# qirui-chen/RGA3-release

Hardware: AMD Instinct MI355X
Metric: video-QA samples/sec (fwd+bwd) at 7B/16-frame — full RGA3 training step (Qwen2.5-VL-7B + SAM2-L + mask losses + AdamW) (higher is better)
Workload: dtype bf16

## Files before the change

include/rga3_hip.h:

```cpp
#ifndef RGA3_HIP_H
#define RGA3_HIP_H

#include <stddef.h>
#include <stdint.h>

#ifdef __cplusplus
extern "C" {
#endif

#define RGA3_EINVAL (-22)

#define RGA3_BF16 0
#define RGA3_F32 1

#define RGA3_ACT_NONE 0
#define RGA3_ACT_GELU 1
#define RGA3_ACT_SWIGLU 2
#define RGA3_ACT_RELU 3

int rga3_version(void);
int rga3_last_error(char* buf, size_t n);

int rga3_gemm_bf16(const void* A, const void* W, const void* bias, const void* residual, const void* colscale, void* C, int64_t M, int64_t N,
                   int64_t K, int64_t lda, int64_t ldw, int64_t ldc, int64_t ldr, int act, int out_dtype, int tile,
// ... 14 lines not shown


int rga3_attn_varlen_fwd(const void* q, const void* k, const void* v, void* o, float* lse, const int32_t* cu_q,
                         const int32_t* cu_k, int nseg, int max_q, int64_t total_q, int Hq, int Hkv, int D, int64_t q_st, int64_t q_sh,
                         int64_t k_st, int64_t k_sh, int64_t v_st, int64_t v_sh, int64_t o_st, int64_t o_sh,
                         float scale, int causal, int impl, float* split_ws, int64_t split_ws_elems, int max_k, int block_q, int block_k, void* stream);
int rga3_attn_varlen_fwd_rope(const void* q, const void* k, const void* v, void* o, float* lse, const int32_t* cu_q, const int32_t* cu_k, int nseg, int max_q,
                              int64_t total_q, int Hq, int Hkv, int D, int64_t q_st, int64_t q_sh, int64_t k_st, int64_t k_sh, int64_t v_st, int64_t v_sh,
                              int64_t o_st, int64_t o_sh, float scale, int causal, const float* cos_q, const float* sin_q, const float* cos_k,
                              const float* sin_k, void* stream);

int rga3_rmsnorm_fwd(const void* x, const void* add, const void* weight, void* y, void* res_out, int64_t rows,
                     int64_t dim, int64_t ldx, float eps, void* stream);

int rga3_layernorm_fwd(const void* x, const void* weight, const void* bias, void* y, int64_t rows, int64_t dim,
                       int64_t ldx, int64_t ldy, float eps, int act, void* stream);
int rga3_layernorm_stats(const void* x, float* stats, int64_t rows, int64_t dim, int64_t ldx, float eps, void* stream);
int rga3_gemm_ln_bf16(const void* A, const void* Wf, const void* bias, const float* colc, const float* rowstat, void* C, int64_t M, int64_t N, int64_t K,
                      int64_t lda, int64_t ldw, int64_t ldc, int act, int tile, void* stream);
int64_t rga3_gemm_lnsum_slices(int64_t N, int tile);
int rga3_gemm_lnsum_bf16(const void* A, const void* W, const void* bias, const void* residual, void* C, int64_t M, int64_t N, int64_t K, int64_t lda,
                         int64_t ldw, int64_t ldc, int64_t ldr, int tile, float* row_parts, void* stream);
int rga3_gemm_lnq_bf16(const void* A, const void* Wf, const void* bias, const float* colc, const float* row_parts, int64_t slices, int64_t norm_width, float eps,
                       void* C, int64_t M, int64_t N, int64_t K, int64_t lda, int64_t ldw, int64_t ldc, int act, int tile, void* stream);

int rga3_rope_inplace(void* x, const float* cos, const float* sin, int64_t T, int h0, int nh, int D, int64_t st,
                      int64_t sh, void* stream);

int rga3_gather_rows(const void* table, const int64_t* idx, void* out, int64_t n_idx, int64_t rows_per_idx,
                     int64_t dim, int64_t ld_table, int64_t ld_out, void* stream);
int rga3_scatter_rows(const void* src, const int64_t* idx, void* out, int64_t n_idx, int64_t rows_per_idx, int64_t dim,
                      int64_t ld_src, int64_t ld_out, void* stream);

int rga3_pad_cols(const void* src, void* dst, int64_t rows, int64_t cols, int64_t ld_src, int64_t ld_dst, void* stream);

int rga3_silu_mul(const void* a, const void* b, void* out, int64_t n, void* stream);
int rga3_add(const void* a, const void* b, void* out, int64_t n, void* stream);

int rga3_cross_entropy_rows(const void* logits, int logits_dtype, const int64_t* labels, float* row_loss,
                            void* dlogits, int64_t rows, int64_t V, int64_t ld, float grad_scale, void* stream);


int rga3_im2col(const void* img, void* out, int64_t F, int C, int H, int W, int ks, int stride, int pad, int64_t ld_out,
                void* stream);
int rga3_maxpool2x2_win(const void* x, void* y, int64_t nwin, int w, int C, int64_t ldx, int64_t ldy, void* stream);
int rga3_upsample2x_add(const void* a, const void* b, void* out, int64_t F, int H, int W, int C, void* stream);
int rga3_add_bcast(const void* a, const void* b, void* out, int64_t rows, int64_t rows_b, int C, int64_t lda, int64_t ldb,
                   int64_t ldo, float alpha, void* stream);
int rga3_bilinear(const void* in, int in_dtype, float* out, const int32_t* plane_idx, int64_t N, int Hi, int Wi, int Ho, int Wo,
                  void* stream);
int rga3_conv3x3s2(const void* x, int x_dtype, const void* w, const void* bias, void* y, int64_t F, int H, int W, int Cin, int Cout,
                   float sig_scale, float sig_bias, void* stream);
int rga3_decimg_rows(const void* keys, int64_t keys_stride, const void* pe, int64_t pe_stride, int hw, const void* kt, const void* vt, int nk, const void* wq, const void* bq,
                     const void* wo, const void* bo, const void* ln_w, const void* ln_b, float eps, const void* wk2, const void* bk2, const void* wv2, const void* bv2,
                     void* keys_out, int64_t keys_out_stride, void* k2, void* v2, int64_t kv_stride, int v2_transposed, float scale, int64_t M, void* stream);
int rga3_attn_fewq(const void* q, int64_t q_stride, const void* k, int64_t k_stride, int64_t k_head_stride, const void* vt, const void* vbias, void* out, int64_t out_stride,
                   int frames, int nq, int nk, int H, float scale, void* stream);
int rga3_copy_many(void* const* dst, const void* const* src, const int64_t* bytes, int n, void* stream);
int rga3_conv3x3s2_ln_gelu(const void* x, int x_dtype, const void* w, const void* bias, const void* ln_w, const void* ln_b, float eps, void* y, int64_t F, int H, int W,
                           int Cin, int Cout, float sig_scale, float sig_bias, void* stream);
int rga3_im2col3x3s2(const void* x, void* cols, int64_t F, int H, int W, int C, void* stream);
int rga3_dwconv7x7(const void* x, const void* w, const void* bias, void* y, int64_t F, int H, int W, int C, void* stream);
int rga3_rope_axial_inplace(void* x, const float* cos, const float* sin, int64_t n_rope, int nq, int C, int64_t ldx, void* stream);
int rga3_pixel_shuffle2x(const void* g, const void* bias, const void* add, void* out, int64_t F, int H, int W, int Co, int act, void* stream);
int rga3_bce_dice_sums(const float* logits, const float* targets, float* out4, int64_t n_masks, int64_t hw, void* stream);
int64_t rga3_bce_dice_sums_ws_floats(int64_t n_masks, int64_t hw);
int rga3_bce_dice_sums_det(const float* logits, const float* targets, float* out4, float* ws, int64_t ws_floats, int64_t n_masks, int64_t hw, void* stream);
int64_t rga3_mask_jf_ws_bytes(int64_t frames, int64_t h, int64_t w);
int rga3_mask_jf_counts(const void* seg, const void* ann, const void* void_pixels, int64_t* counts, void* ws, int64_t ws_bytes, int64_t frames, int64_t h, int64_t w,
                        int radius, void* stream);
int64_t rga3_stom_ws_bytes(int64_t frames, int64_t h, int64_t w);
int rga3_stom_flow(const float* tracks, const void* visibility, int* records, int64_t frames, int64_t n_points, int vip_frame_idx, void* stream);
int rga3_stom_shift_composite(const void* frames_u8, const void* overlay_rgba, const int* records, void* out, int64_t frames, int64_t h, int64_t w, int vip_frame_idx,
                              void* stream);
int rga3_stom_mask_composite(const void* frames_u8, const void* overlay_rgba, const float* tracks, const void* visibility, void* out, void* ws, int64_t ws_bytes,
                             int64_t frames, int64_t h, int64_t w, int64_t n_points, int vip_frame_idx, const void* spans, int ksize, const void* half_widths,
                             int radius, void* stream);


int rga3_attn_varlen_bwd(const void* q, const void* k, const void* v, const void* o, const void* dout, const float* lse, void* dq,
                         void* dk, void* dv, float* delta_ws, const int32_t* cu_q, const int32_t* cu_k, int nseg, int max_q,
                         int max_k, int64_t total_q, int Hq, int Hkv, int D, const int64_t* strides16, float scale, int causal,
                         float* dkv_ws, int64_t total_k, void* stream);
int rga3_hiera_mlp144(const void* x, const void* w1f, const float* c1, const void* d1, const void* w2, const void* b2, void* y, int64_t M, float eps, void* stream);
int64_t rga3_hiera_mlp288_pack_bytes(void);
int rga3_hiera_mlp288_pack(const void* w1f, const float* c1, const void* d1, const void* w2, void* pack, void* stream);
int rga3_hiera_mlp288(const void* x, const void* pack, const void* b2, void* y, int64_t M, float eps, void* stream);
int rga3_mlp3_rows(const void* const* ptrs, const int64_t* dims, int n, int64_t B, void* stream);
int rga3_sam_select_objptr(const void* iou, const void* obj, const void* toks, int64_t tok_bstride, int C, const void* w0, const void* b0, const void* w1, const void* b1,
                           const void* w2, const void* b2, const void* no_obj_ptr, int64_t* best, int32_t* sel, void* obj_ptr, int64_t B, void* stream);
int64_t rga3_memattn_cross_ws_floats(int64_t Nq, int nsplit);
int rga3_memattn_cross(const void* q, const void* k, const void* m, void* out, int64_t Nq, int64_t Nk, int64_t q_stride, int64_t k_stride, int64_t m_stride,
                       int64_t out_stride, float scale, int nsplit, float* ws, void* stream);
int rga3_memlayer_rows(const void* a, int64_t a_stride, int K1, const float* part_o, const float* part_ml, int nsplit, const void* w1, const void* b1,
                       const void* res, int64_t res_stride, void* x_out, int64_t x_stride, const void* ln_w, const void* ln_b, float eps, void* t_out,
                       int64_t t_stride, const void* w2, const void* b2, int N2, void* y_out, int64_t y_stride, const float* cos, const float* sin,
                       int rope_cols, int nq, int64_t M, void* stream);
int rga3_gemm_rows16_many(const void* const* ptrs, const int64_t* dims, int n, void* stream);
int rga3_gemm_stream_k_timeouts(const void* workspace);
int64_t rga3_gemm_timeout_counter_offset(void);
int rga3_gemm_ragged_plan(int64_t M, int64_t N, int64_t K, int cus, int split, int* plan, unsigned* start);
int rga3_gemm_tiles(int entry, int* ids, int* bm, int* bn, int cap);
int rga3_gemm_candidates(int entry, int64_t M, int64_t N, int64_t K, int act, int out_dtype, int epilogue, int* ids, int cap);
int rga3_gemm_tn_slices(int64_t M, int64_t N, int64_t K);
int rga3_rmsnorm_bwd(const void* x, const void* weight, const void* dy, const void* add, void* dx, int64_t rows, int64_t dim, float eps,
                     void* stream);
int rga3_dropout_bf16(const void* x, void* y, int64_t n, float p, int64_t seed, int accumulate, void* stream);
int rga3_dropout_pair_bf16(const void* xa, const void* xb, void* ya, void* yb, int64_t n, float pa, int64_t seed_a, float pb, int64_t seed_b, int sum, void* stream);
int rga3_swiglu_fwd(const void* gu, void* a, int64_t T, int64_t I, void* stream);
int rga3_swiglu_bwd(const void* gu, const void* da, void* dgu, int64_t T, int64_t I, void* stream);
int rga3_transpose16(const void* in, void* out, int64_t R, int64_t C, int64_t ld_in, int64_t ld_out, void* stream);
int rga3_transpose16_many(const void* const* ptrs, const int64_t* dims, int n, void* stream);
int rga3_segment_sum_rows(const void* x, const int64_t* rows, const int64_t* offsets, void* out, int64_t n_out, int64_t dim, int64_t ldx,
                          void* stream);
int rga3_adamw_step(void* param, float* master, const void* grad, float* m, float* v, int64_t n, float lr, float beta1, float beta2,
                    float eps, float weight_decay, int step, float grad_scale, void* stream);
int rga3_sumsq_accum(const void* g, float* out, int64_t n, void* stream);
int rga3_sumsq_det(const void* g, int64_t n, float* partials, int64_t partials_cap, float* out, int accumulate, void* stream);
int rga3_adamw_step_clip(void* param, float* master, const void* grad, float* m, float* v, int64_t n, float lr, float beta1, float beta2,
                         float eps, float weight_decay, int step, const float* sumsq, float max_norm, void* stream);
int rga3_adamw_step_clip_rows(void* param, float* master, const void* grad, float* m, float* v, int64_t rows, int64_t row_len, const uint8_t* row_active,
                              float lr, float beta1, float beta2, float eps, int step, const float* sumsq, float max_norm, void* stream);
int rga3_scatter_add_rows(void* dst, const int64_t* idx, const void* src, int64_t n, int64_t dim, int64_t ld_dst, int64_t ld_src, float scale,
                          void* stream);


int64_t rga3_layernorm_bwd_ws_floats(int64_t rows, int64_t dim);
int rga3_layernorm_bwd(const void* x, const void* weight, const void* dy, void* dx, float* dweight, float* dbias, int64_t rows, int64_t dim,
                       float eps, float* ws, int64_t ws_floats, void* stream);
int rga3_colsum_accum(const void* x, float* out, int64_t rows, int64_t cols, int64_t ld, void* stream);
int64_t rga3_colsum_ws_floats(int64_t rows, int64_t cols);
int rga3_colsum(const void* x, float* out, int64_t rows, int64_t cols, int64_t ld, float* ws, int64_t ws_floats, void* counters, void* stream);
int rga3_act(const void* a, const void* dy, void* out, int64_t n, int kind, void* stream);
int rga3_bilinear_bwd(const float* dout, float* din, const int32_t* plane_idx, int64_t N, int Hi, int Wi, int Ho, int Wo, void* stream);
int rga3_mask_product(const void* hyper, const void* up, float* masks, int64_t B, int64_t NM, int64_t P, int64_t C, void* stream);
int64_t rga3_mask_product_bwd_ws_floats(int64_t B, int64_t NM, int64_t P, int64_t C);
int rga3_mask_product_bwd(const float* dmasks, const void* hyper, const void* up, void* dup, void* dhyper, int64_t B, int64_t NM, int64_t P, int64_t C,
                          float* ws, int64_t ws_floats, void* stream);
int rga3_pixel_shuffle2x_bwd(const void* dout, void* dg, int64_t F, int H, int W, int Co, void* stream);
int rga3_bce_dice_grad(const float* logits, const float* targets, const float* sums4, float* dlogits, int64_t n_masks, int64_t hw,
                       float coef_bce, float coef_dice, void* stream);
int rga3_bce_dice_grad_dev(const float* logits, const float* targets, const float* sums4, float* dlogits, int64_t n_masks, int64_t hw,
                           const float* coef_bce_dev, const float* coef_dice_dev, void* stream);

int rga3_pil_bicubic_coeffs(int in_size, int out_size, int32_t* bounds, int32_t* kk, int64_t kk_capacity, int* ksize_out);
int rga3_sam_preprocess_u8(const void* frames, int64_t T, int H, int W, int out_h, int out_w, const int32_t* bh, const int32_t* kh,
                           int ksize_h, const int32_t* bv, const int32_t* kv, int ksize_v, void* tmp, void* dst_u8, void* dst_bf16,
                           const float* mean3, const float* std3, void* stream);

int rga3_qwen_norm_lut(const float* mean3, const float* std3, int fused, float* lut768);
int rga3_qwen_patchify_u8(const void* frames, int64_t T, int h, int w, const float* lut768, void* out, int out_dtype, int patch, int tpatch,
                          int merge, void* stream);

int rga3_quant_fp8_rows(const void* x, void* q, float* scales, int64_t rows, int64_t K, int64_t ldx, int64_t ldq, void* stream);
int rga3_gemm_fp8(const void* Aq, const void* Wq, const float* sa, const float* sw, const void* bias, const void* residual, void* C, int64_t M,
                  int64_t N, int64_t K, int64_t lda, int64_t ldw, int64_t ldc, int64_t ldr, void* stream);
int rga3_swiglu_fwd_quant_fp8(const void* gu, void* q, float* scales, int64_t T, int64_t I, void* stream);
int rga3_swiglu_bwd_quant_fp8(const void* gu, const void* da, void* q, float* scales, int64_t T, int64_t I, void* stream);

#ifdef __cplusplus
}
#endif
#endif
```

rga3-release_amd/csrc/attn_bwd.hip:

```cpp
#include "common.h"

namespace rga3 {

struct AttnBwdArgs {
    const unsigned short *q, *k, *v, *o, *dout;
    unsigned short *dq, *dk, *dv;
    const float* lse;
    float* delta;
    const int *cu_q, *cu_k;
    long q_st, q_sh, k_st, k_sh, v_st, v_sh, o_st, o_sh, do_st, do_sh, dq_st, dq_sh, dk_st, dk_sh, dv_st, dv_sh;
    int Hq, Hkv, D;
    long total_q;
    float scale, scale_log2;
    int causal;
    float* dkv_ws;
    long total_k;
    int gx, gy;
};

constexpr int BT = 64;

template <int DP, int QT, int NWAVE, bool PAIR>
__global__ __launch_bounds__(64 * NWAVE) void attn_bwd_dq_kernel(AttnBwdArgs p) {
    constexpr int NT = 64 * NWAVE;
    constexpr int BLOCK_M = NWAVE * QT * 16;
    constexpr int CH = DP / 8;
    constexpr int STRIDE = DP * 2 + 32;
    constexpr int DS = DP / 32, DT = DP / 16;
    constexpr int LOADS = (BT * CH) / NT;
    static_assert((BT * CH) % NT == 0, "tile chunks must divide evenly over threads");

    extern __shared__ __attribute__((aligned(16))) char smem[];
    char* Ks = smem;
    char* Vs = smem + BT * STRIDE;

    const int tid = threadIdx.x, lane = tid & 63;
    const int wid = __builtin_amdgcn_readfirstlane(tid >> 6);
    const int g = lane >> 4, c = lane & 15;
    const Wg3 wg = xcd_decode3(p.gx, p.gy);
    const int seg = wg.z, hq = wg.y;
    const int hk = hq / (p.Hq / p.Hkv);
    const int qs = p.cu_q[seg], Lq = p.cu_q[seg + 1] - qs;
    const int ks = p.cu_k[seg], Lk = p.cu_k[seg + 1] - ks;
    const int shift = Lk - Lq;
    const int nqb = (Lq + BLOCK_M - 1) / BLOCK_M;
    int qb_first = wg.x, qb_second = -1;
    if constexpr (PAIR) {
        qb_first = nqb - 1 - wg.x;
        qb_second = wg.x;
        if (qb_second > qb_first) return;
        if (qb_second == qb_first) qb_second = -1;
    } else if (qb_first >= nqb) {
        return;
    }
    for (int pass = 0; pass < (PAIR ? 2 : 1); ++pass) {
    const int qbi = pass == 0 ? qb_first : qb_second;
    if (qbi < 0) break;
    if (pass == 1) __syncthreads();
    const int qb0 = qbi * BLOCK_M;
    const int qw0 = qb0 + wid * (QT * 16);

    bf16x8 qf[QT][DS], dof[QT][DS];
    float lse2[QT], dl[QT];
#pragma unroll
    for (int t = 0; t < QT; ++t) {
        const int qi = qw0 + t * 16 + c;
        const bool ok = qi < Lq;
#pragma unroll
        for (int ds = 0; ds < DS; ++ds) {
            const int d = ds * 32 + g * 8;
            u32x4 z = {0u, 0u, 0u, 0u}, y = {0u, 0u, 0u, 0u};
            if (ok && d < p.D) {
                z = *(const u32x4*)(p.q + (long)(qs + qi) * p.q_st + (long)hq * p.q_sh + d);
                y = *(const u32x4*)(p.dout + (long)(qs + qi) * p.do_st + (long)hq * p.do_sh + d);
            }
            qf[t][ds] = __builtin_bit_cast(bf16x8, z);
            dof[t][ds] = __builtin_bit_cast(bf16x8, y);
        }
        lse2[t] = ok ? p.lse[(long)hq * p.total_q + qs + qi] * 1.4426950408889634f : 0.f;
    }
#pragma unroll
    for (int t = 0; t < QT; ++t) {
        const int qi = qw0 + t * 16 + c;
        const bool ok = qi < Lq;
        float dp = 0.f;
#pragma unroll
        for (int ds = 0; ds < DS; ++ds) {
            const int d = ds * 32 + g * 8;
            if (ok && d < p.D) {
                const u32x4 ov = *(const u32x4*)(p.o + (long)(qs + qi) * p.o_st + (long)hq * p.o_sh + d);
                const u32x4 dv = __builtin_bit_cast(u32x4, dof[t][ds]);
#pragma unroll
                for (int i = 0; i < 4; ++i) {
                    dp += __uint_as_float(ov[i] << 16) * __uint_as_float(dv[i] << 16);
                    dp += __uint_as_float(ov[i] & 0xffff0000u) * __uint_as_float(dv[i] & 0xffff0000u);
                }
            }
        }
        dp += __shfl_xor(dp, 16, 64);
        dp += __shfl_xor(dp, 32, 64);
        dl[t] = ok ? dp : 0.f;
        if (ok && g == 0) p.delta[(long)hq * p.total_q + qs + qi] = dp;
    }

    f32x4 dqacc[QT][DT];
#pragma unroll
// ... 14 lines not shown
            const int r = idx / CH, ch = idx % CH;
            const int key = kt * BT + r;
            u32x4 zk = {0u, 0u, 0u, 0u}, zv = {0u, 0u, 0u, 0u};
            if (key < Lk && ch * 8 < p.D) {
                zk = *(const u32x4*)(p.k + (long)(ks + key) * p.k_st + (long)hk * p.k_sh + ch * 8);
                zv = *(const u32x4*)(p.v + (long)(ks + key) * p.v_st + (long)hk * p.v_sh + ch * 8);
            }
            kreg[i] = zk;
            vreg[i] = zv;
        }
    };
    auto store_tile = [&]() {
#pragma unroll
        for (int i = 0; i < LOADS; ++i) {
            const int idx = tid + i * NT;
            const int r = idx / CH, ch = idx % CH;
            *(u32x4*)(Ks + r * STRIDE + ch * 16) = kreg[i];
            *(u32x4*)(Vs + r * STRIDE + ch * 16) = vreg[i];
        }
    };

    if (ntiles > 0) load_tile(0);
    for (int kt = 0; kt < ntiles; ++kt) {
        __syncthreads();
        store_tile();
        __syncthreads();
        if (kt + 1 < ntiles) load_tile(kt + 1);
        const int k0 = kt * BT;
        const bool need_mask = (k0 + BT > Lk) || (p.causal && (k0 + BT - 1 > qb0 + shift));
#pragma unroll
        for (int t = 0; t < QT; ++t) {
            const int qi = qw0 + t * 16 + c;
            f32x4 s[4], dp[4];
#pragma unroll
            for (int j = 0; j < 4; ++j) { s[j] = f32x4{0.f, 0.f, 0.f, 0.f}; dp[j] = f32x4{0.f, 0.f, 0.f, 0.f}; }
#pragma unroll
            for (int j = 0; j < 4; ++j)
#pragma unroll
                for (int ds = 0; ds < DS; ++ds) {
                    bf16x8 kf = *(const bf16x8*)(Ks + (j * 16 + c) * STRIDE + ds * 64 + g * 16);
                    bf16x8 vf = *(const bf16x8*)(Vs + (j * 16 + c) * STRIDE + ds * 64 + g * 16);
                    s[j] = __builtin_amdgcn_mfma_f32_16x16x32_bf16(kf, qf[t][ds], s[j], 0, 0, 0);
                    dp[j] = __builtin_amdgcn_mfma_f32_16x16x32_bf16(vf, dof[t][ds], dp[j], 0, 0, 0);
                }
            bf16x8 dsf[2];
#pragma unroll
            for (int ss = 0; ss < 2; ++ss) {
                float e[8];
#pragma unroll
                for (int u = 0; u < 8; ++u) {
                    const int j = 2 * ss + (u >> 2), r = u & 3;
                    float pr = __builtin_amdgcn_exp2f(s[j][r] * p.scale_log2 - lse2[t]);
                    if (need_mask) {
                        const int key = k0 + j * 16 + 4 * g + r;
                        const bool ok = (key < Lk) && (!p.causal || key <= qi + shift);
                        pr = ok ? pr : 0.f;
                    }
                    if (qi >= Lq) pr = 0.f;
                    e[u] = pr * (dp[j][r] - dl[t]) * p.scale;
                }
                u32x4 pk;
                pk[0] = pack_bf2(e[0], e[1]); pk[1] = pack_bf2(e[2], e[3]); pk[2] = pack_bf2(e[4], e[5]); pk[3] = pack_bf2(e[6], e[7]);
                dsf[ss] = __builtin_bit_cast(bf16x8, pk);
            }
#pragma unroll
            for (int d = 0; d < DT; ++d)
#pragma unroll
                for (int ss = 0; ss < 2; ++ss) {
                    const char* a0 = Ks + (ss * 32 + 4 * g + (c >> 2)) * STRIDE + (d * 16 + 4 * (c & 3)) * 2;
                    bf16x4 lo = __builtin_amdgcn_ds_read_tr16_b64_v4bf16((__attribute__((address_space(3))) bf16x4*)(a0));
                    bf16x4 hi = __builtin_amdgcn_ds_read_tr16_b64_v4bf16((__attribute__((address_space(3))) bf16x4*)(a0 + 16 * STRIDE));
                    bf16x8 kt8;
                    kt8[0] = lo[0]; kt8[1] = lo[1]; kt8[2] = lo[2]; kt8[3] = lo[3];
                    kt8[4] = hi[0]; kt8[5] = hi[1]; kt8[6] = hi[2]; kt8[7] = hi[3];
                    dqacc[t][d] = __builtin_amdgcn_mfma_f32_16x16x32_bf16(kt8, dsf[ss], dqacc[t][d], 0, 0, 0);
                }
        }
    }
#pragma unroll
    for (int t = 0; t < QT; ++t) {
        const int qi = qw0 + t * 16 + c;
        if (qi < Lq) {
            unsigned short* row = p.dq + (long)(qs + qi) * p.dq_st + (long)hq * p.dq_sh;
#pragma unroll
            for (int d = 0; d < DT; ++d) {
                const int dd = d * 16 + 4 * g;
                if (dd < p.D) {
                    u32x2 pk;
                    pk[0] = pack_bf2(dqacc[t][d][0], dqacc[t][d][1]);
                    pk[1] = pack_bf2(dqacc[t][d][2], dqacc[t][d][3]);
                    *(u32x2*)(row + dd) = pk;
                }
            }
        }
    }
    }
}

template <int DP, int NWAVE, bool SPLIT, bool PAIR>
__global__ __launch_bounds__(64 * NWAVE) void attn_bwd_dkv_kernel(AttnBwdArgs p) {
    constexpr int NT = 64 * NWAVE;
    constexpr int BLOCK_N = NWAVE * 16;
    constexpr int CH = DP / 8;
    constexpr int STRIDE = DP * 2 + 32;
    constexpr int DS = DP / 32, DT = DP / 16;
    constexpr int LOADS = (BT * CH) / NT;
    static_assert((BT * CH) % NT == 0, "tile chunks must divide evenly over threads");

    extern __shared__ __attribute__((aligned(16))) char smem[];
    char* Qs = smem;
    char* Os = smem + BT * STRIDE;
    float* Ls = (float*)(smem + 2 * BT * STRIDE);

    const int tid = threadIdx.x, lane = tid & 63;
    const int wid = __builtin_amdgcn_readfirstlane(tid >> 6);
    const int g = lane >> 4, c = lane & 15;
    const Wg3 wg = xcd_decode3(p.gx, p.gy);
    const int seg = wg.z;
    const int group = p.Hq / p.Hkv;
    const int hk = SPLIT ? wg.y / group : wg.y;
    const int hh0 = SPLIT ? wg.y % group : 0, hh1 = SPLIT ? hh0 + 1 : group;
    const int qs = p.cu_q[seg], Lq = p.cu_q[seg + 1] - qs;
    const int ks = p.cu_k[seg], Lk = p.cu_k[seg + 1] - ks;
    const int shift = Lk - Lq;
    const int nkb = (Lk + BLOCK_N - 1) / BLOCK_N;
    int kb_first = wg.x, kb_second = -1;
    if constexpr (PAIR) {
        kb_first = wg.x;
        kb_second = nkb - 1 - wg.x;
        if (kb_first > kb_second) return;
        if (kb_second == kb_first) kb_second = -1;
    } else if (kb_first >= nkb) {
        return;
    }
    for (int pass = 0; pass < (PAIR ? 2 : 1); ++pass) {
    const int kbi = pass == 0 ? kb_first : kb_second;
    if (kbi < 0) break;
    if (pass == 1) __syncthreads();
    const int kb0 = kbi * BLOCK_N;
    const int key = kb0 + wid * 16 + c;

    bf16x8 kf[DS], vf[DS];
#pragma unroll
    for (int ds = 0; ds < DS; ++ds) {
        const int d = ds * 32 + g * 8;
        u32x4 z = {0u, 0u, 0u, 0u}, y = {0u, 0u, 0u, 0u};
        if (key < Lk && d < p.D) {
            z = *(const u32x4*)(p.k + (long)(ks + key) * p.k_st + (long)hk * p.k_sh + d);
            y = *(const u32x4*)(p.v + (long)(ks + key) * p.v_st + (long)hk * p.v_sh + d);
        }
        kf[ds] = __builtin_bit_cast(bf16x8, z);
        vf[ds] = __builtin_bit_cast(bf16x8, y);
    }
    f32x4 dkacc[DT], dvacc[DT];
#pragma unroll
    for (int d = 0; d < DT; ++d) { dkacc[d] = f32x4{0.f, 0.f, 0.f, 0.f}; dvacc[d] = f32x4{0.f, 0.f, 0.f, 0.f}; }

    int q_begin = 0;
    if (p.causal) q_begin = max(0, kb0 - shift);
    const int t0 = q_begin / BT;
    const int ntq = (Lq + BT - 1) / BT;

    u32x4 qreg[LOADS], oreg[LOADS];
    float lreg = 0.f, dreg = 0.f;
    auto load_tile = [&](int hq_, int qt_) {
#pragma unroll
        for (int i = 0; i < LOADS; ++i) {
            const int idx = tid + i * NT;
            const int r = idx / CH, ch = idx % CH;
            const int qi = qt_ * BT + r;
            u32x4 zq = {0u, 0u, 0u, 0u}, zo = {0u, 0u, 0u, 0u};
            if (qi < Lq && ch * 8 < p.D) {
                zq = *(const u32x4*)(p.q + (long)(qs + qi) * p.q_st + (long)hq_ * p.q_sh + ch * 8);
                zo = *(const u32x4*)(p.dout + (long)(qs + qi) * p.do_st + (long)hq_ * p.do_sh + ch * 8);
            }
            qreg[i] = zq;
            oreg[i] = zo;
        }
        if (tid < BT) {
            const int qi = qt_ * BT + tid;
            lreg = (qi < Lq) ? p.lse[(long)hq_ * p.total_q + qs + qi] * 1.4426950408889634f : 0.f;
            dreg = (qi < Lq) ? p.delta[(long)hq_ * p.total_q + qs + qi] : 0.f;
        }
// ... 16 lines not shown
        const int hq = hk * group + hh;
        for (int qt = t0; qt < ntq; ++qt) {
            __syncthreads();
            store_tile();
            __syncthreads();
            if (qt + 1 < ntq) load_tile(hq, qt + 1);
            else if (hh + 1 < hh1) load_tile(hq + 1, t0);
            const int q0 = qt * BT;
            f32x4 s[4], dp[4];
#pragma unroll
            for (int j = 0; j < 4; ++j) { s[j] = f32x4{0.f, 0.f, 0.f, 0.f}; dp[j] = f32x4{0.f, 0.f, 0.f, 0.f}; }
#pragma unroll
            for (int j = 0; j < 4; ++j)
#pragma unroll
                for (int ds = 0; ds < DS; ++ds) {
                    bf16x8 qa = *(const bf16x8*)(Qs + (j * 16 + c) * STRIDE + ds * 64 + g * 16);
                    bf16x8 oa = *(const bf16x8*)(Os + (j * 16 + c) * STRIDE + ds * 64 + g * 16);
                    s[j] = __builtin_amdgcn_mfma_f32_16x16x32_bf16(qa, kf[ds], s[j], 0, 0, 0);
                    dp[j] = __builtin_amdgcn_mfma_f32_16x16x32_bf16(oa, vf[ds], dp[j], 0, 0, 0);
                }
            bf16x8 pf[2], dsf[2];
#pragma unroll
            for (int ss = 0; ss < 2; ++ss) {
                float e[8], f[8];
#pragma unroll
                for (int u = 0; u < 8; ++u) {
                    const int j = 2 * ss + (u >> 2), r = u & 3;
                    const int ql = j * 16 + 4 * g + r;
                    const int qi = q0 + ql;
                    float pr = __builtin_amdgcn_exp2f(s[j][r] * p.scale_log2 - Ls[ql]);
                    const bool ok = (qi < Lq) && (key < Lk) && (!p.causal || key <= qi + shift);
                    pr = ok ? pr : 0.f;
                    e[u] = pr;
                    f[u] = pr * (dp[j][r] - Ls[BT + ql]) * p.scale;
                }
                u32x4 a, b;
                a[0] = pack_bf2(e[0], e[1]); a[1] = pack_bf2(e[2], e[3]); a[2] = pack_bf2(e[4], e[5]); a[3] = pack_bf2(e[6], e[7]);
                b[0] = pack_bf2(f[0], f[1]); b[1] = pack_bf2(f[2], f[3]); b[2] = pack_bf2(f[4], f[5]); b[3] = pack_bf2(f[6], f[7]);
                pf[ss] = __builtin_bit_cast(bf16x8, a);
                dsf[ss] = __builtin_bit_cast(bf16x8, b);
            }
#pragma unroll
            for (int d = 0; d < DT; ++d)
#pragma unroll
                for (int ss = 0; ss < 2; ++ss) {
                    const int roff = (ss * 32 + 4 * g + (c >> 2)) * STRIDE + (d * 16 + 4 * (c & 3)) * 2;
                    bf16x4 ol = __builtin_amdgcn_ds_read_tr16_b64_v4bf16((__attribute__((address_space(3))) bf16x4*)(Os + roff));
                    bf16x4 oh = __builtin_amdgcn_ds_read_tr16_b64_v4bf16((__attribute__((address_space(3))) bf16x4*)(Os + roff + 16 * STRIDE));
                    bf16x4 ql_ = __builtin_amdgcn_ds_read_tr16_b64_v4bf16((__attribute__((address_space(3))) bf16x4*)(Qs + roff));
                    bf16x4 qh_ = __builtin_amdgcn_ds_read_tr16_b64_v4bf16((__attribute__((address_space(3))) bf16x4*)(Qs + roff + 16 * STRIDE));
                    bf16x8 ot, qt8;
                    ot[0] = ol[0]; ot[1] = ol[1]; ot[2] = ol[2]; ot[3] = ol[3]; ot[4] = oh[0]; ot[5] = oh[1]; ot[6] = oh[2]; ot[7] = oh[3];
                    qt8[0] = ql_[0]; qt8[1] = ql_[1]; qt8[2] = ql_[2]; qt8[3] = ql_[3]; qt8[4] = qh_[0]; qt8[5] = qh_[1]; qt8[6] = qh_[2]; qt8[7] = qh_[3];
                    dvacc[d] = __builtin_amdgcn_mfma_f32_16x16x32_bf16(ot, pf[ss], dvacc[d], 0, 0, 0);
                    dkacc[d] = __builtin_amdgcn_mfma_f32_16x16x32_bf16(qt8, dsf[ss], dkacc[d], 0, 0, 0);
                }
        }
    }
    if constexpr (SPLIT) {
        if (key < Lk) {
            const long half = (long)group * p.total_k * p.Hkv * p.D;
            float* wk = p.dkv_ws + (((long)hh0 * p.total_k + ks + key) * p.Hkv + hk) * p.D;
#pragma unroll
            for (int d = 0; d < DT; ++d) {
                const int dd = d * 16 + 4 * g;
                if (dd < p.D) {
                    *(f32x4*)(wk + dd) = dkacc[d];
                    *(f32x4*)(wk + half + dd) = dvacc[d];
                }
            }
        }
        continue;
    }
    if (key < Lk) {
        unsigned short* rk = p.dk + (long)(ks + key) * p.dk_st + (long)hk * p.dk_sh;
        unsigned short* rv = p.dv + (long)(ks + key) * p.dv_st + (long)hk * p.dv_sh;
#pragma unroll
        for (int d = 0; d < DT; ++d) {
            const int dd = d * 16 + 4 * g;
            if (dd < p.D) {
                u32x2 a, b;
                a[0] = pack_bf2(dkacc[d][0], dkacc[d][1]); a[1] = pack_bf2(dkacc[d][2], dkacc[d][3]);
                b[0] = pack_bf2(dvacc[d][0], dvacc[d][1]); b[1] = pack_bf2(dvacc[d][2], dvacc[d][3]);
                *(u32x2*)(rk + dd) = a;
                *(u32x2*)(rv + dd) = b;
            }
        }
    }
    }
}

__global__ __launch_bounds__(256) void attn_dkv_reduce_kernel(AttnBwdArgs p) {
    const int group = p.Hq / p.Hkv;
    const int d4 = p.D / 4;
    const long idx = (long)blockIdx.x * 256 + threadIdx.x;
    const long total = p.total_k * p.Hkv * d4;
    if (idx >= total) return;
    const int dd = (int)(idx % d4) * 4;
    const long row = idx / d4;
    const int hk = (int)(row % p.Hkv);
    const long key = row / p.Hkv;
    const long plane = p.total_k * p.Hkv * (long)p.D, half = (long)group * plane;
    const float* w = p.dkv_ws + row * p.D + dd;
    f32x4 sk = *(const f32x4*)w, sv = *(const f32x4*)(w + half);
    for (int h = 1; h < group; ++h) {
        sk += *(const f32x4*)(w + h * plane);
        sv += *(const f32x4*)(w + half + h * plane);
    }
    u32x2 a, b;
    a[0] = pack_bf2(sk[0], sk[1]); a[1] = pack_bf2(sk[2], sk[3]);
    b[0] = pack_bf2(sv[0], sv[1]); b[1] = pack_bf2(sv[2], sv[3]);
    *(u32x2*)(p.dk + key * p.dk_st + (long)hk * p.dk_sh + dd) = a;
    *(u32x2*)(p.dv + key * p.dv_st + (long)hk * p.dv_sh + dd) = b;
}

template <auto K>
static int launch_bwd_grid(AttnBwdArgs& a, int lds, unsigned gx, int gy, int nseg, int nwave, hipStream_t st, const char* name) {
    a.gx = (int)gx; a.gy = gy;
    return launch_lds<K>(dim3(gx * (unsigned)gy * (unsigned)nseg), dim3(64 * nwave), lds, st, name, a);
}

template <int DP>
static int launch_bwd(const AttnBwdArgs& a0, int nseg, int max_q, int max_k, hipStream_t st) {
    AttnBwdArgs a = a0;
    a.gx = 1; a.gy = 1;
    constexpr int NW = (DP == 128) ? 8 : 4;
#ifdef RGA3_BWD_DQ_QT2
    constexpr int QT = 2, NWQ = 4;
#else
    constexpr int QT = (DP >= 128) ? 1 : 2, NWQ = NW;
#endif
    constexpr int BLOCK_M = NWQ * QT * 16;
    constexpr int LDS_DQ = 2 * BT * (DP * 2 + 32);
    constexpr int LDS_DKV = 2 * BT * (DP * 2 + 32) + 2 * BT * 4;
    const unsigned nqb = (unsigned)cdiv(max_q, BLOCK_M), nkb = (unsigned)cdiv(max_k, 16 * NW);
    const bool pair = a.causal && nqb >= 4 && nkb >= 4;
    const unsigned gq = pair ? (nqb + 1) / 2 : nqb, gk = pair ? (nkb + 1) / 2 : nkb;
    if (int rc = pair ? launch_bwd_grid<attn_bwd_dq_kernel<DP, QT, NWQ, true>>(a, LDS_DQ, gq, a.Hq, nseg, NWQ, st, "attn_bwd_dq_kernel")
                      : launch_bwd_grid<attn_bwd_dq_kernel<DP, QT, NWQ, false>>(a, LDS_DQ, gq, a.Hq, nseg, NWQ, st, "attn_bwd_dq_kernel"))
        return rc;
    if (a.dkv_ws && a.Hq > a.Hkv) {
        if (int rc = pair ? launch_bwd_grid<attn_bwd_dkv_kernel<DP, NW, true, true>>(a, LDS_DKV, gk, a.Hq, nseg, NW, st, "attn_bwd_dkv_kernel<split>")
                          : launch_bwd_grid<attn_bwd_dkv_kernel<DP, NW, true, false>>(a, LDS_DKV, gk, a.Hq, nseg, NW, st, "attn_bwd_dkv_kernel<split>"))
            return rc;
        const long rows = a.total_k * a.Hkv;
        hipLaunchKernelGGL(attn_dkv_reduce_kernel, dim3((unsigned)cdiv(rows * (a.D / 4), 256)), dim3(256), 0, st, a);
        RGA3_CHECK_LAUNCH("attn_dkv_reduce_kernel");
        return 0;
    }
    return pair ? launch_bwd_grid<attn_bwd_dkv_kernel<DP, NW, false, true>>(a, LDS_DKV, gk, a.Hkv, nseg, NW, st, "attn_bwd_dkv_kernel")
                : launch_bwd_grid<attn_bwd_dkv_kernel<DP, NW, false, false>>(a, LDS_DKV, gk, a.Hkv, nseg, NW, st, "attn_bwd_dkv_kernel");
}

}

using namespace rga3;

extern "C" int rga3_attn_varlen_bwd(const void* q, const void* k, const void* v, const void* o, const void* dout, const float* lse,
                                    void* dq, void* dk, void* dv, float* delta_ws, const int32_t* cu_q, const int32_t* cu_k, int nseg,
                                    int max_q, int max_k, int64_t total_q, int Hq, int Hkv, int D, const int64_t* strides16, float scale,
                                    int causal, float* dkv_ws, int64_t total_k, void* stream) {
    RGA3_CHECK_ARG(q && k && v && o && dout && lse && dq && dk && dv && delta_ws && cu_q && cu_k && strides16, "attn_bwd: null pointer");
    RGA3_CHECK_ARG(nseg > 0 && max_q > 0 && max_k > 0 && total_q > 0, "attn_bwd: sizes");
    RGA3_CHECK_ARG(Hq > 0 && Hkv > 0 && Hq % Hkv == 0, "attn_bwd: Hq=%d Hkv=%d", Hq, Hkv);
    RGA3_CHECK_ARG(D >= 8 && D <= 128 && D % 8 == 0, "attn_bwd: head dim %d unsupported (multiple of 8, <= 128)", D);
    for (int i = 0; i < 16; ++i) RGA3_CHECK_ARG(strides16[i] % 4 == 0, "attn_bwd: stride %d must be a multiple of 4 elements", i);
    for (int i = 0; i < 10; ++i) RGA3_CHECK_ARG(strides16[i] % 8 == 0, "attn_bwd: input stride %d must be a multiple of 8 elements", i);
    {
        static const char* const names[8] = {"q", "k", "v", "o", "dout", "dq", "dk", "dv"};
        for (int i = 0; i < 8; ++i) {
            const bool kv = i == 1 || i == 2 || i == 6 || i == 7;
            RGA3_CHECK_HEADS("attn_bwd", names[i], strides16[2 * i], strides16[2 * i + 1], kv ? total_k : total_q, kv ? Hkv : Hq, D);
        }
    }
    AttnBwdArgs a;
    a.q = (const unsigned short*)q; a.k = (const unsigned short*)k; a.v = (const unsigned short*)v; a.o = (const unsigned short*)o;
    a.dout = (const unsigned short*)dout; a.dq = (unsigned short*)dq; a.dk = (unsigned short*)dk; a.dv = (unsigned short*)dv;
    a.lse = lse; a.delta = delta_ws; a.cu_q = cu_q; a.cu_k = cu_k;
    a.q_st = strides16[0]; a.q_sh = strides16[1]; a.k_st = strides16[2]; a.k_sh = strides16[3]; a.v_st = strides16[4]; a.v_sh = strides16[5];
    a.o_st = strides16[6]; a.o_sh = strides16[7]; a.do_st = strides16[8]; a.do_sh = strides16[9]; a.dq_st = strides16[10]; a.dq_sh = strides16[11];
    a.dk_st = strides16[12]; a.dk_sh = strides16[13]; a.dv_st = strides16[14]; a.dv_sh = strides16[15];
    a.Hq = Hq; a.Hkv = Hkv; a.D = D; a.total_q = total_q; a.scale = scale; a.scale_log2 = scale * 1.4426950408889634f; a.causal = causal;
    a.dkv_ws = dkv_ws; a.total_k = total_k;
    RGA3_CHECK_ARG(!dkv_ws || (total_k > 0 && D % 4 == 0), "attn_bwd: dkv_ws needs total_k");
    hipStream_t st = (hipStream_t)stream;
    if (D <= 32) return launch_bwd<32>(a, nseg, max_q, max_k, st);
    if (D <= 64) return launch_bwd<64>(a, nseg, max_q, max_k, st);
    if (D <= 96) return launch_bwd<96>(a, nseg, max_q, max_k, st);
    return launch_bwd<128>(a, nseg, max_q, max_k, st);
}
```

rga3-release_amd/csrc/common.h:

```cpp
#pragma once
#include <hip/hip_runtime.h>

#include "errors.h"

namespace rga3 {

#define RGA3_CHECK_LAUNCH(name)                                                                  \
    do {                                                                                         \
        hipError_t e__ = hipGetLastError();                                                      \
        if (e__ != hipSuccess) return ::rga3::fail(-(int)e__, "%s: %s", name, hipGetErrorString(e__)); \
    } while (0)

struct LdsGrant { int bytes[16] = {0}; };
inline int grant_dyn_lds(const void* kern, int bytes, LdsGrant& g, const char* name) {
    if (bytes <= 48 * 1024) return 0;
    int dev = 0;
    if (hipGetDevice(&dev) != hipSuccess || dev < 0) dev = 0;
    const bool tracked = dev < 16;
    if (tracked && g.bytes[dev] >= bytes) return 0;
    hipError_t e = hipFuncSetAttribute(kern, hipFuncAttributeMaxDynamicSharedMemorySize, bytes);
    if (e != hipSuccess) return fail(-(int)e, "%s: hipFuncSetAttribute(%d B dynamic LDS): %s", name, bytes, hipGetErrorString(e));
    if (tracked) g.bytes[dev] = bytes;
    return 0;
}

template <auto K, class... A>
int launch_lds(dim3 grid, dim3 block, int lds, hipStream_t st, const char* name, const A&... args) {
    static LdsGrant grant;
    if (int rc = grant_dyn_lds((const void*)K, lds, grant, name)) return rc;
    hipLaunchKernelGGL(K, grid, block, lds, st, args...);
    RGA3_CHECK_LAUNCH(name);
    return 0;
}

typedef __attribute__((ext_vector_type(8))) __bf16 bf16x8;
typedef __attribute__((ext_vector_type(4))) __bf16 bf16x4;
typedef __attribute__((ext_vector_type(2))) __bf16 bf16x2;
typedef __attribute__((ext_vector_type(4))) float f32x4;
typedef __attribute__((ext_vector_type(16))) float f32x16;
typedef __attribute__((ext_vector_type(4))) unsigned int u32x4;
typedef __attribute__((ext_vector_type(2))) unsigned int u32x2;

typedef __attribute__((address_space(3))) void lds_void;
typedef const __attribute__((address_space(1))) void gbl_void;

__device__ __forceinline__ float bf2f(unsigned short u) { return __uint_as_float(((unsigned int)u) << 16); }
__device__ __forceinline__ unsigned short f2bf(float f) {
    __bf16 b = (__bf16)f;
    return __builtin_bit_cast(unsigned short, b);
}
__device__ __forceinline__ unsigned int pack_bf2(float lo, float hi) {
    bf16x2 v;
    v[0] = (__bf16)lo;
    v[1] = (__bf16)hi;
    return __builtin_bit_cast(unsigned int, v);
}
__device__ __forceinline__ void unpack8(const u32x4& v, float* f) {
#pragma unroll
    for (int i = 0; i < 4; ++i) {
        f[2 * i] = __uint_as_float(v[i] << 16);
        f[2 * i + 1] = __uint_as_float(v[i] & 0xffff0000u);
    }
}
__device__ __forceinline__ u32x4 pack8(const float* f) {
    u32x4 v;
#pragma unroll
    for (int i = 0; i < 4; ++i) v[i] = pack_bf2(f[2 * i], f[2 * i + 1]);
    return v;
}
__device__ __forceinline__ float bf16_round(float v) { return bf2f(f2bf(v)); }

__device__ __forceinline__ float wave_sum(float v) {
#pragma unroll
    for (int o = 32; o > 0; o >>= 1) v += __shfl_xor(v, o, 64);
    return v;
}
__device__ __forceinline__ float wave_max(float v) {
#pragma unroll
    for (int o = 32; o > 0; o >>= 1) v = fmaxf(v, __shfl_xor(v, o, 64));
    return v;
}

__device__ __forceinline__ float swiglu_fwd_elem(float g, float u) {
#pragma clang fp contract(off)
    const float silu = g / (1.f + __expf(-g));
    return bf16_round(silu) * u;
}
__device__ __forceinline__ void swiglu_bwd_elem(float g, float u, float d, float& dg, float& du) {
#pragma clang fp contract(off)
    const float sg = 1.f / (1.f + __expf(-g));
    const float silu = g * sg;
    du = d * silu;
    dg = d * u * sg * (1.f + g * (1.f - sg));
}

static inline int64_t cdiv(int64_t a, int64_t b) { return (a + b - 1) / b; }

static inline unsigned grid1d(long total, int per_block = 256, long cap = 256L * 32) {
    long b = cdiv(total, per_block);
    if (b < 1) b = 1;
    return (unsigned)(b > cap ? cap : b);
}

typedef const unsigned short* cus;
typedef unsigned short* us;

constexpr int kNumXCD = 8;

__device__ __forceinline__ unsigned xcd_remap(unsigned bid, unsigned nwg) {
    unsigned q = nwg / kNumXCD, r = nwg % kNumXCD, x = bid % kNumXCD;
    unsigned base = (x < r) ? x * (q + 1) : r * (q + 1) + (x - r) * q;
    return base + bid / kNumXCD;
}

struct Wg3 { int x, y, z; };
__device__ __forceinline__ Wg3 xcd_decode3(int gx, int gy) {
    const unsigned lid = xcd_remap(blockIdx.x, gridDim.x);
    Wg3 w;
    w.y = (int)(lid % (unsigned)gy);
    w.x = (int)((lid / (unsigned)gy) % (unsigned)gx);
    w.z = (int)(lid / ((unsigned)gy * (unsigned)gx));
    return w;
}

}
```

rga3-release_amd/csrc/rowops.hip:

```cpp
#include "common.h"

namespace rga3 {

template <int MAXC>
__global__ __launch_bounds__(256) void rmsnorm_kernel(const unsigned short* __restrict__ x, const unsigned short* __restrict__ add,
                                                      const unsigned short* __restrict__ w, unsigned short* __restrict__ y,
                                                      unsigned short* __restrict__ res_out, long rows, int dim, long ldx, float eps) {
    const int lane = threadIdx.x & 63;
    const long row = (long)blockIdx.x * 4 + (threadIdx.x >> 6);
    if (row >= rows) return;
    const int nch = dim / 8;
    u32x4 buf[MAXC], abuf[MAXC];
    float ss = 0.f;
#pragma unroll
    for (int i = 0; i < MAXC; ++i) {
        const int ch = lane + i * 64;
        if (ch < nch) {
            buf[i] = *(const u32x4*)(x + row * ldx + ch * 8);
            if (add) abuf[i] = *(const u32x4*)(add + row * ldx + ch * 8);
        }
    }
#pragma unroll
    for (int i = 0; i < MAXC; ++i) {
        const int ch = lane + i * 64;
        if (ch < nch) {
            u32x4 v = buf[i];
            float f[8];
            unpack8(v, f);
            if (add) {
                float fa[8];
                unpack8(abuf[i], fa);
#pragma unroll
                for (int e = 0; e < 8; ++e) f[e] = bf2f(f2bf(f[e] + fa[e]));
                v = pack8(f);
                if (res_out) *(u32x4*)(res_out + row * ldx + ch * 8) = v;
                buf[i] = v;
            }
#pragma unroll
            for (int e = 0; e < 8; ++e) ss += f[e] * f[e];
        }
        __builtin_amdgcn_sched_barrier(0);
    }
    ss = wave_sum(ss);
    const float rinv = rsqrtf(ss / (float)dim + eps);
#pragma unroll
    for (int i = 0; i < MAXC; ++i) asm volatile("" : "+v"(buf[i]));
#pragma unroll
    for (int i = 0; i < MAXC; ++i) {
        const int ch = lane + i * 64;
        if (ch < nch) {
            float f[8], fw[8];
            unpack8(buf[i], f);
            unpack8(*(const u32x4*)(w + ch * 8), fw);
#pragma unroll
            for (int e = 0; e < 8; ++e) f[e] = fw[e] * bf2f(f2bf(f[e] * rinv));
            *(u32x4*)(y + row * ldx + ch * 8) = pack8(f);
        }
        __builtin_amdgcn_sched_barrier(0);
    }
}

template <int MAXC>
__global__ __launch_bounds__(256) void rmsnorm_block_kernel(const unsigned short* __restrict__ x, const unsigned short* __restrict__ add,
                                                            const unsigned short* __restrict__ w, unsigned short* __restrict__ y,
                                                            unsigned short* __restrict__ res_out, long rows, int dim, long ldx, float eps) {
    __shared__ float part[4];
    const int tid = threadIdx.x;
    const long row = blockIdx.x;
    const int nch = dim / 8;
    u32x4 buf[MAXC], wv[MAXC];
    float ss = 0.f;
#pragma unroll
    for (int i = 0; i < MAXC; ++i) {
        const int ch = tid + i * 256;
        if (ch < nch) {
            u32x4 v = *(const u32x4*)(x + row * ldx + ch * 8);
            wv[i] = *(const u32x4*)(w + ch * 8);
            float f[8];
            unpack8(v, f);
            if (add) {
                u32x4 a = *(const u32x4*)(add + row * ldx + ch * 8);
                float fa[8];
                unpack8(a, fa);
#pragma unroll
                for (int e = 0; e < 8; ++e) f[e] = bf2f(f2bf(f[e] + fa[e]));
                v = pack8(f);
                if (res_out) *(u32x4*)(res_out + row * ldx + ch * 8) = v;
            }
            buf[i] = v;
#pragma unroll
            for (int e = 0; e < 8; ++e) ss += f[e] * f[e];
        }
    }
    ss = wave_sum(ss);
    if ((tid & 63) == 0) part[tid >> 6] = ss;
    __syncthreads();
    ss = part[0] + part[1] + part[2] + part[3];
    const float rinv = rsqrtf(ss / (float)dim + eps);
#pragma unroll
    for (int i = 0; i < MAXC; ++i) {
        const int ch = tid + i * 256;
        if (ch < nch) {
            float f[8], fw[8];
            unpack8(buf[i], f);
            unpack8(wv[i], fw);
#pragma unroll
            for (int e = 0; e < 8; ++e) f[e] = fw[e] * bf2f(f2bf(f[e] * rinv));
            *(u32x4*)(y + row * ldx + ch * 8) = pack8(f);
        }
    }
}

template <int MAXC>
__global__ __launch_bounds__(256) void layernorm_kernel(const unsigned short* __restrict__ x, const unsigned short* __restrict__ w,
                                                        const unsigned short* __restrict__ b, unsigned short* __restrict__ y,
                                                        long rows, int dim, long ldx, long ldy, float eps, int act, float* __restrict__ stats = nullptr) {
    const int lane = threadIdx.x & 63;
    const long row = (long)blockIdx.x * 4 + (threadIdx.x >> 6);
    if (row >= rows) return;
    const int nch = dim / 8;
    u32x4 buf[MAXC];
    float s1 = 0.f;
#pragma unroll
    for (int i = 0; i < MAXC; ++i) {
        const int ch = lane + i * 64;
        if (ch < nch) {
            buf[i] = *(const u32x4*)(x + row * ldx + ch * 8);
            float f[8];
            unpack8(buf[i], f);
#pragma unroll
            for (int e = 0; e < 8; ++e) s1 += f[e];
        }
    }
    const float mean = wave_sum(s1) / (float)dim;
    float s2 = 0.f;
#pragma unroll
    for (int i = 0; i < MAXC; ++i) {
        const int ch = lane + i * 64;
        if (ch < nch) {
            float f[8];
            unpack8(buf[i], f);
#pragma unroll
            for (int e = 0; e < 8; ++e) { float d = f[e] - mean; s2 += d * d; }
        }
    }
    const float rinv = rsqrtf(wave_sum(s2) / (float)dim + eps);
    if (stats) {
        if (lane == 0) *(float2*)(stats + 2 * row) = make_float2(mean, rinv);
        return;
    }
#pragma unroll
    for (int i = 0; i < MAXC; ++i) {
        const int ch = lane + i * 64;
        if (ch < nch) {
            float f[8], fw[8], fb[8];
            unpack8(buf[i], f);
            unpack8(*(const u32x4*)(w + ch * 8), fw);
            if (b) unpack8(*(const u32x4*)(b + ch * 8), fb);
#pragma unroll
            for (int e = 0; e < 8; ++e) {
                f[e] = (f[e] - mean) * rinv * fw[e] + (b ? fb[e] : 0.f);
                if (act == 1) { float t = bf2f(f2bf(f[e])); f[e] = 0.5f * t * (1.0f + erff(t * 0.70710678118654752f)); }
            }
            *(u32x4*)(y + row * ldy + ch * 8) = pack8(f);
        }
    }
}

template <int LPR>
__global__ __launch_bounds__(256) void layernorm_rows_kernel(const unsigned short* __restrict__ x, const unsigned short* __restrict__ w,
                                                             const unsigned short* __restrict__ b, unsigned short* __restrict__ y,
                                                             long rows, int dim, long ldx, long ldy, float eps, int act, float* __restrict__ stats = nullptr) {
    constexpr int RPW = 64 / LPR;
    const int lane = threadIdx.x & 63;
    const int sub = lane % LPR;
    const long row = ((long)blockIdx.x * 4 + (threadIdx.x >> 6)) * RPW + lane / LPR;
    const bool live = row < rows;
    const int nch = dim / 8;
    u32x4 buf[2];
    float f[2][8];
    float s1 = 0.f;
#pragma unroll
    for (int i = 0; i < 2; ++i) {
        const int ch = sub + i * LPR;
        buf[i] = u32x4{0u, 0u, 0u, 0u};
        if (live && ch < nch) buf[i] = *(const u32x4*)(x + row * ldx + ch * 8);
        unpack8(buf[i], f[i]);
#pragma unroll
        for (int e = 0; e < 8; ++e) s1 += f[i][e];
    }
#pragma unroll
// ... 45 lines not shown
#pragma unroll
    for (int i = 0; i < NCHL; ++i) {
        const int ch = sub + i * LPR;
        buf[i] = (ch < nch) ? *(const u32x4*)(x + rowc * ldx + ch * 8) : u32x4{0u, 0u, 0u, 0u};
    }
    float s1 = 0.f;
#pragma unroll
    for (int i = 0; i < NCHL; ++i) {
        float f[8];
        unpack8(buf[i], f);
#pragma unroll
        for (int e = 0; e < 8; ++e) s1 += f[e];
    }
#pragma unroll
    for (int o = LPR / 2; o > 0; o >>= 1) s1 += __shfl_xor(s1, o, 64);
    const float mean = s1 / (float)dim;
    float s2 = 0.f;
#pragma unroll
    for (int i = 0; i < NCHL; ++i) {
        if (sub + i * LPR < nch) {
            float f[8];
            unpack8(buf[i], f);
#pragma unroll
            for (int e = 0; e < 8; ++e) { const float d = f[e] - mean; s2 += d * d; }
        }
    }
#pragma unroll
    for (int o = LPR / 2; o > 0; o >>= 1) s2 += __shfl_xor(s2, o, 64);
    if (row < rows && sub == 0) *(float2*)(stats + 2 * row) = make_float2(mean, rsqrtf(s2 / (float)dim + eps));
}

__global__ __launch_bounds__(256) void layernorm_tiny_kernel(const unsigned short* __restrict__ x, const unsigned short* __restrict__ w,
                                                             const unsigned short* __restrict__ b, unsigned short* __restrict__ y, long rows, int dim, long ldx,
                                                             long ldy, float eps, int act) {
    const long row = (long)blockIdx.x * 256 + threadIdx.x;
    if (row >= rows) return;
    float f[16];
    float s1 = 0.f;
    for (int e = 0; e < dim; ++e) { f[e] = bf2f(x[row * ldx + e]); s1 += f[e]; }
    const float mean = s1 / (float)dim;
    float s2 = 0.f;
    for (int e = 0; e < dim; ++e) { const float d = f[e] - mean; s2 += d * d; }
    const float rinv = rsqrtf(s2 / (float)dim + eps);
    for (int e = 0; e < dim; ++e) {
        float v = (f[e] - mean) * rinv * bf2f(w[e]) + (b ? bf2f(b[e]) : 0.f);
        if (act == 1) { const float t = bf2f(f2bf(v)); v = 0.5f * t * (1.0f + erff(t * 0.70710678118654752f)); }
        y[row * ldy + e] = f2bf(v);
    }
}

template <int HG>
__global__ __launch_bounds__(256) void rope_kernel(unsigned short* __restrict__ x, const float* __restrict__ cs, const float* __restrict__ sn,
                                                   long T, int h0, int nh, int D, long st, long sh) {
    const int half = D / 2, cph = half / 8;
    const int ngrp = nh / HG;
    const long idx = (long)blockIdx.x * 256 + threadIdx.x;
    const long total = T * ngrp * cph;
    if (idx >= total) return;
    const int ch = (int)(idx % cph);
    const int hg = (int)((idx / cph) % ngrp);
    const long t = idx / ((long)cph * ngrp);
    float c1[8], s1[8], c2[8], s2[8];
    {
        const float* cp = cs + t * D + ch * 8;
        const float* sp = sn + t * D + ch * 8;
        *(f32x4*)&c1[0] = *(const f32x4*)cp;        *(f32x4*)&c1[4] = *(const f32x4*)(cp + 4);
        *(f32x4*)&s1[0] = *(const f32x4*)sp;        *(f32x4*)&s1[4] = *(const f32x4*)(sp + 4);
        *(f32x4*)&c2[0] = *(const f32x4*)(cp + half); *(f32x4*)&c2[4] = *(const f32x4*)(cp + half + 4);
        *(f32x4*)&s2[0] = *(const f32x4*)(sp + half); *(f32x4*)&s2[4] = *(const f32x4*)(sp + half + 4);
    }
    unsigned short* p1 = x + t * st + (long)(h0 + hg * HG) * sh + ch * 8;
    u32x4 va[HG], vb[HG];
#pragma unroll
    for (int h = 0; h < HG; ++h) {
        va[h] = *(const u32x4*)(p1 + h * sh);
        vb[h] = *(const u32x4*)(p1 + h * sh + half);
    }
#pragma unroll
    for (int h = 0; h < HG; ++h) {
        float a[8], b[8], o1[8], o2[8];
        unpack8(va[h], a);
        unpack8(vb[h], b);
#pragma unroll
        for (int e = 0; e < 8; ++e) {
            o1[e] = a[e] * c1[e] - b[e] * s1[e];
            o2[e] = b[e] * c2[e] + a[e] * s2[e];
        }
        *(u32x4*)(p1 + h * sh) = pack8(o1);
        *(u32x4*)(p1 + h * sh + half) = pack8(o2);
    }
}

template <bool SCATTER>
__global__ __launch_bounds__(256) void move_rows_kernel(const unsigned short* __restrict__ src, const long* __restrict__ idx,
                                                        unsigned short* __restrict__ dst, long n_idx, long rpi, int dim, long ld_src,
                                                        long ld_dst) {
    const int nch = dim / 8;
    const long total = n_idx * rpi * nch;
    for (long i = (long)blockIdx.x * 256 + threadIdx.x; i < total; i += (long)gridDim.x * 256) {
        const int ch = (int)(i % nch);
        const long r = i / nch;
        const long u = r / rpi, w = r % rpi;
        const long other = idx[u] * rpi + w;
        const long srow = SCATTER ? r : other, drow = SCATTER ? other : r;
        *(u32x4*)(dst + drow * ld_dst + ch * 8) = *(const u32x4*)(src + srow * ld_src + ch * 8);
    }
}

__global__ __launch_bounds__(256) void pad_cols_kernel(const unsigned short* __restrict__ src, unsigned short* __restrict__ dst, long rows,
                                                       int cols, long ld_src, long ld_dst) {
    const int nch = (int)(ld_dst / 8);
    const long total = rows * nch;
    for (long i = (long)blockIdx.x * 256 + threadIdx.x; i < total; i += (long)gridDim.x * 256) {
        const int ch = (int)(i % nch);
        const long r = i / nch;
        u32x4 v = {0u, 0u, 0u, 0u};
        if (ch * 8 + 8 <= cols && (ld_src & 7) == 0) {
            v = *(const u32x4*)(src + r * ld_src + ch * 8);
        } else if (ch * 8 < cols) {
            unsigned short tmp[8] = {0, 0, 0, 0, 0, 0, 0, 0};
            for (int e = 0; e < 8 && ch * 8 + e < cols; ++e) tmp[e] = src[r * ld_src + ch * 8 + e];
#pragma unroll
            for (int e = 0; e < 4; ++e) v[e] = (unsigned)tmp[2 * e] | ((unsigned)tmp[2 * e + 1] << 16);
        }
        *(u32x4*)(dst + r * ld_dst + ch * 8) = v;
    }
}

template <int OP>
__global__ __launch_bounds__(256) void ew2_kernel(const unsigned short* __restrict__ a, const unsigned short* __restrict__ b,
                                                  unsigned short* __restrict__ o, long n) {
    const long nv = n / 8;
    for (long i = (long)blockIdx.x * 256 + threadIdx.x; i < nv; i += (long)gridDim.x * 256) {
        float fa[8], fb[8];
        unpack8(*(const u32x4*)(a + i * 8), fa);
        unpack8(*(const u32x4*)(b + i * 8), fb);
#pragma unroll
        for (int e = 0; e < 8; ++e) {
            if (OP == 0) fa[e] = bf2f(f2bf(fa[e] / (1.f + __expf(-fa[e])))) * fb[e];
            else fa[e] = fa[e] + fb[e];
        }
        *(u32x4*)(o + i * 8) = pack8(fa);
    }
    if (blockIdx.x == 0 && threadIdx.x == 0) {
        for (long i = nv * 8; i < n; ++i) {
            float x = bf2f(a[i]), y = bf2f(b[i]);
            o[i] = f2bf(OP == 0 ? bf2f(f2bf(x / (1.f + __expf(-x)))) * y : x + y);
        }
    }
}

template <bool F32>
__global__ __launch_bounds__(256) void ce_rows_kernel(const void* __restrict__ logits, const long* __restrict__ labels, float* __restrict__ row_loss,
                                                      unsigned short* __restrict__ dlogits, long V, long ld, float gscale) {
    __shared__ float red_m[4], red_s[4];
    const long row = blockIdx.x;
    const long lab = labels[row];
    const int tid = threadIdx.x;
    if (lab < 0) {
        if (tid == 0) row_loss[row] = 0.f;
        if (dlogits)
            for (long i = tid; i < V; i += 256) dlogits[row * ld + i] = 0;
        return;
    }
    auto ld1 = [&](long i) -> float {
        if (F32) return ((const float*)logits)[row * ld + i];
        return bf2f(((const unsigned short*)logits)[row * ld + i]);
    };
    constexpr int EPV = F32 ? 4 : 8;
    const bool vec = (ld % EPV == 0) && ((((uintptr_t)logits) & 15) == 0);
// ... 9 lines not shown
    float m = -INFINITY;
    for (long j = tid; j < nv; j += 256) {
        float f[EPV];
        ldv(j, f);
#pragma unroll
        for (int e = 0; e < EPV; ++e) m = fmaxf(m, f[e]);
    }
    for (long i = nv * EPV + tid; i < V; i += 256) m = fmaxf(m, ld1(i));
    m = wave_max(m);
    if ((tid & 63) == 0) red_m[tid >> 6] = m;
    __syncthreads();
    const float M = fmaxf(fmaxf(red_m[0], red_m[1]), fmaxf(red_m[2], red_m[3]));
    float s = 0.f;
    for (long j = tid; j < nv; j += 256) {
        float f[EPV];
        ldv(j, f);
#pragma unroll
        for (int e = 0; e < EPV; ++e) s += __expf(f[e] - M);
    }
    for (long i = nv * EPV + tid; i < V; i += 256) s += __expf(ld1(i) - M);
    s = wave_sum(s);
    if ((tid & 63) == 0) red_s[tid >> 6] = s;
    __syncthreads();
    const float S = (red_s[0] + red_s[1]) + (red_s[2] + red_s[3]);
    const float lse = M + logf(S);
    if (tid == 0) row_loss[row] = lse - ld1(lab);
    if (dlogits) {
        const bool vout = vec && (ld % 8 == 0) && ((((uintptr_t)dlogits) & 15) == 0) && !F32;
        const long nvo = vout ? nv : 0;
        for (long j = tid; j < nvo; j += 256) {
            float f[8];
            unpack8(*(const u32x4*)((const unsigned short*)logits + row * ld + j * 8), f);
#pragma unroll
            for (int e = 0; e < 8; ++e) f[e] = (__expf(f[e] - lse) - ((j * 8 + e) == lab ? 1.f : 0.f)) * gscale;
            *(u32x4*)(dlogits + row * ld + j * 8) = pack8(f);
        }
        for (long i = nvo * 8 + tid; i < V; i += 256) {
            float pr = __expf(ld1(i) - lse);
            dlogits[row * ld + i] = f2bf((pr - (i == lab ? 1.f : 0.f)) * gscale);
        }
    }
}

}

using namespace rga3;

extern "C" int rga3_rmsnorm_fwd(const void* x, const void* add, const void* weight, void* y, void* res_out, int64_t rows,
                                int64_t dim, int64_t ldx, float eps, void* stream) {
    RGA3_CHECK_ARG(x && weight && y, "rmsnorm: null pointer");
    RGA3_CHECK_ARG(rows > 0 && dim > 0 && dim % 8 == 0 && ldx % 8 == 0 && dim <= 8192, "rmsnorm: rows=%ld dim=%ld ldx=%ld", (long)rows, (long)dim, (long)ldx);
    RGA3_CHECK_ARG(!res_out || add, "rmsnorm: res_out requires add");
    RGA3_CHECK_LD("rmsnorm", "ldx", ldx, dim, rows);
    hipStream_t st = (hipStream_t)stream;
    dim3 grid((unsigned)cdiv(rows, 4));
    const unsigned short *xp = (const unsigned short*)x, *ap = (const unsigned short*)add, *wp = (const unsigned short*)weight;
    unsigned short *yp = (unsigned short*)y, *rp = (unsigned short*)res_out;
    if (dim >= 2048 && dim <= 256 * 8 * 4) {
        const int nb = (int)cdiv(dim / 8, 256);
        dim3 g2((unsigned)rows);
        if (nb <= 2) hipLaunchKernelGGL(rmsnorm_block_kernel<2>, g2, dim3(256), 0, st, xp, ap, wp, yp, rp, (long)rows, (int)dim, (long)ldx, eps);
        else hipLaunchKernelGGL(rmsnorm_block_kernel<4>, g2, dim3(256), 0, st, xp, ap, wp, yp, rp, (long)rows, (int)dim, (long)ldx, eps);
        RGA3_CHECK_LAUNCH("rmsnorm_block_kernel");
        return 0;
    }
    const int nslot = (int)cdiv(dim / 8, 64);
#define RGA3_RMS(N) hipLaunchKernelGGL(rmsnorm_kernel<N>, grid, dim3(256), 0, st, xp, ap, wp, yp, rp, (long)rows, (int)dim, (long)ldx, eps)
    switch (nslot) {
        case 1: RGA3_RMS(1); break;
        case 2: RGA3_RMS(2); break;
        case 3: RGA3_RMS(3); break;
        case 4: RGA3_RMS(4); break;
        case 5: RGA3_RMS(5); break;
        case 6: RGA3_RMS(6); break;
        case 7: RGA3_RMS(7); break;
        case 8: RGA3_RMS(8); break;
        default: RGA3_RMS(16); break;
    }
#undef RGA3_RMS
    RGA3_CHECK_LAUNCH("rmsnorm_kernel");
    return 0;
}

extern "C" int rga3_layernorm_fwd(const void* x, const void* weight, const void* bias, void* y, int64_t rows, int64_t dim,
                                  int64_t ldx, int64_t ldy, float eps, int act, void* stream) {
    RGA3_CHECK_ARG(x && weight && y, "layernorm: null pointer");
    RGA3_CHECK_LD("layernorm", "ldx", ldx, dim, rows);
    RGA3_CHECK_LD("layernorm", "ldy", ldy, dim, rows);
    hipStream_t st = (hipStream_t)stream;
    if (rows > 0 && dim > 0 && dim <= 16 && (dim % 8 != 0 || ldx % 8 != 0 || ldy % 8 != 0)) {
        hipLaunchKernelGGL(layernorm_tiny_kernel, dim3((unsigned)cdiv(rows, 256)), dim3(256), 0, st, (const unsigned short*)x, (const unsigned short*)weight,
                           (const unsigned short*)bias, (unsigned short*)y, (long)rows, (int)dim, (long)ldx, (long)ldy, eps, act);
        RGA3_CHECK_LAUNCH("layernorm_tiny_kernel");
        return 0;
    }
    RGA3_CHECK_ARG(rows > 0 && dim > 0 && dim % 8 == 0 && ldx % 8 == 0 && ldy % 8 == 0 && dim <= 8192, "layernorm: rows=%ld dim=%ld", (long)rows, (long)dim);
    dim3 grid((unsigned)cdiv(rows, 4));
    const unsigned short *xp = (const unsigned short*)x, *wp = (const unsigned short*)weight, *bp = (const unsigned short*)bias;
    unsigned short* yp = (unsigned short*)y;
    if (dim <= 16 * 8 * 2) {
        hipLaunchKernelGGL(layernorm_rows_kernel<16>, dim3((unsigned)cdiv(rows, 16)), dim3(256), 0, st, xp, wp, bp, yp, (long)rows, (int)dim, (long)ldx, (long)ldy, eps, act, (float*)nullptr);
    } else if (dim <= 32 * 8 * 2) {
        hipLaunchKernelGGL(layernorm_rows_kernel<32>, dim3((unsigned)cdiv(rows, 8)), dim3(256), 0, st, xp, wp, bp, yp, (long)rows, (int)dim, (long)ldx, (long)ldy, eps, act, (float*)nullptr);
    } else if (dim <= 64 * 8 * 4) hipLaunchKernelGGL(layernorm_kernel<4>, grid, dim3(256), 0, st, xp, wp, bp, yp, (long)rows, (int)dim, (long)ldx, (long)ldy, eps, act, (float*)nullptr);
    else if (dim <= 64 * 8 * 8) hipLaunchKernelGGL(layernorm_kernel<8>, grid, dim3(256), 0, st, xp, wp, bp, yp, (long)rows, (int)dim, (long)ldx, (long)ldy, eps, act, (float*)nullptr);
    else hipLaunchKernelGGL(layernorm_kernel<16>, grid, dim3(256), 0, st, xp, wp, bp, yp, (long)rows, (int)dim, (long)ldx, (long)ldy, eps, act, (float*)nullptr);
    RGA3_CHECK_LAUNCH("layernorm_kernel");
    return 0;
}

extern "C" int rga3_layernorm_stats(const void* x, float* stats, int64_t rows, int64_t dim, int64_t ldx, float eps, void* stream) {
    RGA3_CHECK_ARG(x && stats && rows > 0 && dim > 0 && dim % 8 == 0 && ldx % 8 == 0 && dim <= 8192, "layernorm_stats: rows=%ld dim=%ld", (long)rows, (long)dim);
    RGA3_CHECK_ARG((((uintptr_t)x) & 15) == 0 && (((uintptr_t)stats) & 7) == 0, "layernorm_stats: pointer alignment");
    RGA3_CHECK_LD("layernorm_stats", "ldx", ldx, dim, rows);
    hipStream_t st = (hipStream_t)stream;
    const unsigned short* xp = (const unsigned short*)x;
    const unsigned short* nul = nullptr;
    dim3 grid((unsigned)cdiv(rows, 4));
    if (dim <= 16 * 8 * 2) hipLaunchKernelGGL(layernorm_rows_kernel<16>, dim3((unsigned)cdiv(rows, 16)), dim3(256), 0, st, xp, nul, nul, (unsigned short*)nullptr, (long)rows, (int)dim, (long)ldx, 0L, eps, 0, stats);
    else if (dim <= 32 * 8 * 2) hipLaunchKernelGGL(layernorm_rows_kernel<32>, dim3((unsigned)cdiv(rows, 8)), dim3(256), 0, st, xp, nul, nul, (unsigned short*)nullptr, (long)rows, (int)dim, (long)ldx, 0L, eps, 0, stats);
    else if (dim <= 8 * 9 * 8) hipLaunchKernelGGL((layernorm_stats_kernel<8, 9>), dim3((unsigned)cdiv(rows, 32)), dim3(256), 0, st, xp, stats, (long)rows, (int)dim, (long)ldx, eps);
    else if (dim <= 16 * 9 * 8) hipLaunchKernelGGL((layernorm_stats_kernel<16, 9>), dim3((unsigned)cdiv(rows, 16)), dim3(256), 0, st, xp, stats, (long)rows, (int)dim, (long)ldx, eps);
    else if (dim <= 64 * 8 * 4) hipLaunchKernelGGL(layernorm_kernel<4>, grid, dim3(256), 0, st, xp, nul, nul, (unsigned short*)nullptr, (long)rows, (int)dim, (long)ldx, 0L, eps, 0, stats);
    else if (dim <= 64 * 8 * 8) hipLaunchKernelGGL(layernorm_kernel<8>, grid, dim3(256), 0, st, xp, nul, nul, (unsigned short*)nullptr, (long)rows, (int)dim, (long)ldx, 0L, eps, 0, stats);
    else hipLaunchKernelGGL(layernorm_kernel<16>, grid, dim3(256), 0, st, xp, nul, nul, (unsigned short*)nullptr, (long)rows, (int)dim, (long)ldx, 0L, eps, 0, stats);
    RGA3_CHECK_LAUNCH("layernorm_stats");
    return 0;
}

extern "C" int rga3_rope_inplace(void* x, const float* cos, const float* sin, int64_t T, int h0, int nh, int D, int64_t st,
                                 int64_t sh, void* stream) {
    RGA3_CHECK_ARG(x && cos && sin, "rope: null pointer");
    RGA3_CHECK_ARG(T > 0 && nh > 0 && D > 0 && D % 16 == 0 && st % 8 == 0 && sh % 8 == 0, "rope: T=%ld nh=%d D=%d", (long)T, nh, D);
    RGA3_CHECK_ARG((((uintptr_t)cos | (uintptr_t)sin) & 15) == 0, "rope: cos/sin tables must be 16-byte aligned");
    RGA3_CHECK_ARG(h0 >= 0, "rope: h0 %d", h0);
    RGA3_CHECK_HEADS("rope", "x", st, sh, T, (int64_t)h0 + nh, D);
    if (nh % 4 == 0) {
        const long total = (long)T * (nh / 4) * (D / 16);
        hipLaunchKernelGGL(rope_kernel<4>, dim3((unsigned)cdiv(total, 256)), dim3(256), 0, (hipStream_t)stream, (unsigned short*)x, cos, sin, (long)T,
                           h0, nh, D, (long)st, (long)sh);
    } else {
        const long total = (long)T * nh * (D / 16);
        hipLaunchKernelGGL(rope_kernel<1>, dim3((unsigned)cdiv(total, 256)), dim3(256), 0, (hipStream_t)stream, (unsigned short*)x, cos, sin, (long)T,
                           h0, nh, D, (long)st, (long)sh);
    }
    RGA3_CHECK_LAUNCH("rope_kernel");
    return 0;
}

extern "C" int rga3_gather_rows(const void* table, const int64_t* idx, void* out, int64_t n_idx, int64_t rows_per_idx,
                                int64_t dim, int64_t ld_table, int64_t ld_out, void* stream) {
    RGA3_CHECK_ARG(table && idx && out, "gather_rows: null pointer");
    RGA3_CHECK_ARG(n_idx > 0 && rows_per_idx > 0 && dim > 0 && dim % 8 == 0 && ld_table % 8 == 0 && ld_out % 8 == 0, "gather_rows: bad shape");
    RGA3_CHECK_LD("gather_rows", "ld_table", ld_table, dim, 2);
    RGA3_CHECK_LD("gather_rows", "ld_out", ld_out, dim, n_idx * rows_per_idx);
    const long total = n_idx * rows_per_idx * (dim / 8);
    hipLaunchKernelGGL(move_rows_kernel<false>, dim3(grid1d(total)), dim3(256), 0, (hipStream_t)stream, (const unsigned short*)table,
                       (const long*)idx, (unsigned short*)out, (long)n_idx, (long)rows_per_idx, (int)dim, (long)ld_table, (long)ld_out);
    RGA3_CHECK_LAUNCH("gather_rows");
    return 0;
}

extern "C" int rga3_scatter_rows(const void* src, const int64_t* idx, void* out, int64_t n_idx, int64_t rows_per_idx, int64_t dim,
                                 int64_t ld_src, int64_t ld_out, void* stream) {
    RGA3_CHECK_ARG(src && idx && out, "scatter_rows: null pointer");
    RGA3_CHECK_ARG(n_idx > 0 && rows_per_idx > 0 && dim > 0 && dim % 8 == 0 && ld_src % 8 == 0 && ld_out % 8 == 0, "scatter_rows: bad shape");
// ... 53 lines not shown
```

rga3-release_amd/csrc/trainops.hip:

```cpp
#include "common.h"

namespace rga3 {

template <int MAXC>
__global__ __launch_bounds__(256) void rmsnorm_bwd_kernel(const unsigned short* __restrict__ x, const unsigned short* __restrict__ w,
                                                          const unsigned short* __restrict__ dy, const unsigned short* __restrict__ add,
                                                          unsigned short* __restrict__ dx, long rows, int dim, float eps) {
    const int lane = threadIdx.x & 63;
    const long row = (long)blockIdx.x * 4 + (threadIdx.x >> 6);
    if (row >= rows) return;
    const int nch = dim / 8;
    u32x4 xb[MAXC], gb[MAXC];
    float ss = 0.f, sg = 0.f;
#pragma unroll
    for (int i = 0; i < MAXC; ++i) {
        const int ch = lane + i * 64;
        if (ch < nch) {
            float fx[8], fd[8], fw[8];
            xb[i] = *(const u32x4*)(x + row * dim + ch * 8);
            unpack8(xb[i], fx);
            unpack8(*(const u32x4*)(dy + row * dim + ch * 8), fd);
            unpack8(*(const u32x4*)(w + ch * 8), fw);
#pragma unroll
            for (int e = 0; e < 8; ++e) {
                fd[e] *= fw[e];
                ss += fx[e] * fx[e];
                sg += fd[e] * fx[e];
            }
            gb[i] = pack8(fd);
        }
    }
    ss = wave_sum(ss);
    sg = wave_sum(sg);
    const float r = rsqrtf(ss / (float)dim + eps);
    const float coef = r * r * r * sg / (float)dim;
#pragma unroll
    for (int i = 0; i < MAXC; ++i) {
        const int ch = lane + i * 64;
        if (ch < nch) {
            float fx[8], fg[8], fa[8];
            unpack8(xb[i], fx);
            unpack8(gb[i], fg);
            if (add) unpack8(*(const u32x4*)(add + row * dim + ch * 8), fa);
#pragma unroll
            for (int e = 0; e < 8; ++e) fg[e] = r * fg[e] - fx[e] * coef + (add ? fa[e] : 0.f);
            *(u32x4*)(dx + row * dim + ch * 8) = pack8(fg);
        }
    }
}

template <int NC>
__global__ __launch_bounds__(256) void rmsnorm_bwd_block_kernel(const unsigned short* __restrict__ x, const unsigned short* __restrict__ w,
                                                                const unsigned short* __restrict__ dy, const unsigned short* __restrict__ add,
                                                                unsigned short* __restrict__ dx, int dim, float eps) {
    __shared__ float red[2][4];
    const int lane = threadIdx.x & 63, wv = threadIdx.x >> 6;
    const long row = blockIdx.x;
    const int nch = dim / 8;
    float fx[NC][8], fg[NC][8];
    float ss = 0.f, sg = 0.f;
#pragma unroll
    for (int i = 0; i < NC; ++i) {
        const int ch = threadIdx.x + i * 256;
        if (ch < nch) {
            float fw[8];
            unpack8(*(const u32x4*)(x + row * dim + ch * 8), fx[i]);
            unpack8(*(const u32x4*)(dy + row * dim + ch * 8), fg[i]);
            unpack8(*(const u32x4*)(w + ch * 8), fw);
#pragma unroll
            for (int e = 0; e < 8; ++e) {
                fg[i][e] *= fw[e];
                ss += fx[i][e] * fx[i][e];
                sg += fg[i][e] * fx[i][e];
            }
        }
    }
    ss = wave_sum(ss);
    sg = wave_sum(sg);
    if (lane == 0) { red[0][wv] = ss; red[1][wv] = sg; }
    __syncthreads();
    ss = (red[0][0] + red[0][1]) + (red[0][2] + red[0][3]);
    sg = (red[1][0] + red[1][1]) + (red[1][2] + red[1][3]);
    const float r = rsqrtf(ss / (float)dim + eps);
    const float coef = r * r * r * sg / (float)dim;
#pragma unroll
    for (int i = 0; i < NC; ++i) {
        const int ch = threadIdx.x + i * 256;
        if (ch < nch) {
            float fa[8], o[8];
            if (add) unpack8(*(const u32x4*)(add + row * dim + ch * 8), fa);
#pragma unroll
            for (int e = 0; e < 8; ++e) o[e] = r * fg[i][e] - fx[i][e] * coef + (add ? fa[e] : 0.f);
            *(u32x4*)(dx + row * dim + ch * 8) = pack8(o);
        }
    }
}

__global__ __launch_bounds__(256) void swiglu_bwd_kernel(const unsigned short* __restrict__ gu, const unsigned short* __restrict__ da,
                                                         unsigned short* __restrict__ dgu, long T, long I) {
    const long nch = I / 8;
    const long total = T * nch;
    for (long i = (long)blockIdx.x * 256 + threadIdx.x; i < total; i += (long)gridDim.x * 256) {
        const long ch = i % nch, t = i / nch;
        const long blk = ch / 2, half = ch % 2;
        const long goff = t * 2 * I + blk * 32 + half * 8;
        float g[8], u[8], d[8], dg[8], du[8];
        unpack8(*(const u32x4*)(gu + goff), g);
        unpack8(*(const u32x4*)(gu + goff + 16), u);
        unpack8(*(const u32x4*)(da + t * I + ch * 8), d);
#pragma unroll
        for (int e = 0; e < 8; ++e) swiglu_bwd_elem(g[e], u[e], d[e], dg[e], du[e]);
        *(u32x4*)(dgu + goff) = pack8(dg);
        *(u32x4*)(dgu + goff + 16) = pack8(du);
    }
}

__global__ __launch_bounds__(256) void swiglu_fwd_kernel(const unsigned short* __restrict__ gu, unsigned short* __restrict__ a, long T, long I) {
    const long nch = I / 8;
    const long total = T * nch;
    for (long i = (long)blockIdx.x * 256 + threadIdx.x; i < total; i += (long)gridDim.x * 256) {
        const long ch = i % nch, t = i / nch;
        const long blk = ch / 2, half = ch % 2;
        const long goff = t * 2 * I + blk * 32 + half * 8;
        float g[8], u[8], o[8];
        unpack8(*(const u32x4*)(gu + goff), g);
        unpack8(*(const u32x4*)(gu + goff + 16), u);
#pragma unroll
        for (int e = 0; e < 8; ++e) o[e] = swiglu_fwd_elem(g[e], u[e]);
        *(u32x4*)(a + t * I + ch * 8) = pack8(o);
    }
}

__global__ __launch_bounds__(256) void transpose16_kernel(const unsigned short* __restrict__ in, unsigned short* __restrict__ out, long R, long C,
                                                          long ldi, long ldo) {
    __shared__ unsigned short tile[64][66];
    const long r0 = (long)blockIdx.y * 64, c0 = (long)blockIdx.x * 64;
    const int tx = threadIdx.x & 63, ty = threadIdx.x >> 6;
    for (int i = ty; i < 64; i += 4) {
        const long r = r0 + i, c = c0 + tx;
        tile[i][tx] = (r < R && c < C) ? in[r * ldi + c] : (unsigned short)0;
    }
    __syncthreads();
    for (int i = ty; i < 64; i += 4) {
        const long c = c0 + i, r = r0 + tx;
        if (c < C && r < R) out[c * ldo + r] = tile[tx][i];
    }
}

constexpr int TR_MANY = 64;
struct TransposeMany {
// ... 71 lines not shown
    float s = 0.f;
    const long n8 = n / 8;
    for (long i = (long)blockIdx.x * 256 + threadIdx.x; i < n8; i += (long)gridDim.x * 256) {
        float f[8];
        unpack8(*(const u32x4*)(g + i * 8), f);
#pragma unroll
        for (int e = 0; e < 8; ++e) s += f[e] * f[e];
    }
    if (blockIdx.x == 0 && threadIdx.x < (n & 7)) {
        const float x = bf2f(g[n8 * 8 + threadIdx.x]);
        s += x * x;
    }
    s = wave_sum(s);
    if ((threadIdx.x & 63) == 0) red[threadIdx.x >> 6] = s;
    __syncthreads();
    if (threadIdx.x == 0) partials[blockIdx.x] = (red[0] + red[1]) + (red[2] + red[3]);
}

__global__ __launch_bounds__(256) void sumsq_finish_kernel(const float* __restrict__ partials, int np, float* __restrict__ out, int accumulate) {
    __shared__ float red[256];
    float s = 0.f;
    for (int i = threadIdx.x; i < np; i += 256) s += partials[i];
    red[threadIdx.x] = s;
    __syncthreads();
    for (int o = 128; o > 0; o >>= 1) {
        if ((int)threadIdx.x < o) red[threadIdx.x] += red[threadIdx.x + o];
        __syncthreads();
    }
    if (threadIdx.x == 0) out[0] = (accumulate ? out[0] : 0.f) + red[0];
}

__global__ __launch_bounds__(256) void adamw8_kernel(unsigned short* __restrict__ p, float* __restrict__ master, const unsigned short* __restrict__ g,
                                                     float* __restrict__ m, float* __restrict__ v, long n, float lr, float b1, float b2, float eps,
                                                     float wd, float bc1, float bc2, const float* __restrict__ sumsq, float max_norm,
                                                     const unsigned char* __restrict__ row_active, long row_len8) {
    float gscale = 1.f;
    if (sumsq) gscale = fminf(1.f, max_norm / (sqrtf(sumsq[0]) + 1e-6f));
    const long n8 = n / 8;
    const float decay = 1.f - lr * wd, ibc1 = 1.f / bc1, ibc2 = 1.f / bc2;
    for (long i = (long)blockIdx.x * 256 + threadIdx.x; i < n8; i += (long)gridDim.x * 256) {
        if (row_active && !row_active[i / row_len8]) continue;
        float gr[8], w[8], mi[8], vi[8];
        unpack8(*(const u32x4*)(g + i * 8), gr);
        *(f32x4*)(w) = *(const f32x4*)(master + i * 8);     *(f32x4*)(w + 4) = *(const f32x4*)(master + i * 8 + 4);
        *(f32x4*)(mi) = *(const f32x4*)(m + i * 8);         *(f32x4*)(mi + 4) = *(const f32x4*)(m + i * 8 + 4);
        *(f32x4*)(vi) = *(const f32x4*)(v + i * 8);         *(f32x4*)(vi + 4) = *(const f32x4*)(v + i * 8 + 4);
#pragma unroll
        for (int e = 0; e < 8; ++e) {
            const float x = gr[e] * gscale;
            mi[e] = b1 * mi[e] + (1.f - b1) * x;
            vi[e] = b2 * vi[e] + (1.f - b2) * x * x;
            w[e] = w[e] * decay - lr * (mi[e] * ibc1) / (sqrtf(vi[e] * ibc2) + eps);
        }
        *(f32x4*)(master + i * 8) = *(f32x4*)(w);           *(f32x4*)(master + i * 8 + 4) = *(f32x4*)(w + 4);
        *(f32x4*)(m + i * 8) = *(f32x4*)(mi);               *(f32x4*)(m + i * 8 + 4) = *(f32x4*)(mi + 4);
        *(f32x4*)(v + i * 8) = *(f32x4*)(vi);               *(f32x4*)(v + i * 8 + 4) = *(f32x4*)(vi + 4);
        *(u32x4*)(p + i * 8) = pack8(w);
    }
    if (blockIdx.x == 0 && threadIdx.x < (n & 7)) {
        const long i = n8 * 8 + threadIdx.x;
        const float x = bf2f(g[i]) * gscale;
        const float mm = b1 * m[i] + (1.f - b1) * x, vv = b2 * v[i] + (1.f - b2) * x * x;
        const float w = master[i] * decay - lr * (mm * ibc1) / (sqrtf(vv * ibc2) + eps);
        m[i] = mm; v[i] = vv; master[i] = w; p[i] = f2bf(w);
    }
}

__global__ __launch_bounds__(256) void scatter_add_rows_kernel(unsigned short* __restrict__ dst, const long* __restrict__ idx, const unsigned short* __restrict__ src,
                                                               long n, int dim, long ld_dst, long ld_src, float scale) {
    const int nch = dim / 8;
    for (long t = (long)blockIdx.x * 256 + threadIdx.x; t < n * nch; t += (long)gridDim.x * 256) {
        const long r = t / nch;
        const int ch = (int)(t % nch);
        float a[8], b[8];
        unsigned short* d = dst + idx[r] * ld_dst + ch * 8;
        unpack8(*(const u32x4*)d, a);
        unpack8(*(const u32x4*)(src + r * ld_src + ch * 8), b);
#pragma unroll
        for (int e = 0; e < 8; ++e) a[e] += scale * b[e];
        *(u32x4*)d = pack8(a);
    }
}

__device__ __forceinline__ unsigned dropout_hash(unsigned long long seed, unsigned long long ctr) {
    unsigned x = (unsigned)ctr ^ (unsigned)seed, y = (unsigned)(ctr >> 32) ^ (unsigned)(seed >> 32);
    x *= 0xcc9e2d51u; x = (x << 15) | (x >> 17); x *= 0x1b873593u;
    y ^= x; y = (y << 13) | (y >> 19); y = y * 5u + 0xe6546b64u;
    y ^= y >> 16; y *= 0x85ebca6bu; y ^= y >> 13; y *= 0xc2b2ae35u; y ^= y >> 16;
    return y;
}

__global__ __launch_bounds__(256) void dropout_kernel(const unsigned short* __restrict__ x, unsigned short* __restrict__ y, long n8, unsigned thr,
                                                      float inv_keep, unsigned long long seed, int accumulate) {
    for (long g = (long)blockIdx.x * 256 + threadIdx.x; g < n8; g += (long)gridDim.x * 256) {
        const u32x4 v = *(const u32x4*)(x + g * 8);
        u32x4 o = {0u, 0u, 0u, 0u};
        if (accumulate) o = *(const u32x4*)(y + g * 8);
#pragma unroll
        for (int j = 0; j < 4; ++j) {
            const unsigned h = dropout_hash(seed, (unsigned long long)g * 4 + j);
            const float lo = ((h & 0xffffu) >= thr) ? __uint_as_float(v[j] << 16) * inv_keep : 0.f;
            const float hi = ((h >> 16) >= thr) ? __uint_as_float(v[j] & 0xffff0000u) * inv_keep : 0.f;
            const float alo = accumulate ? __uint_as_float(o[j] << 16) : 0.f, ahi = accumulate ? __uint_as_float(o[j] & 0xffff0000u) : 0.f;
            o[j] = pack_bf2(alo + lo, ahi + hi);
        }
        *(u32x4*)(y + g * 8) = o;
    }
}

__global__ __launch_bounds__(256) void dropout_pair_kernel(const unsigned short* __restrict__ xa, const unsigned short* __restrict__ xb, unsigned short* ya,
                                                           unsigned short* yb, long n8, unsigned thr_a, float ik_a, unsigned long long seed_a, unsigned thr_b,
                                                           float ik_b, unsigned long long seed_b, int sum) {
    const bool same = xa == xb;
    for (long g = (long)blockIdx.x * 256 + threadIdx.x; g < n8; g += (long)gridDim.x * 256) {
        const u32x4 va = *(const u32x4*)(xa + g * 8);
        const u32x4 vb = same ? va : *(const u32x4*)(xb + g * 8);
        u32x4 o = {0u, 0u, 0u, 0u};
        if (sum) o = *(const u32x4*)(ya + g * 8);
        u32x4 oa, ob;
#pragma unroll
        for (int j = 0; j < 4; ++j) {
            const unsigned ha = dropout_hash(seed_a, (unsigned long long)g * 4 + j), hb = dropout_hash(seed_b, (unsigned long long)g * 4 + j);
            const float alo = ((ha & 0xffffu) >= thr_a) ? __uint_as_float(va[j] << 16) * ik_a : 0.f;
            const float ahi = ((ha >> 16) >= thr_a) ? __uint_as_float(va[j] & 0xffff0000u) * ik_a : 0.f;
            const float blo = ((hb & 0xffffu) >= thr_b) ? __uint_as_float(vb[j] << 16) * ik_b : 0.f;
            const float bhi = ((hb >> 16) >= thr_b) ? __uint_as_float(vb[j] & 0xffff0000u) * ik_b : 0.f;
            if (sum) {
                oa[j] = pack_bf2(__uint_as_float(o[j] << 16) + alo + blo, __uint_as_float(o[j] & 0xffff0000u) + ahi + bhi);
            } else {
                oa[j] = pack_bf2(alo, ahi);
                ob[j] = pack_bf2(blo, bhi);
            }
        }
        *(u32x4*)(ya + g * 8) = oa;
        if (!sum) *(u32x4*)(yb + g * 8) = ob;
    }
}

}

using namespace rga3;

extern "C" int rga3_rmsnorm_bwd(const void* x, const void* weight, const void* dy, const void* add, void* dx, int64_t rows, int64_t dim,
                                float eps, void* stream) {
    RGA3_CHECK_ARG(x && weight && dy && dx && rows > 0 && dim > 0 && dim % 8 == 0 && dim <= 8192, "rmsnorm_bwd: bad args");
    hipStream_t st = (hipStream_t)stream;
    if (dim > 1024) {
        dim3 gb((unsigned)rows);
        if (dim <= 2048) hipLaunchKernelGGL(rmsnorm_bwd_block_kernel<1>, gb, dim3(256), 0, st, (cus)x, (cus)weight, (cus)dy, (cus)add, (us)dx, (int)dim, eps);
        else if (dim <= 4096) hipLaunchKernelGGL(rmsnorm_bwd_block_kernel<2>, gb, dim3(256), 0, st, (cus)x, (cus)weight, (cus)dy, (cus)add, (us)dx, (int)dim, eps);
        else hipLaunchKernelGGL(rmsnorm_bwd_block_kernel<4>, gb, dim3(256), 0, st, (cus)x, (cus)weight, (cus)dy, (cus)add, (us)dx, (int)dim, eps);
        RGA3_CHECK_LAUNCH("rmsnorm_bwd_block");
        return 0;
    }
    dim3 grid((unsigned)cdiv(rows, 4));
    if (dim <= 2048) hipLaunchKernelGGL(rmsnorm_bwd_kernel<4>, grid, dim3(256), 0, st, (cus)x, (cus)weight, (cus)dy, (cus)add, (us)dx, (long)rows, (int)dim, eps);
    else if (dim <= 4096) hipLaunchKernelGGL(rmsnorm_bwd_kernel<8>, grid, dim3(256), 0, st, (cus)x, (cus)weight, (cus)dy, (cus)add, (us)dx, (long)rows, (int)dim, eps);
    else hipLaunchKernelGGL(rmsnorm_bwd_kernel<16>, grid, dim3(256), 0, st, (cus)x, (cus)weight, (cus)dy, (cus)add, (us)dx, (long)rows, (int)dim, eps);
    RGA3_CHECK_LAUNCH("rmsnorm_bwd");
    return 0;
}

extern "C" int rga3_dropout_bf16(const void* x, void* y, int64_t n, float p, int64_t seed, int accumulate, void* stream) {
    RGA3_CHECK_ARG(x && y && n > 0 && n % 8 == 0, "dropout: n=%ld must be a positive multiple of 8", (long)n);
    RGA3_CHECK_ARG(p >= 0.f && p < 1.f, "dropout: p=%f", p);
    const unsigned thr = (unsigned)(p * 65536.0f + 0.5f);
    const float inv_keep = 1.0f / (1.0f - (float)thr / 65536.0f);
    long blocks = cdiv(n / 8, 256);
    if (blocks > 65536) blocks = 65536;
    hipLaunchKernelGGL(dropout_kernel, dim3((unsigned)blocks), dim3(256), 0, (hipStream_t)stream, (const unsigned short*)x, (unsigned short*)y, (long)(n / 8),
                       thr, inv_keep, (unsigned long long)seed, accumulate);
    RGA3_CHECK_LAUNCH("dropout_kernel");
    return 0;
}

extern "C" int rga3_dropout_pair_bf16(const void* xa, const void* xb, void* ya, void* yb, int64_t n, float pa, int64_t seed_a, float pb, int64_t seed_b, int sum,
                                      void* stream) {
    RGA3_CHECK_ARG(xa && xb && ya && (sum || yb) && n > 0 && n % 8 == 0, "dropout_pair: null pointer / n=%ld must be a positive multiple of 8", (long)n);
    RGA3_CHECK_ARG(pa >= 0.f && pa < 1.f && pb >= 0.f && pb < 1.f, "dropout_pair: p=%f / %f", pa, pb);
    RGA3_CHECK_ARG((((uintptr_t)xa | (uintptr_t)xb | (uintptr_t)ya | (uintptr_t)yb) & 15) == 0, "dropout_pair: pointers must be 16-byte aligned");
    const unsigned ta = (unsigned)(pa * 65536.0f + 0.5f), tb = (unsigned)(pb * 65536.0f + 0.5f);
    long blocks = cdiv(n / 8, 256);
    if (blocks > 65536) blocks = 65536;
    hipLaunchKernelGGL(dropout_pair_kernel, dim3((unsigned)blocks), dim3(256), 0, (hipStream_t)stream, (cus)xa, (cus)xb, (us)ya, (us)yb, (long)(n / 8), ta,
                       1.0f / (1.0f - (float)ta / 65536.0f), (unsigned long long)seed_a, tb, 1.0f / (1.0f - (float)tb / 65536.0f), (unsigned long long)seed_b, sum);
    RGA3_CHECK_LAUNCH("dropout_pair_kernel");
    return 0;
}

extern "C" int rga3_swiglu_bwd(const void* gu, const void* da, void* dgu, int64_t T, int64_t I, void* stream) {
    RGA3_CHECK_ARG(gu && da && dgu && T > 0 && I > 0 && I % 16 == 0, "swiglu_bwd: bad args");
    hipLaunchKernelGGL(swiglu_bwd_kernel, dim3(grid1d(T * (I / 8))), dim3(256), 0, (hipStream_t)stream, (cus)gu, (cus)da, (us)dgu, (long)T, (long)I);
    RGA3_CHECK_LAUNCH("swiglu_bwd");
    return 0;
}

extern "C" int rga3_swiglu_fwd(const void* gu, void* a, int64_t T, int64_t I, void* stream) {
    RGA3_CHECK_ARG(gu && a && T > 0 && I > 0 && I % 16 == 0, "swiglu_fwd: bad args");
    hipLaunchKernelGGL(swiglu_fwd_kernel, dim3(grid1d(T * (I / 8))), dim3(256), 0, (hipStream_t)stream, (cus)gu, (us)a, (long)T, (long)I);
    RGA3_CHECK_LAUNCH("swiglu_fwd");
    return 0;
}

extern "C" int rga3_transpose16(const void* in, void* out, int64_t R, int64_t C, int64_t ld_in, int64_t ld_out, void* stream) {
    RGA3_CHECK_ARG(in && out && R > 0 && C > 0, "transpose16: bad args");
    RGA3_CHECK_LD("transpose16", "ld_in", ld_in, C, 2);
    RGA3_CHECK_LD("transpose16", "ld_out", ld_out, R, 2);
    RGA3_CHECK_ARG(cdiv(R, 64) <= 65535, "transpose16: too many rows");
    hipLaunchKernelGGL(transpose16_kernel, dim3((unsigned)cdiv(C, 64), (unsigned)cdiv(R, 64)), dim3(256), 0, (hipStream_t)stream, (cus)in, (us)out, (long)R,
                       (long)C, (long)ld_in, (long)ld_out);
    RGA3_CHECK_LAUNCH("transpose16");
    return 0;
}

extern "C" int rga3_transpose16_many(const void* const* ptrs, const int64_t* dims, int n, void* stream) {
    RGA3_CHECK_ARG(ptrs && dims && n >= 1 && n <= TR_MANY, "transpose16_many: n %d (1..64)", n);
    TransposeMany p;
    long mr = 0, mc = 0;
    for (int i = 0; i < n; ++i) {
        p.in[i] = (const unsigned short*)ptrs[2 * i];
        p.out[i] = (unsigned short*)ptrs[2 * i + 1];
        RGA3_CHECK_ARG(p.in[i] && p.out[i] && dims[2 * i] > 0 && dims[2 * i + 1] > 0 && dims[2 * i] < (1 << 30) && dims[2 * i + 1] < (1 << 30), "transpose16_many: matrix %d", i);
        p.R[i] = (int)dims[2 * i];
        p.C[i] = (int)dims[2 * i + 1];
        if (p.R[i] > mr) mr = p.R[i];
        if (p.C[i] > mc) mc = p.C[i];
    }
    RGA3_CHECK_ARG(cdiv(mr, 64) <= 65535, "transpose16_many: too many rows");
    hipLaunchKernelGGL(transpose16_many_kernel, dim3((unsigned)cdiv(mc, 64), (unsigned)cdiv(mr, 64), (unsigned)n), dim3(256), 0, (hipStream_t)stream, p);
    RGA3_CHECK_LAUNCH("transpose16_many");
    return 0;
}

extern "C" int rga3_segment_sum_rows(const void* x, const int64_t* rows, const int64_t* offsets, void* out, int64_t n_out, int64_t dim,
                                     int64_t ldx, void* stream) {
    RGA3_CHECK_ARG(x && rows && offsets && out && n_out > 0 && dim % 8 == 0 && ldx % 8 == 0, "segment_sum_rows: bad args");
    RGA3_CHECK_LD("segment_sum_rows", "ldx", ldx, dim, 2);
    hipLaunchKernelGGL(segment_sum_rows_kernel, dim3((unsigned)n_out), dim3(256), 0, (hipStream_t)stream, (cus)x, (const long*)rows, (const long*)offsets,
                       (us)out, (int)dim, (long)ldx);
    RGA3_CHECK_LAUNCH("segment_sum_rows");
    return 0;
}

extern "C" int rga3_adamw_step(void* param, float* master, const void* grad, float* m, float* v, int64_t n, float lr, float beta1, float beta2,
                               float eps, float weight_decay, int step, float grad_scale, void* stream) {
    RGA3_CHECK_ARG(param && master && grad && m && v && n > 0 && step >= 1, "adamw_step: bad args");
    const float bc1 = 1.f - powf(beta1, (float)step), bc2 = 1.f - powf(beta2, (float)step);
    hipLaunchKernelGGL(adamw_kernel, dim3(grid1d(n)), dim3(256), 0, (hipStream_t)stream, (us)param, master, (cus)grad, m, v, (long)n, lr, beta1, beta2, eps,
                       weight_decay, bc1, bc2, grad_scale);
    RGA3_CHECK_LAUNCH("adamw_step");
    return 0;
}

extern "C" int rga3_sumsq_accum(const void* g, float* out, int64_t n, void* stream) {
    RGA3_CHECK_ARG(g && out && n > 0, "sumsq_accum: bad args");
    hipLaunchKernelGGL(sumsq_kernel, dim3(grid1d(n, 256, 2048)), dim3(256), 0, (hipStream_t)stream, (cus)g, out, (long)n);
    RGA3_CHECK_LAUNCH("sumsq_accum");
    return 0;
}

extern "C" int rga3_sumsq_det(const void* g, int64_t n, float* partials, int64_t partials_cap, float* out, int accumulate, void* stream) {
    RGA3_CHECK_ARG(g && partials && out && n > 0 && partials_cap >= 1, "sumsq_det: bad args");
    RGA3_CHECK_ARG(((uintptr_t)g & 15) == 0, "sumsq_det: gradient pointer must be 16-byte aligned");
    long nb = cdiv(n, 8 * 256 * 4);
    if (nb < 1) nb = 1;
    if (nb > partials_cap) nb = partials_cap;
    if (nb > 2048) nb = 2048;
    hipLaunchKernelGGL(sumsq_partials_kernel, dim3((unsigned)nb), dim3(256), 0, (hipStream_t)stream, (cus)g, partials, (long)n);
// ... 40 lines not shown
```

rga3-release_amd/rga3/hip/lib.py:

```python
from __future__ import annotations

import ctypes as C
import os

_HERE = os.path.dirname(os.path.abspath(__file__))
LIB_PATH = os.path.normpath(os.path.join(_HERE, "..", "..", "librga3_hip.so"))

_p, _i, _i64, _f, _sz = C.c_void_p, C.c_int, C.c_int64, C.c_float, C.c_size_t

SIGNATURES = {
    "rga3_version": [],
    "rga3_last_error": [C.c_char_p, _sz],
    "rga3_gemm_bf16": [_p, _p, _p, _p, _p, _p, _i64, _i64, _i64, _i64, _i64, _i64, _i64, _i, _i, _i, _p, _i64, _p],
    "rga3_gemm_rms_bf16": [_p, _p, _p, _p, _p, _i64, _i64, _i64, _i64, _i64, _i64, _i64, _i, _i, _p, _i64, _p, _i64, _f, _p, _p],
    "rga3_gemm_workspace_bytes": [],
    "rga3_gemm_tn_bf16": [_p, _p, _p, _p, _i64, _i64, _i64, _i64, _i64, _i64, _i, _p, _i64, _p, _p],
    "rga3_gemm_tn_many": [_p, _p, _i, _p, _i64, _p],
    "rga3_gemm_swiglu_pre_bf16": [_p, _p, _p, _p, _p, _i64, _i64, _i64, _i64, _i64, _i64, _i64, _i, _p, _i64, _p],
    "rga3_gemm_cat_bf16": [_p, _p, _p, _p, _i64, _i64, _i64, _i64, _i64, _i64, _p, _p, _i64, _i64, _i64, _p, _p, _i64, _i64, _i64, _i, _p],
    "rga3_attn_varlen_fwd": [_p, _p, _p, _p, _p, _p, _p, _i, _i, _i64, _i, _i, _i, _i64, _i64, _i64, _i64, _i64, _i64,
                             _i64, _i64, _f, _i, _i, _p, _i64, _i, _i, _i, _p],
    "rga3_attn_varlen_fwd_rope": [_p, _p, _p, _p, _p, _p, _p, _i, _i, _i64, _i, _i, _i, _i64, _i64, _i64, _i64, _i64, _i64, _i64, _i64, _f, _i, _p, _p, _p, _p, _p],
    "rga3_rmsnorm_fwd": [_p, _p, _p, _p, _p, _i64, _i64, _i64, _f, _p],
    "rga3_layernorm_fwd": [_p, _p, _p, _p, _i64, _i64, _i64, _i64, _f, _i, _p],
    "rga3_layernorm_stats": [_p, _p, _i64, _i64, _i64, _f, _p],
    "rga3_gemm_ln_bf16": [_p, _p, _p, _p, _p, _p, _i64, _i64, _i64, _i64, _i64, _i64, _i, _i, _p],
    "rga3_gemm_lnsum_slices": [_i64, _i],
    "rga3_gemm_lnsum_bf16": [_p, _p, _p, _p, _p, _i64, _i64, _i64, _i64, _i64, _i64, _i64, _i, _p, _p],
    "rga3_gemm_lnq_bf16": [_p, _p, _p, _p, _p, _i64, _i64, _f, _p, _i64, _i64, _i64, _i64, _i64, _i64, _i, _i, _p],
    "rga3_rope_inplace": [_p, _p, _p, _i64, _i, _i, _i, _i64, _i64, _p],
    "rga3_gather_rows": [_p, _p, _p, _i64, _i64, _i64, _i64, _i64, _p],
    "rga3_scatter_rows": [_p, _p, _p, _i64, _i64, _i64, _i64, _i64, _p],
    "rga3_pad_cols": [_p, _p, _i64, _i64, _i64, _i64, _p],
    "rga3_silu_mul": [_p, _p, _p, _i64, _p],
    "rga3_add": [_p, _p, _p, _i64, _p],
    "rga3_cross_entropy_rows": [_p, _i, _p, _p, _p, _i64, _i64, _i64, _f, _p],
    "rga3_im2col": [_p, _p, _i64, _i, _i, _i, _i, _i, _i, _i64, _p],
    "rga3_maxpool2x2_win": [_p, _p, _i64, _i, _i, _i64, _i64, _p],
    "rga3_upsample2x_add": [_p, _p, _p, _i64, _i, _i, _i, _p],
    "rga3_add_bcast": [_p, _p, _p, _i64, _i64, _i, _i64, _i64, _i64, _f, _p],
    "rga3_bilinear": [_p, _i, _p, _p, _i64, _i, _i, _i, _i, _p],
    "rga3_conv3x3s2": [_p, _i, _p, _p, _p, _i64, _i, _i, _i, _i, _f, _f, _p],
    "rga3_decimg_rows": [_p, _i64, _p, _i64, _i, _p, _p, _i, _p, _p, _p, _p, _p, _p, _f, _p, _p, _p, _p, _p, _i64, _p, _p, _i64, _i, _f, _i64, _p],
    "rga3_attn_fewq": [_p, _i64, _p, _i64, _i64, _p, _p, _p, _i64, _i, _i, _i, _i, _f, _p],
    "rga3_copy_many": [_p, _p, _p, _i, _p],
    "rga3_conv3x3s2_ln_gelu": [_p, _i, _p, _p, _p, _p, _f, _p, _i64, _i, _i, _i, _i, _f, _f, _p],
    "rga3_dwconv7x7": [_p, _p, _p, _p, _i64, _i, _i, _i, _p],
    "rga3_rope_axial_inplace": [_p, _p, _p, _i64, _i, _i, _i64, _p],
    "rga3_pixel_shuffle2x": [_p, _p, _p, _p, _i64, _i, _i, _i, _i, _p],
    "rga3_bce_dice_sums": [_p, _p, _p, _i64, _i64, _p],
    "rga3_bce_dice_sums_ws_floats": [_i64, _i64],
    "rga3_bce_dice_sums_det": [_p, _p, _p, _p, _i64, _i64, _i64, _p],
    "rga3_mask_jf_ws_bytes": [_i64, _i64, _i64],
    "rga3_mask_jf_counts": [_p, _p, _p, _p, _p, _i64, _i64, _i64, _i64, _i, _p],
    "rga3_stom_ws_bytes": [_i64, _i64, _i64],
    "rga3_stom_flow": [_p, _p, _p, _i64, _i64, _i, _p],
    "rga3_stom_shift_composite": [_p, _p, _p, _p, _i64, _i64, _i64, _i, _p],
    "rga3_stom_mask_composite": [_p, _p, _p, _p, _p, _p, _i64, _i64, _i64, _i64, _i64, _i, _p, _i, _p, _i, _p],
    "rga3_attn_varlen_bwd": [_p, _p, _p, _p, _p, _p, _p, _p, _p, _p, _p, _p, _i, _i, _i, _i64, _i, _i, _i, _p, _f, _i, _p, _i64, _p],
    "rga3_transpose16_many": [_p, _p, _i, _p],
    "rga3_hiera_mlp144": [_p, _p, _p, _p, _p, _p, _p, _i64, _f, _p],
    "rga3_hiera_mlp288_pack_bytes": [],
    "rga3_hiera_mlp288_pack": [_p, _p, _p, _p, _p, _p],
    "rga3_hiera_mlp288": [_p, _p, _p, _p, _i64, _f, _p],
    "rga3_mlp3_rows": [_p, _p, _i, _i64, _p],
    "rga3_sam_select_objptr": [_p, _p, _p, _i64, _i, _p, _p, _p, _p, _p, _p, _p, _p, _p, _p, _i64, _p],
    "rga3_memattn_cross_ws_floats": [_i64, _i],
    "rga3_memattn_cross": [_p, _p, _p, _p, _i64, _i64, _i64, _i64, _i64, _i64, _f, _i, _p, _p],
    "rga3_memlayer_rows": [_p, _i64, _i, _p, _p, _i, _p, _p, _p, _i64, _p, _i64, _p, _p, _f, _p, _i64, _p, _p, _i, _p, _i64, _p, _p, _i, _i, _i64, _p],
    "rga3_gemm_rows16_many": [_p, _p, _i, _p],
    "rga3_gemm_stream_k_timeouts": [_p],
    "rga3_gemm_timeout_counter_offset": [],
    "rga3_gemm_ragged_plan": [_i64, _i64, _i64, _i, _i, _p, _p],
    "rga3_gemm_tiles": [_i, _p, _p, _p, _i],
    "rga3_gemm_candidates": [_i, _i64, _i64, _i64, _i, _i, _i, _p, _i],
    "rga3_gemm_tn_slices": [_i64, _i64, _i64],
    "rga3_quant_fp8_rows": [_p, _p, _p, _i64, _i64, _i64, _i64, _p],
    "rga3_gemm_fp8": [_p, _p, _p, _p, _p, _p, _p, _i64, _i64, _i64, _i64, _i64, _i64, _i64, _p],
    "rga3_swiglu_fwd_quant_fp8": [_p, _p, _p, _i64, _i64, _p],
    "rga3_swiglu_bwd_quant_fp8": [_p, _p, _p, _p, _i64, _i64, _p],
    "rga3_im2col3x3s2": [_p, _p, _i64, _i, _i, _i, _p],
    "rga3_pil_bicubic_coeffs": [_i, _i, _p, _p, _i64, _p],
    "rga3_sam_preprocess_u8": [_p, _i64, _i, _i, _i, _i, _p, _p, _i, _p, _p, _i, _p, _p, _p, _p, _p, _p],
    "rga3_qwen_norm_lut": [_p, _p, _i, _p],
    "rga3_qwen_patchify_u8": [_p, _i64, _i, _i, _p, _p, _i, _i, _i, _i, _p],
    "rga3_rmsnorm_bwd": [_p, _p, _p, _p, _p, _i64, _i64, _f, _p],
    "rga3_dropout_bf16": [_p, _p, _i64, _f, _i64, _i, _p],
    "rga3_dropout_pair_bf16": [_p, _p, _p, _p, _i64, _f, _i64, _f, _i64, _i, _p],
    "rga3_swiglu_fwd": [_p, _p, _i64, _i64, _p],
    "rga3_swiglu_bwd": [_p, _p, _p, _i64, _i64, _p],
    "rga3_transpose16": [_p, _p, _i64, _i64, _i64, _i64, _p],
    "rga3_segment_sum_rows": [_p, _p, _p, _p, _i64, _i64, _i64, _p],
    "rga3_adamw_step": [_p, _p, _p, _p, _p, _i64, _f, _f, _f, _f, _f, _i, _f, _p],
    "rga3_sumsq_accum": [_p, _p, _i64, _p],
    "rga3_sumsq_det": [_p, _i64, _p, _i64, _p, _i, _p],
    "rga3_adamw_step_clip": [_p, _p, _p, _p, _p, _i64, _f, _f, _f, _f, _f, _i, _p, _f, _p],
    "rga3_adamw_step_clip_rows": [_p, _p, _p, _p, _p, _i64, _i64, _p, _f, _f, _f, _f, _i, _p, _f, _p],
    "rga3_scatter_add_rows": [_p, _p, _p, _i64, _i64, _i64, _i64, _f, _p],
    "rga3_layernorm_bwd_ws_floats": [_i64, _i64],
    "rga3_layernorm_bwd": [_p, _p, _p, _p, _p, _p, _i64, _i64, _f, _p, _i64, _p],
    "rga3_colsum_accum": [_p, _p, _i64, _i64, _i64, _p],
    "rga3_colsum_ws_floats": [_i64, _i64],
    "rga3_colsum": [_p, _p, _i64, _i64, _i64, _p, _i64, _p, _p],
    "rga3_act": [_p, _p, _p, _i64, _i, _p],
    "rga3_bilinear_bwd": [_p, _p, _p, _i64, _i, _i, _i, _i, _p],
    "rga3_mask_product": [_p, _p, _p, _i64, _i64, _i64, _i64, _p],
    "rga3_mask_product_bwd_ws_floats": [_i64, _i64, _i64, _i64],
    "rga3_mask_product_bwd": [_p, _p, _p, _p, _p, _i64, _i64, _i64, _i64, _p, _i64, _p],
    "rga3_pixel_shuffle2x_bwd": [_p, _p, _i64, _i, _i, _i, _p],
    "rga3_bce_dice_grad": [_p, _p, _p, _p, _i64, _i64, _f, _f, _p],
    "rga3_bce_dice_grad_dev": [_p, _p, _p, _p, _i64, _i64, _p, _p, _p],
}

_INT64_RESULTS = ("rga3_gemm_lnsum_slices", "rga3_hiera_mlp288_pack_bytes", "rga3_gemm_workspace_bytes", "rga3_memattn_cross_ws_floats", "rga3_gemm_timeout_counter_offset", "rga3_layernorm_bwd_ws_floats", "rga3_colsum_ws_floats", "rga3_mask_product_bwd_ws_floats", "rga3_bce_dice_sums_ws_floats", "rga3_mask_jf_ws_bytes", "rga3_stom_ws_bytes")

_lib = None


class Rga3Error(RuntimeError):
    pass


def load():
    global _lib
    if _lib is not None:
        return _lib
    if not os.path.exists(LIB_PATH):
        raise Rga3Error(
            f"{LIB_PATH} not found: the HIP extension is required (no fallback path). "
            "Run `make -C rga3-release_amd/csrc` or `python -c 'import __graft_entry__ as g; g.build()'`.")
    import torch

    _thip = os.path.join(os.path.dirname(torch.__file__), "lib", "libamdhip64.so")
    if os.path.exists(_thip):
        C.CDLL(_thip, mode=C.RTLD_GLOBAL)
    lib = C.CDLL(LIB_PATH)
    for name, argtypes in SIGNATURES.items():
        fn = getattr(lib, name)
        fn.argtypes = argtypes
        fn.restype = C.c_int64 if name in _INT64_RESULTS else C.c_int
    _lib = lib
    return lib


def last_error() -> str:
    buf = C.create_string_buffer(512)
    load().rga3_last_error(buf, 512)
    return buf.value.decode("utf-8", "replace")


_TILE_ENTRIES = ("plain", "shared", "ln", "lnsum", "cat_k", "cat_n")
_tiles = {}


def gemm_tiles(entry: str) -> dict:
    if entry not in _tiles:
        ids, bm, bn = ((C.c_int * 64)() for _ in range(3))
        n = load().rga3_gemm_tiles(_TILE_ENTRIES.index(entry), ids, bm, bn, 64)
        if not 0 < n <= 64:
            raise Rga3Error("rga3_gemm_tiles failed: " + last_error())
        _tiles[entry] = {ids[i]: bn[i] for i in range(n)}
    return _tiles[entry]


def gemm_candidates(entry: str, M: int, N: int, K: int, act: int = 0, out_dtype: int = 0, bias=False, residual=False, colscale=False) -> tuple:
    ids = (C.c_int * 64)()
    n = load().rga3_gemm_candidates(_TILE_ENTRIES.index(entry), M, N, K, act, out_dtype, bool(bias) | bool(residual) << 1 | bool(colscale) << 2, ids, 64)
    if not 0 <= n <= 64:
        raise Rga3Error("rga3_gemm_candidates failed: " + last_error())
    return tuple(ids[:n])

# ... 12 lines not shown
```

rga3-release_amd/rga3/hip/ops.py:

```python
from __future__ import annotations

import math

import torch

from . import lib as _lib
from . import tuner as _tuner
from .derived import derived as _derived

BF16, F32 = 0, 1
ACT = {"none": 0, "gelu": 1, "swiglu": 2, "relu": 3}


def _stream():
    return torch.cuda.current_stream().cuda_stream


def _ptr(t):
    return 0 if t is None else t.data_ptr()


def _need_cuda(*ts):
    for t in ts:
        if t is not None and not t.is_cuda:
# ... 841 lines not shown
    seg, ann, vd = (None if t is None else t.contiguous() for t in (segmentation, annotation, void_pixels))
    out = torch.empty((T, 6), dtype=torch.int64, device=ann.device)
    ws = torch.empty(nws, dtype=torch.uint8, device=ann.device)
    _lib.check(L.rga3_mask_jf_counts(seg.data_ptr(), ann.data_ptr(), _ptr(vd), out.data_ptr(), ws.data_ptr(), nws, T, h, w, int(radius), _stream()), "mask_jf_counts")
    return out


STOM_MAX_POINTS = 16384
STOM_MAX_KERNEL = 128
_stom_ws = {}


def _stom_points(name, tracks, visibility, vip_frame_idx):
    _need_cuda(tracks, visibility)
    if tracks.dtype != torch.float32 or tracks.dim() != 3 or tracks.shape[2] != 2 or not tracks.is_contiguous():
        raise _lib.Rga3Error(f"{name}: tracks are contiguous float32 [T, N, 2], got {tracks.dtype} {tuple(tracks.shape)}")
    T, N = tracks.shape[:2]
    if visibility.dtype not in (torch.bool, torch.uint8) or tuple(visibility.shape) != (T, N) or not visibility.is_contiguous() or visibility.device != tracks.device:
        raise _lib.Rga3Error(f"{name}: visibility is contiguous bool [{T}, {N}] on {tracks.device}, got {visibility.dtype} {tuple(visibility.shape)} on {visibility.device}")
    if not 1 <= N <= STOM_MAX_POINTS:
        raise _lib.Rga3Error(f"{name}: {N} points per frame (1..{STOM_MAX_POINTS})")
    if not 0 <= vip_frame_idx < T:
        raise _lib.Rga3Error(f"{name}: vip_frame_idx {vip_frame_idx} outside [0, {T})")
    return T, N


def _stom_frames(name, frames, overlay):
    _need_cuda(frames, overlay)
    if frames.dtype != torch.uint8 or frames.dim() != 4 or frames.shape[3] != 3 or frames.shape[0] == 0 or not frames.is_contiguous():
        raise _lib.Rga3Error(f"{name}: frames are contiguous uint8 [T, H, W, 3], got {frames.dtype} {tuple(frames.shape)}")
    T, H, W, _ = frames.shape
    if overlay.dtype != torch.uint8 or tuple(overlay.shape) != (H, W, 4) or not overlay.is_contiguous() or overlay.device != frames.device:
        raise _lib.Rga3Error(f"{name}: the overlay is contiguous uint8 [{H}, {W}, 4] on {frames.device}, got {overlay.dtype} {tuple(overlay.shape)} on {overlay.device}")
    return T, H, W


def stom_flow(tracks, visibility, vip_frame_idx: int):
    T, N = _stom_points("stom_flow", tracks, visibility, vip_frame_idx)
    rec = torch.empty((T, 4), dtype=torch.int32, device=tracks.device)
    _lib.check(_lib.load().rga3_stom_flow(tracks.data_ptr(), visibility.data_ptr(), rec.data_ptr(), T, N, int(vip_frame_idx), _stream()), "stom_flow")
    return rec


def stom_shift_composite(frames, overlay, records, vip_frame_idx: int):
    T, H, W = _stom_frames("stom_shift_composite", frames, overlay)
    _need_cuda(records)
    if records.dtype != torch.int32 or tuple(records.shape) != (T, 4) or not records.is_contiguous() or records.device != frames.device:
        raise _lib.Rga3Error(f"stom_shift_composite: records are contiguous int32 [{T}, 4] on {frames.device}, got {records.dtype} {tuple(records.shape)}")
    if not 0 <= vip_frame_idx < T:
        raise _lib.Rga3Error(f"stom_shift_composite: vip_frame_idx {vip_frame_idx} outside [0, {T})")
    out = torch.empty_like(frames)
    _lib.check(_lib.load().rga3_stom_shift_composite(frames.data_ptr(), overlay.data_ptr(), records.data_ptr(), out.data_ptr(), T, H, W, int(vip_frame_idx), _stream()),
               "stom_shift_composite")
    return out


def stom_mask_composite(frames, overlay, tracks, visibility, vip_frame_idx: int, spans, ksize: int, half_widths, radius: int):
    import numpy as np

    T, H, W = _stom_frames("stom_mask_composite", frames, overlay)
    Tp, N = _stom_points("stom_mask_composite", tracks, visibility, vip_frame_idx)
    if Tp != T or tracks.device != frames.device:
        raise _lib.Rga3Error(f"stom_mask_composite: {Tp} frames of tracks on {tracks.device} for {T} frames on {frames.device}")
    if not 0 <= ksize <= STOM_MAX_KERNEL:
        raise _lib.Rga3Error(f"stom_mask_composite: structuring element of {ksize} (0..{STOM_MAX_KERNEL})")
    spans = np.ascontiguousarray(spans, dtype=np.uint8)
    half_widths = np.ascontiguousarray(half_widths, dtype=np.uint8)
    if spans.shape != (max(ksize, 1), 2) or radius < 0 or half_widths.shape != (radius + 1,):
        raise _lib.Rga3Error(f"stom_mask_composite: spans {spans.shape} / half widths {half_widths.shape} do not fit ksize {ksize} / radius {radius}")
    L = _lib.load()
    nws = int(L.rga3_stom_ws_bytes(T, H, W))
    if nws < 0:
        raise _lib.Rga3Error("stom_ws_bytes failed: " + _lib.last_error())
    key = _ws_key(frames.device)
    ws = _stom_ws.get(key)
    if ws is None or ws.numel() < nws:
        ws = _stom_ws[key] = torch.empty(nws, dtype=torch.uint8, device=frames.device)
    out = torch.empty_like(frames)
    _lib.check(L.rga3_stom_mask_composite(frames.data_ptr(), overlay.data_ptr(), tracks.data_ptr(), visibility.data_ptr(), out.data_ptr(), ws.data_ptr(), nws, T, H, W, N,
                                          int(vip_frame_idx), spans.ctypes.data, int(ksize), half_widths.ctypes.data, int(radius), _stream()), "stom_mask_composite")
    return out


def attn_varlen_bwd(q, k, v, o, dout, lse, cu_q, cu_k, max_q: int, max_k: int, scale: float, causal: bool, dq=None, dk=None, dv=None):
    import ctypes
    _need_cuda(q, k, v, o, dout, lse)
    Tq, Hq, D = q.shape
    Hkv = k.shape[1]
    dq = torch.empty_like(q) if dq is None else dq
    dk = torch.empty((k.shape[0], Hkv, D), dtype=torch.bfloat16, device=q.device) if dk is None else dk
    dv = torch.empty((k.shape[0], Hkv, D), dtype=torch.bfloat16, device=q.device) if dv is None else dv
    for t in (q, k, v, o, dout, dq, dk, dv):
        assert t.dtype == torch.bfloat16 and t.stride(2) == 1
    delta = torch.empty((Hq, Tq), dtype=torch.float32, device=q.device)
    Tk = k.shape[0]
    dkv_ws = torch.empty((2 * Hq * Tk * D,), dtype=torch.float32, device=q.device) if (Hq > Hkv and D % 4 == 0) else None
    st = (ctypes.c_int64 * 16)(q.stride(0), q.stride(1), k.stride(0), k.stride(1), v.stride(0), v.stride(1), o.stride(0), o.stride(1),
                               dout.stride(0), dout.stride(1), dq.stride(0), dq.stride(1), dk.stride(0), dk.stride(1), dv.stride(0), dv.stride(1))
    rc = _lib.load().rga3_attn_varlen_bwd(q.data_ptr(), k.data_ptr(), v.data_ptr(), o.data_ptr(), dout.data_ptr(), lse.data_ptr(), dq.data_ptr(),
                                          dk.data_ptr(), dv.data_ptr(), delta.data_ptr(), cu_q.data_ptr(), cu_k.data_ptr(), cu_q.numel() - 1, int(max_q),
                                          int(max_k), Tq, Hq, Hkv, D, ctypes.cast(st, ctypes.c_void_p), float(scale), int(bool(causal)), _ptr(dkv_ws), Tk, _stream())
    _lib.check(rc, "attn_varlen_bwd")
    return dq, dk, dv


def rmsnorm_bwd(x, weight, dy, eps: float, add=None):
    _need_cuda(x, weight, dy, add)
    assert x.is_contiguous() and dy.is_contiguous() and x.dtype == dy.dtype == torch.bfloat16 and (add is None or add.is_contiguous())
    dx = torch.empty_like(x)
    _lib.check(_lib.load().rga3_rmsnorm_bwd(x.data_ptr(), weight.data_ptr(), dy.data_ptr(), _ptr(add), dx.data_ptr(), x.shape[0], x.shape[1], float(eps),
                                            _stream()), "rmsnorm_bwd")
    return dx


def quant_fp8_rows(x):
    _need_cuda(x)
    assert x.dtype == torch.bfloat16 and x.dim() == 2 and x.stride(1) == 1 and x.shape[1] % 8 == 0
    rows, K = x.shape
    q = torch.empty((rows, K), dtype=torch.uint8, device=x.device)
    sc = torch.empty((rows,), dtype=torch.float32, device=x.device)
    _lib.check(_lib.load().rga3_quant_fp8_rows(x.data_ptr(), q.data_ptr(), sc.data_ptr(), rows, K, x.stride(0), q.stride(0), _stream()), "quant_fp8_rows")
    return q, sc


def gemm_fp8(aq, sa, wq, sw, bias=None, residual=None, out=None):
    _need_cuda(aq, wq, sa, sw, bias, residual)
    assert aq.dtype == torch.uint8 and wq.dtype == torch.uint8 and aq.stride(1) == 1 and wq.stride(1) == 1 and aq.shape[1] == wq.shape[1]
    M, K = aq.shape
    N = wq.shape[0]
    if out is None:
        out = torch.empty((M, N), dtype=torch.bfloat16, device=aq.device)
    assert out.dtype == torch.bfloat16 and out.stride(1) == 1 and sa.dtype == torch.float32 and sw.dtype == torch.float32
    _lib.check(_lib.load().rga3_gemm_fp8(aq.data_ptr(), wq.data_ptr(), sa.data_ptr(), sw.data_ptr(), _ptr(bias), _ptr(residual), out.data_ptr(), M, N, K,
                                         aq.stride(0), wq.stride(0), out.stride(0), residual.stride(0) if residual is not None else 0, _stream()), "gemm_fp8")
    return out


def swiglu_fwd_quant(gu):
    _need_cuda(gu)
    assert gu.dtype == torch.bfloat16 and gu.is_contiguous() and gu.shape[1] % 32 == 0
    T, I = gu.shape[0], gu.shape[1] // 2
    q = torch.empty((T, I), dtype=torch.uint8, device=gu.device)
    sc = torch.empty((T,), dtype=torch.float32, device=gu.device)
    _lib.check(_lib.load().rga3_swiglu_fwd_quant_fp8(gu.data_ptr(), q.data_ptr(), sc.data_ptr(), T, I, _stream()), "swiglu_fwd_quant_fp8")
    return q, sc


def swiglu_bwd_quant(gu, da):
    _need_cuda(gu, da)
    assert gu.dtype == da.dtype == torch.bfloat16 and gu.is_contiguous() and da.is_contiguous() and gu.shape[1] == 2 * da.shape[1]
    T, I = da.shape
    q = torch.empty((T, 2 * I), dtype=torch.uint8, device=gu.device)
    sc = torch.empty((T,), dtype=torch.float32, device=gu.device)
    _lib.check(_lib.load().rga3_swiglu_bwd_quant_fp8(gu.data_ptr(), da.data_ptr(), q.data_ptr(), sc.data_ptr(), T, I, _stream()), "swiglu_bwd_quant_fp8")
    return q, sc


def dropout(x, p: float, seed: int, out=None, accumulate: bool = False):
    _need_cuda(x, out)
    assert x.dtype == torch.bfloat16 and x.is_contiguous() and x.numel() % 8 == 0
    if out is None:
        assert not accumulate
        out = torch.empty_like(x)
    assert out.is_contiguous() and out.shape == x.shape and out.dtype == torch.bfloat16
    _lib.check(_lib.load().rga3_dropout_bf16(x.data_ptr(), out.data_ptr(), x.numel(), float(p), int(seed) & 0x7FFFFFFFFFFFFFFF, int(bool(accumulate)), _stream()),
               "dropout")
    return out


def dropout_pair(xa, pa: float, seed_a: int, xb, pb: float, seed_b: int, accumulate_into=None):
    _need_cuda(xa, xb, accumulate_into)
    assert xa.dtype == xb.dtype == torch.bfloat16 and xa.is_contiguous() and xb.is_contiguous() and xa.shape == xb.shape and xa.numel() % 8 == 0
    L = _lib.load()
    if accumulate_into is None:
        ya, yb = torch.empty_like(xa), torch.empty_like(xb)
        _lib.check(L.rga3_dropout_pair_bf16(xa.data_ptr(), xb.data_ptr(), ya.data_ptr(), yb.data_ptr(), xa.numel(), float(pa), int(seed_a), float(pb), int(seed_b), 0,
                                            _stream()), "dropout_pair_bf16")
        return ya, yb
    out = accumulate_into
    assert out.dtype == torch.bfloat16 and out.is_contiguous() and out.shape == xa.shape
    _lib.check(L.rga3_dropout_pair_bf16(xa.data_ptr(), xb.data_ptr(), out.data_ptr(), None, xa.numel(), float(pa), int(seed_a), float(pb), int(seed_b), 1, _stream()),
               "dropout_pair_bf16")
    return out


def swiglu_fwd(gu):
    _need_cuda(gu)
    assert gu.dtype == torch.bfloat16 and gu.is_contiguous() and gu.shape[1] % 32 == 0
    a = torch.empty((gu.shape[0], gu.shape[1] // 2), dtype=torch.bfloat16, device=gu.device)
    _lib.check(_lib.load().rga3_swiglu_fwd(gu.data_ptr(), a.data_ptr(), gu.shape[0], gu.shape[1] // 2, _stream()), "swiglu_fwd")
    return a


def swiglu_bwd(gu, da):
    _need_cuda(gu, da)
    assert gu.is_contiguous() and da.is_contiguous() and gu.shape[1] == 2 * da.shape[1]
    dgu = torch.empty_like(gu)
    _lib.check(_lib.load().rga3_swiglu_bwd(gu.data_ptr(), da.data_ptr(), dgu.data_ptr(), gu.shape[0], da.shape[1], _stream()), "swiglu_bwd")
    return dgu


def transpose(x):
    _need_cuda(x)
    assert x.dim() == 2 and x.stride(1) == 1 and x.element_size() == 2
    R, C = x.shape
    out = torch.empty((C, R), dtype=x.dtype, device=x.device)
    _lib.check(_lib.load().rga3_transpose16(x.data_ptr(), out.data_ptr(), R, C, x.stride(0), R, _stream()), "transpose16")
    return out


def transpose_many(mats):
    import ctypes
    outs = []
    for a in range(0, len(mats), 64):
        grp = mats[a:a + 64]
        n = len(grp)
        ptrs, dims = (ctypes.c_void_p * (2 * n))(), (ctypes.c_int64 * (2 * n))()
        for i, x in enumerate(grp):
            _need_cuda(x)
            assert x.dim() == 2 and x.is_contiguous() and x.element_size() == 2
            o = torch.empty((x.shape[1], x.shape[0]), dtype=x.dtype, device=x.device)
            ptrs[2 * i], ptrs[2 * i + 1] = x.data_ptr(), o.data_ptr()
            dims[2 * i], dims[2 * i + 1] = x.shape[0], x.shape[1]
            outs.append(o)
        _lib.check(_lib.load().rga3_transpose16_many(ctypes.cast(ptrs, ctypes.c_void_p), ctypes.cast(dims, ctypes.c_void_p), n, _stream()), "transpose16_many")
    return outs


def segment_sum_rows(x, rows, offsets):
    _need_cuda(x, rows, offsets)
    assert x.dtype == torch.bfloat16 and x.stride(1) == 1 and rows.dtype == torch.int64 and offsets.dtype == torch.int64
    n = offsets.numel() - 1
    out = torch.empty((n, x.shape[1]), dtype=torch.bfloat16, device=x.device)
    if n > 0:
        _lib.check(_lib.load().rga3_segment_sum_rows(x.data_ptr(), rows.data_ptr(), offsets.data_ptr(), out.data_ptr(), n, x.shape[1], x.stride(0), _stream()),
                   "segment_sum_rows")
    return out


def adamw_step_(param, master, grad, m, v, lr, beta1, beta2, eps, weight_decay, step: int, grad_scale: float = 1.0):
    _need_cuda(param, master, grad, m, v)
    assert param.dtype == grad.dtype == torch.bfloat16 and master.dtype == m.dtype == v.dtype == torch.float32
    assert param.is_contiguous() and grad.is_contiguous() and master.is_contiguous()
    _lib.check(_lib.load().rga3_adamw_step(param.data_ptr(), master.data_ptr(), grad.data_ptr(), m.data_ptr(), v.data_ptr(), param.numel(), float(lr),
                                           float(beta1), float(beta2), float(eps), float(weight_decay), int(step), float(grad_scale), _stream()), "adamw_step")


def sumsq_accum_(g, out):
    _need_cuda(g, out)
    assert g.dtype == torch.bfloat16 and g.is_contiguous() and out.dtype == torch.float32
    _lib.check(_lib.load().rga3_sumsq_accum(g.data_ptr(), out.data_ptr(), g.numel(), _stream()), "sumsq_accum")


def sumsq_det_(g, partials, out, accumulate: bool):
    _need_cuda(g, partials, out)
    assert g.dtype == torch.bfloat16 and g.is_contiguous() and out.dtype == partials.dtype == torch.float32
    _lib.check(_lib.load().rga3_sumsq_det(g.data_ptr(), g.numel(), partials.data_ptr(), partials.numel(), out.data_ptr(), int(bool(accumulate)), _stream()), "sumsq_det")


def adamw_step_clip_(param, master, grad, m, v, lr, beta1, beta2, eps, weight_decay, step: int, sumsq=None, max_norm: float = 0.0):
    _need_cuda(param, master, grad, m, v, sumsq)
    assert param.dtype == grad.dtype == torch.bfloat16 and master.dtype == m.dtype == v.dtype == torch.float32
    assert param.is_contiguous() and grad.is_contiguous() and master.is_contiguous()
    _lib.check(_lib.load().rga3_adamw_step_clip(param.data_ptr(), master.data_ptr(), grad.data_ptr(), m.data_ptr(), v.data_ptr(), param.numel(), float(lr),
                                                float(beta1), float(beta2), float(eps), float(weight_decay), int(step), _ptr(sumsq), float(max_norm), _stream()),
               "adamw_step_clip")
# ... 178 lines not shown
```

rga3-release_amd/rga3/model/qwen_train.py:

```python
from __future__ import annotations

import math
import os

import numpy as np
import torch
import torch.nn as nn

from ..hip import ops
from ..hip.derived import derived as _wt
from ..utils.staging import upload
from . import qwen2_5_vl as _Q
from .qwen2_5_vl import GatedMLP, Linear


class LoRALinear(Linear):

    def __init__(self, base: Linear, r: int, alpha: float, dropout: float = 0.0):
        super().__init__(base.in_features, base.out_features, bias=base.bias is not None, device=base.weight.device, dtype=base.weight.dtype)
        self.weight, self.bias = base.weight, base.bias
        self.weight.requires_grad_(False)
        if self.bias is not None:
            self.bias.requires_grad_(False)
        mk = lambda i, o: Linear(i, o, bias=False, device=base.weight.device, dtype=base.weight.dtype)
# ... 58 lines not shown

def _fgemm(x, owner, key, srcs, build, bias=None, residual=None, out=None):
    if _fp8["on"] and x.shape[1] % 128 == 0:
        q, sc = _fp8_pack(owner, key, *srcs, build=build)
        xq, xs = ops.quant_fp8_rows(x)
        if _fp8_tap[0] is not None:
            _fp8_tap[0](key, xq, xs)
        return ops.gemm_fp8(xq, xs, q, sc, bias=bias, residual=residual, out=out)
    w = _wt(owner, key, *srcs, build=build)
    return ops.gemm(x, w, bias, residual=residual, out=out)


def _fgemm_q(xq, xs, owner, key, srcs, build, bias=None, residual=None, out=None):
    q, sc = _fp8_pack(owner, key, *srcs, build=build)
    if _fp8_tap[0] is not None:
        _fp8_tap[0](key, xq, xs)
    return ops.gemm_fp8(xq, xs, q, sc, bias=bias, residual=residual, out=out)


def _fp8_fused(k: int) -> bool:
    return _fp8["on"] and k % 128 == 0


def vision_block_forward_fp8(blk, x, cu, max_len, cos, sin):
    at, mlp = blk.attn, blk.mlp
    N = x.shape[0]
    H, D = at.num_heads, at.head_dim
    h1 = blk.norm1(x)
    qkv = _fgemm(h1, at, "wqkv", (at.qkv.weight,), lambda: at.qkv.weight.detach(), bias=at.qkv.bias).view(N, 3 * H, D)
    if ops.attn_rope_win_ok(max_len, D):
        att = ops.attn_varlen_rope(qkv[:, :H], qkv[:, H:2 * H], qkv[:, 2 * H:], cu, cu, max_len, D ** -0.5, cos, sin, causal=False, rope_k=True)
    else:
        ops.rope_(qkv, cos, sin, 0, 2 * H)
        att = ops.attn_varlen(qkv[:, :H], qkv[:, H:2 * H], qkv[:, 2 * H:], cu, cu, max_len, D ** -0.5, causal=False, max_k=max_len)
    x1 = _fgemm(att.view(N, H * D), at, "wproj", (at.proj.weight,), lambda: at.proj.weight.detach(), bias=at.proj.bias, residual=x)
    h2 = blk.norm2(x1)
    wgu, bgu, wd = mlp._packed()
    gu = _fgemm(h2, mlp, "wgu", (mlp.gate_proj.weight, mlp.up_proj.weight), lambda: wgu, bias=bgu)
    return _down_from_gu(mlp, gu, wd, x1)


def _lora_parts(lin):
    if isinstance(lin, LoRALinear):
        return lin.lora_A["default"].weight, lin.lora_B["default"].weight, lin.scaling
    return None


_lora_cache = {}


def _lora_versions(lin):
    A, B = lin.lora_A["default"].weight, lin.lora_B["default"].weight
    return A._version, A.data_ptr(), B._version, B.data_ptr()


def _lora_build(mods):
    groups = {}
    for m in mods:
        A, B = m.lora_A["default"].weight, m.lora_B["default"].weight
        groups.setdefault((tuple(A.shape), tuple(B.shape), float(m.scaling), A.dtype, A.device), []).append(m)
    with torch.no_grad():
        for (_, _, sc, _, _), grp in groups.items():
            A = torch.stack([m.lora_A["default"].weight.detach() for m in grp])
            B = torch.stack([m.lora_B["default"].weight.detach() for m in grp])
            As = A * sc
            At = A.transpose(1, 2).contiguous()
            Bts = (B * sc).transpose(1, 2).contiguous()
            for i, m in enumerate(grp):
                _lora_cache[id(m)] = (_lora_versions(m), As[i], At[i], Bts[i])


def lora_refresh(layers):
    mods = [p for layer in layers for p in (layer.self_attn.q_proj, layer.self_attn.v_proj) if isinstance(p, LoRALinear)]
    if mods and any((e := _lora_cache.get(id(m))) is None or e[0] != _lora_versions(m) for m in (mods[0], mods[-1])):
        _lora_build(mods)
    ats = [layer.self_attn for layer in layers if _lora_cat_ok(layer.self_attn)]
    if ats and len({(a.num_heads, a.num_kv, a.head_dim, a.q_proj.lora_A["default"].weight.shape[0], float(a.q_proj.scaling), float(a.v_proj.scaling)) for a in ats}) == 1:
        if any((e := _lora_cat.get(id(a))) is None or e[0] != _lora_versions(a.q_proj) + _lora_versions(a.v_proj) for a in (ats[0], ats[-1])):
            _lora_cat_build(ats)


_LORA_FOLD = os.environ.get("RGA3_LORA_FOLD", "1") != "0"
_SWIGLU_PRE = os.environ.get("RGA3_SWIGLU_PRE", "1") != "0"
_lora_cat = {}
_lora_cat_store = {}


def set_lora_fold(on: bool):
    global _LORA_FOLD
    _LORA_FOLD = bool(on)


def _lora_cat_ok(at) -> bool:
    q, v = at.q_proj, at.v_proj
    if not (_LORA_FOLD and isinstance(q, LoRALinear) and isinstance(v, LoRALinear)) or isinstance(at.k_proj, LoRALinear):
        return False
    rq, rv = q.lora_A["default"].weight.shape[0], v.lora_A["default"].weight.shape[0]
    return rq == rv and (2 * rq) % 64 == 0 and q.lora_A["default"].weight.dtype == torch.bfloat16 and q.weight.shape[1] % 64 == 0


def _lora_cat_build(ats):
    with torch.no_grad():
        at0 = ats[0]
        Hq, Hk, D = at0.num_heads, at0.num_kv, at0.head_dim
        r = at0.q_proj.lora_A["default"].weight.shape[0]
        Nq, Nall = Hq * D, (Hq + 2 * Hk) * D
        Bq = torch.stack([a.q_proj.lora_B["default"].weight.detach() for a in ats])
        Bv = torch.stack([a.v_proj.lora_B["default"].weight.detach() for a in ats])
        ids = tuple(id(a) for a in ats)
        key = (ids, Nall, r, Bq.dtype, Bq.device)
        st = _lora_cat_store.get(key)
        if st is None:
            for k in [k for k in _lora_cat_store if k != key and not set(k[0]).isdisjoint(ids)]:
                del _lora_cat_store[k]
            st = (torch.zeros((len(ats), Nall, 2 * r), dtype=Bq.dtype, device=Bq.device), torch.zeros((len(ats), 2 * r, Nall), dtype=Bq.dtype, device=Bq.device))
            _lora_cat_store[key] = st
        W2, Wn = st
        W2[:, :Nq, :r] = Bq
        W2[:, Nq + Hk * D:, r:] = Bv
        Wn[:, :r, :Nq] = (Bq * float(at0.q_proj.scaling)).transpose(1, 2)
        Wn[:, r:, Nq + Hk * D:] = (Bv * float(at0.v_proj.scaling)).transpose(1, 2)
        for i, a in enumerate(ats):
            _lora_cat[id(a)] = (_lora_versions(a.q_proj) + _lora_versions(a.v_proj), W2[i], Wn[i])


def _lora_cat_ops(at):
    e = _lora_cat.get(id(at))
    if e is None or e[0] != _lora_versions(at.q_proj) + _lora_versions(at.v_proj):
        _lora_cat_build([at])
        e = _lora_cat[id(at)]
    return e[1], e[2]


def _lora_ops(lin):
    e = _lora_cache.get(id(lin))
    if e is None or e[0] != _lora_versions(lin):
        _lora_build([lin])
        e = _lora_cache[id(lin)]
    return e[1], e[2], e[3]


_drop_state = {"step": 0}


def next_dropout_seed(layer_idx: int, which: int, advance: bool = True) -> int:
    if advance:
        _drop_state["step"] += 1
    base = torch.initial_seed() & 0xFFFFFF
    return ((base << 39) ^ (_drop_state["step"] << 12) ^ (layer_idx << 2) ^ which) & 0x7FFFFFFFFFFFFFFF


def preview_dropout_seeds(n_layers: int):
    saved = _drop_state["step"]
    try:
        return [(next_dropout_seed(li, 0), next_dropout_seed(li, 1, advance=False)) for li in range(n_layers)]
    finally:
        _drop_state["step"] = saved


def _lora_dropout(at):
    pq = at.q_proj.dropout_p if isinstance(at.q_proj, LoRALinear) and at.q_proj.training else 0.0
    pv = at.v_proj.dropout_p if isinstance(at.v_proj, LoRALinear) and at.v_proj.training else 0.0
    return pq, pv


def _drop_pair(h1, pq, pv, seeds):
    if pq > 0.0 and pv > 0.0 and h1.is_contiguous():
        return ops.dropout_pair(h1, pq, seeds[0], h1, pv, seeds[1])
    return (ops.dropout(h1, pq, seeds[0]) if pq > 0.0 else h1), (ops.dropout(h1, pv, seeds[1]) if pv > 0.0 else h1)


def qkv_with_lora(at, h1, seeds=None, want_inputs=False):
    Hq, Hk, D = at.num_heads, at.num_kv, at.head_dim
    wqkv, bqkv = at._packed()
    lq, lv = _lora_parts(at.q_proj), _lora_parts(at.v_proj)
    pq, pv = _lora_dropout(at)
    if seeds is None and (pq > 0.0 or pv > 0.0):
        lid = getattr(at, "layer_idx", 0) or 0
        seeds = (next_dropout_seed(lid, 0), next_dropout_seed(lid, 1, advance=False))
    if not _fp8["on"] and h1.shape[0] > 16 and _lora_cat_ok(at):
        r = lq[0].shape[0]
        hq, hv = _drop_pair(h1, pq, pv, seeds)
        tt = torch.empty((h1.shape[0], 2 * r), dtype=h1.dtype, device=h1.device)
        tq = ops.gemm(hq, _lora_ops(at.q_proj)[0], out=tt[:, :r])
        tv = ops.gemm(hv, _lora_ops(at.v_proj)[0], out=tt[:, r:])
        qkv2 = ops.gemm_cat(h1, wqkv, bqkv, a2=tt, w2=_lora_cat_ops(at)[0])
        return (qkv2, tq, tv, hq, hv) if want_inputs else (qkv2, tq, tv)
    if _fp8["on"] and h1.shape[1] % 128 == 0:
        qkv2 = _fgemm(h1, at, "wqkv", (at.q_proj.weight, at.k_proj.weight, at.v_proj.weight), lambda: wqkv, bias=bqkv)
    else:
        qkv2 = ops.gemm(h1, wqkv, bqkv)
    tq = tv = None
    hq = hv = h1
    if lq is not None and lv is not None and pq > 0.0 and pv > 0.0:
        hq, hv = _drop_pair(h1, pq, pv, seeds)
        pq = pv = 0.0
    if lq is not None:
        if pq > 0.0:
            hq = ops.dropout(h1, pq, seeds[0])
        tq = ops.gemm(hq, _lora_ops(at.q_proj)[0])
        oq = qkv2[:, : Hq * D]
        ops.gemm(tq, lq[1].detach(), residual=oq, out=oq)
    if lv is not None:
        if pv > 0.0:
            hv = ops.dropout(h1, pv, seeds[1])
        tv = ops.gemm(hv, _lora_ops(at.v_proj)[0])
        ov = qkv2[:, (Hq + Hk) * D:]
        ops.gemm(tv, lv[1].detach(), residual=ov, out=ov)
    return (qkv2, tq, tv, hq, hv) if want_inputs else (qkv2, tq, tv)


def _layer_forward_fp8(layer, x, cos, sin, cu, max_len, seeds):
    at, mlp = layer.self_attn, layer.mlp
    Hq, Hk, D = at.num_heads, at.num_kv, at.head_dim
    T = x.shape[0]
    w1, w2 = layer.input_layernorm, layer.post_attention_layernorm
    h1 = ops.rmsnorm(x, w1.weight, w1.variance_epsilon)
    qkv2 = qkv_with_lora(at, h1, seeds=seeds)[0]
    qkv = qkv2.view(T, Hq + 2 * Hk, D)
    ops.rope_(qkv, cos, sin, 0, Hq + Hk)
    att = ops.attn_varlen(qkv[:, :Hq], qkv[:, Hq:Hq + Hk], qkv[:, Hq + Hk:], cu, cu, max_len, D ** -0.5, causal=True)
    x1 = _fgemm(att.view(T, Hq * D), at, "wo", (at.o_proj.weight,), lambda: at.o_proj.weight.detach(), residual=x)
    h2 = ops.rmsnorm(x1, w2.weight, w2.variance_epsilon)
    wgu, bgu, wd = mlp._packed()
    gu = _fgemm(h2, mlp, "wgu", (mlp.gate_proj.weight, mlp.up_proj.weight), lambda: wgu, bias=bgu)
    return _down_from_gu(mlp, gu, wd, x1)


def _down_from_gu(mlp, gu, wd, x1):
    if _fp8_fused(gu.shape[1] // 2):
        aq, asc = ops.swiglu_fwd_quant(gu)
        return _fgemm_q(aq, asc, mlp, "wd", (mlp.down_proj.weight,), lambda: wd, bias=mlp.down_proj.bias, residual=x1)
    return _fgemm(ops.swiglu_fwd(gu), mlp, "wd", (mlp.down_proj.weight,), lambda: wd, bias=mlp.down_proj.bias, residual=x1)


_acts = {"store": True}


def set_activation_recompute(on: bool):
    _acts["store"] = not on


def _layer_forward_store(layer, x, cos, sin, cu, max_len, seeds):
    at, mlp = layer.self_attn, layer.mlp
    Hq, Hk, D = at.num_heads, at.num_kv, at.head_dim
    T = x.shape[0]
    w1, w2 = layer.input_layernorm, layer.post_attention_layernorm
    h1 = ops.rmsnorm(x, w1.weight, w1.variance_epsilon)
    qkv2, tq, tv, hq_in, hv_in = qkv_with_lora(at, h1, seeds=seeds, want_inputs=True)
    qkv = qkv2.view(T, Hq + 2 * Hk, D)
    ops.rope_(qkv, cos, sin, 0, Hq + Hk)
    att, lse = ops.attn_varlen(qkv[:, :Hq], qkv[:, Hq:Hq + Hk], qkv[:, Hq + Hk:], cu, cu, max_len, D ** -0.5, causal=True, return_lse=True)
    x1 = _fgemm(att.view(T, Hq * D), at, "wo", (at.o_proj.weight,), lambda: at.o_proj.weight.detach(), residual=x)
    h2 = ops.rmsnorm(x1, w2.weight, w2.variance_epsilon)
    wgu, bgu, wd = mlp._packed()
    if not _fp8["on"] and _SWIGLU_PRE and T > 4:
        a_, gu = ops.gemm_swiglu_pre(h2, wgu, bgu)
        y = _fgemm(a_, mlp, "wd", (mlp.down_proj.weight,), lambda: wd, bias=mlp.down_proj.bias, residual=x1)
    else:
        gu = _fgemm(h2, mlp, "wgu", (mlp.gate_proj.weight, mlp.up_proj.weight), lambda: wgu, bias=bgu)
        y = _down_from_gu(mlp, gu, wd, x1)
    return y, (h1, qkv, att, lse, x1, h2, gu, tq, tv, hq_in, hv_in)


def _neg_table(sin):
    return _wt(None, "neg_sin", sin, build=lambda: (-sin).contiguous())


class DecoderLayerFn(torch.autograd.Function):

    @staticmethod
    def forward(ctx, x, aq, bq, av, bv, layer, cos, sin, cu, max_len, seeds):
        at0 = layer.self_attn
        ctx.stored = False
        if _acts["store"]:
            with torch.no_grad():
                y, saved = _layer_forward_store(layer, x, cos, sin, cu, max_len, seeds)
            ctx.stored = True
            ctx.seeds = seeds
            ctx.layer, ctx.cos, ctx.sin, ctx.cu, ctx.max_len = layer, cos, sin, cu, max_len
            ctx.save_for_backward(x, *saved)
            return y
        if _fp8["on"]:
            with torch.no_grad():
                y = _layer_forward_fp8(layer, x, cos, sin, cu, max_len, seeds)
        else:
            at0._lora_drop_seeds = seeds
            try:
                with torch.no_grad():
                    y = layer(x, cos, sin, cu, max_len, None)
            finally:
                at0._lora_drop_seeds = None
        ctx.seeds = seeds
        ctx.layer, ctx.cos, ctx.sin, ctx.cu, ctx.max_len = layer, cos, sin, cu, max_len
        ctx.save_for_backward(x)
        return y

    @staticmethod
    def backward(ctx, dy):
        x = ctx.saved_tensors[0]
        layer, cos, sin, cu, max_len = ctx.layer, ctx.cos, ctx.sin, ctx.cu, ctx.max_len
        at, mlp = layer.self_attn, layer.mlp
        Hq, Hk, D = at.num_heads, at.num_kv, at.head_dim
        T = x.shape[0]
        dy = dy.contiguous()
        with torch.no_grad():
            w1, w2 = layer.input_layernorm, layer.post_attention_layernorm
            wqkv, bqkv = at._packed()
            lq, lv = _lora_parts(at.q_proj), _lora_parts(at.v_proj)
            pq, pv = _lora_dropout(at)
            wgu, bgu, wd = mlp._packed()
            if ctx.stored:
                h1, qkv, att, lse, x1, h2, gu, tq, tv, hq_in, hv_in = ctx.saved_tensors[1:]
            else:
                h1 = ops.rmsnorm(x, w1.weight, w1.variance_epsilon)
                qkv2, tq, tv, hq_in, hv_in = qkv_with_lora(at, h1, seeds=ctx.seeds, want_inputs=True)
                qkv = qkv2.view(T, Hq + 2 * Hk, D)
                ops.rope_(qkv, cos, sin, 0, Hq + Hk)
                att, lse = ops.attn_varlen(qkv[:, :Hq], qkv[:, Hq:Hq + Hk], qkv[:, Hq + Hk:], cu, cu, max_len, D ** -0.5, causal=True, return_lse=True)
                x1 = _fgemm(att.view(T, Hq * D), at, "wo", (at.o_proj.weight,), lambda: at.o_proj.weight.detach(), residual=x)
                h2 = ops.rmsnorm(x1, w2.weight, w2.variance_epsilon)
                gu = _fgemm(h2, mlp, "wgu", (mlp.gate_proj.weight, mlp.up_proj.weight), lambda: wgu, bias=bgu)
            q, k, v = qkv[:, :Hq], qkv[:, Hq:Hq + Hk], qkv[:, Hq + Hk:]
            da = _fgemm(dy, mlp, "wd_t", (mlp.down_proj.weight,), lambda: ops.transpose(wd))
            if _fp8_fused(gu.shape[1]):
                dq, dsc = ops.swiglu_bwd_quant(gu, da)
                del gu, da
                dh2 = _fgemm_q(dq, dsc, mlp, "wgu_t", (mlp.gate_proj.weight, mlp.up_proj.weight), lambda: ops.transpose(wgu))
                del dq
            else:
                dgu = ops.swiglu_bwd(gu, da)
                del gu, da
                dh2 = _fgemm(dgu, mlp, "wgu_t", (mlp.gate_proj.weight, mlp.up_proj.weight), lambda: ops.transpose(wgu))
                del dgu
            dx1 = ops.rmsnorm_bwd(x1, w2.weight, dh2, w2.variance_epsilon, add=dy)
            datt = _fgemm(dx1, at, "wo_t", (at.o_proj.weight,), lambda: ops.transpose(at.o_proj.weight.detach())).view(T, Hq, D)
            dqkv = torch.empty_like(qkv)
            ops.attn_varlen_bwd(q, k, v, att, datt, lse, cu, cu, max_len, max_len, D ** -0.5, True, dq=dqkv[:, :Hq], dk=dqkv[:, Hq:Hq + Hk],
                                dv=dqkv[:, Hq + Hk:])
            ops.rope_(dqkv, cos, _neg_table(sin), 0, Hq + Hk)
            dqkv2 = dqkv.view(T, (Hq + 2 * Hk) * D)
            fold = (not _fp8["on"]) and T > 16 and _lora_cat_ok(at)
            dtt = None
            if fold:
                wqkv_t = _wt(at, "wqkv_t", at.q_proj.weight, at.k_proj.weight, at.v_proj.weight, build=lambda: ops.transpose(wqkv))
                dh1, dtt = ops.gemm_cat(dqkv2, wqkv_t, wn=_lora_cat_ops(at)[1])
            else:
                dh1 = _fgemm(dqkv2, at, "wqkv_t", (at.q_proj.weight, at.k_proj.weight, at.v_proj.weight), lambda: ops.transpose(wqkv))
            grads = [None, None, None, None]
            if lq is not None or lv is not None:
                tn_pairs, tn_slots = [], []
                pend = []
                for slot, lp, lin, t_, cols, pdrop, hin, sd in ((0, lq, at.q_proj, tq, (0, Hq * D), pq, hq_in, 0),
                                                                (2, lv, at.v_proj, tv, ((Hq + Hk) * D, (Hq + 2 * Hk) * D), pv, hv_in, 1)):
                    if lp is None:
                        continue
                    _, At, Bts = _lora_ops(lin)
                    dsl = dqkv2[:, cols[0]:cols[1]]
                    if dtt is not None:
                        rr = dtt.shape[1] // 2
                        dt = dtt[:, :rr] if slot == 0 else dtt[:, rr:]
                    else:
                        dt = ops.gemm(dsl, Bts)
                    tn_pairs += [(dt, h1 if pdrop == 0.0 else hin), (dsl, t_)]
                    tn_slots += [slot, slot + 1]
                    if pdrop == 0.0:
                        ops.gemm(dt, At, residual=dh1, out=dh1)
                    else:
                        pend.append((ops.gemm(dt, At), pdrop, ctx.seeds[sd]))
                if len(pend) == 2 and dh1.is_contiguous():
                    ops.dropout_pair(pend[0][0], pend[0][1], pend[0][2], pend[1][0], pend[1][1], pend[1][2], accumulate_into=dh1)
                else:
                    for xg, pg, sg in pend:
                        ops.dropout(xg, pg, sg, out=dh1, accumulate=True)
                for sl, gw in zip(tn_slots, ops.gemm_tn_many(tn_pairs)):
                    grads[sl] = gw
            dx = ops.rmsnorm_bwd(x, w1.weight, dh1, w1.variance_epsilon, add=dx1)
        return (dx, grads[0], grads[1], grads[2], grads[3], None, None, None, None, None, None)


class EmbedFn(torch.autograd.Function):

    @staticmethod
    def forward(ctx, weight, ids_dev, ids_np, grad_rows_np, plan=None):
        from ..parallel.ddp import sparse_sink_for

        ctx.shape = weight.shape
        ctx.sink = sparse_sink_for(weight)
        ctx.weight = weight
        plan = plan if plan is not None else {}
        if "embed_bwd" not in plan:
            rows = grad_rows_np
            ids = ids_np[rows]
            order = np.argsort(ids, kind="stable")
            uniq, counts = np.unique(ids[order], return_counts=True)
            off = np.concatenate([[0], np.cumsum(counts)]).astype(np.int64)
            dev = weight.device
            plan["embed_bwd"] = (upload(rows[order].astype(np.int64), dev), upload(off, dev), upload(uniq.astype(np.int64), dev),
                                 uniq.astype(np.int64))
        ctx.csr = plan["embed_bwd"]
        if ctx.sink is not None:
            ctx.sink.announce_sparse(weight, ctx.csr[3])
        return ops.gather_rows(weight, ids_dev)

    @staticmethod
    def backward(ctx, dx):
        rows_dev, off_dev, uniq_dev, _ = ctx.csr
        seg = ops.segment_sum_rows(dx.contiguous(), rows_dev, off_dev)
        if ctx.sink is not None:
            ctx.sink.add_sparse(ctx.weight, uniq_dev, seg)
            return None, None, None, None, None
        dW = torch.zeros(ctx.shape, dtype=dx.dtype, device=dx.device)
        ops.scatter_rows_(dW, uniq_dev, seg)
        return dW, None, None, None, None


class NormHeadCEFn(torch.autograd.Function):

    @staticmethod
    def forward(ctx, h, lm_w, norm_w, eps, valid_rows_dev, targets_dev, n_valid):
        hn = ops.rmsnorm(h, norm_w, eps)
        if n_valid == 0:
            ctx.n = 0
            ctx.save_for_backward(h, norm_w)
            ctx.eps = eps
            return torch.zeros((), device=h.device, dtype=torch.float32), hn
        hv = ops.gather_rows(hn, valid_rows_dev)
        logits = ops.gemm(hv, lm_w)
        row_loss, dlogits = ops.cross_entropy_rows(logits, targets_dev, want_grad=True, grad_scale=1.0 / n_valid)
        ctx.save_for_backward(h, lm_w, norm_w, hv, dlogits, valid_rows_dev)
        ctx.eps, ctx.n = eps, n_valid
        return row_loss.sum() / n_valid, hn

    @staticmethod
    def backward(ctx, gloss, ghn):
        if ctx.n == 0:
            h, norm_w = ctx.saved_tensors
            with torch.no_grad():
                dh = ops.rmsnorm_bwd(h, norm_w, ghn.contiguous() if ghn is not None else torch.zeros_like(h), ctx.eps)
            return dh, None, None, None, None, None, None
        h, lm_w, norm_w, hv, dlogits, rows = ctx.saved_tensors
        n = ctx.n
        with torch.no_grad():
            dlogits = (dlogits.float() * gloss).to(dlogits.dtype)
            dW = None
            if lm_w.requires_grad:
                from ..parallel.ddp import dense_grad_out_for
                dW = ops.gemm_tn(dlogits, hv, out=dense_grad_out_for(lm_w))
            n8 = (n + 7) // 8 * 8
            dl = dlogits
            if n8 != n:
                dl = torch.zeros((n8, dlogits.shape[1]), dtype=dlogits.dtype, device=dlogits.device)
                dl[:n] = dlogits
            dhv = ops.gemm_tn(ops.transpose(dl), lm_w.detach())[:n].contiguous()
            dhn = ghn.contiguous().clone() if ghn is not None else torch.zeros_like(h)
            dhn_rows = ops.add(ops.gather_rows(dhn, rows), dhv)
            ops.scatter_rows_(dhn, rows, dhn_rows)
            dh = ops.rmsnorm_bwd(h, norm_w, dhn, ctx.eps)
        return dh, dW, None, None, None, None, None

# ... 25 lines not shown
```

Measured before the change: 7.599.

## Fuse RoPE into attention backward, rmsnorm with LoRA dropout fwd and bwd

```diff
diff --git a/include/rga3_hip.h b/include/rga3_hip.h
--- a/include/rga3_hip.h
+++ b/include/rga3_hip.h
@@ -120,6 +120,11 @@
                          void* dk, void* dv, float* delta_ws, const int32_t* cu_q, const int32_t* cu_k, int nseg, int max_q,
                          int max_k, int64_t total_q, int Hq, int Hkv, int D, const int64_t* strides16, float scale, int causal,
                          float* dkv_ws, int64_t total_k, void* stream);
+int rga3_attn_varlen_bwd_rope(const void* q, const void* k, const void* v, const void* o, const void* dout, const float* lse, void* dq,
+                              void* dk, void* dv, float* delta_ws, const int32_t* cu_q, const int32_t* cu_k, int nseg, int max_q,
+                              int max_k, int64_t total_q, int Hq, int Hkv, int D, const int64_t* strides16, float scale, int causal,
+                              float* dkv_ws, int64_t total_k, const float* cos_q, const float* sin_q, const float* cos_k, const float* sin_k,
+                              void* stream);
 int rga3_hiera_mlp144(const void* x, const void* w1f, const float* c1, const void* d1, const void* w2, const void* b2, void* y, int64_t M, float eps, void* stream);
 int64_t rga3_hiera_mlp288_pack_bytes(void);
 int rga3_hiera_mlp288_pack(const void* w1f, const float* c1, const void* d1, const void* w2, void* pack, void* stream);
@@ -145,6 +150,10 @@
                      void* stream);
 int rga3_dropout_bf16(const void* x, void* y, int64_t n, float p, int64_t seed, int accumulate, void* stream);
 int rga3_dropout_pair_bf16(const void* xa, const void* xb, void* ya, void* yb, int64_t n, float pa, int64_t seed_a, float pb, int64_t seed_b, int sum, void* stream);
+int rga3_rmsnorm_drop_pair_fwd(const void* x, const void* weight, void* y, void* ya, void* yb, int64_t rows, int64_t dim, int64_t ldx, int64_t ldy, int64_t ld_ya,
+                               int64_t ld_yb, float eps, float pa, int64_t seed_a, float pb, int64_t seed_b, void* stream);
+int rga3_rmsnorm_bwd_lora(const void* x, const void* weight, const void* dy, const void* add, void* dx, const void* pq, const void* pv, int64_t rows, int64_t dim,
+                          int64_t ld_pq, int64_t ld_pv, float eps, float pa, int64_t seed_a, float pb, int64_t seed_b, void* stream);
 int rga3_swiglu_fwd(const void* gu, void* a, int64_t T, int64_t I, void* stream);
 int rga3_swiglu_bwd(const void* gu, const void* da, void* dgu, int64_t T, int64_t I, void* stream);
 int rga3_transpose16(const void* in, void* out, int64_t R, int64_t C, int64_t ld_in, int64_t ld_out, void* stream);
diff --git a/rga3-release_amd/csrc/attn_bwd.hip b/rga3-release_amd/csrc/attn_bwd.hip
--- a/rga3-release_amd/csrc/attn_bwd.hip
+++ b/rga3-release_amd/csrc/attn_bwd.hip
@@ -16,12 +16,26 @@
     float* dkv_ws;
     long total_k;
     int gx, gy;
+    const float *cos_q, *sin_q, *cos_k, *sin_k;
 };
 
+__device__ __forceinline__ void store_rotated(unsigned short* row, int dd, const f32x4& lo, const f32x4& hi, const float* cs, const float* sn) {
+    const f32x4 c1 = *(const f32x4*)(cs + dd), s1 = *(const f32x4*)(sn + dd), c2 = *(const f32x4*)(cs + dd + 64), s2 = *(const f32x4*)(sn + dd + 64);
+    float o1[4], o2[4];
+#pragma unroll
+    for (int e = 0; e < 4; ++e) rope_rotate(bf16_round(lo[e]), bf16_round(hi[e]), c1[e], s1[e], c2[e], s2[e], o1[e], o2[e]);
+    u32x2 a, b;
+    a[0] = pack_bf2(o1[0], o1[1]); a[1] = pack_bf2(o1[2], o1[3]);
+    b[0] = pack_bf2(o2[0], o2[1]); b[1] = pack_bf2(o2[2], o2[3]);
+    *(u32x2*)(row + dd) = a;
+    *(u32x2*)(row + dd + 64) = b;
+}
+
 constexpr int BT = 64;
 
-template <int DP, int QT, int NWAVE, bool PAIR>
+template <int DP, int QT, int NWAVE, bool PAIR, bool ROPE = false>
 __global__ __launch_bounds__(64 * NWAVE) void attn_bwd_dq_kernel(AttnBwdArgs p) {
+    static_assert(!ROPE || DP == 128, "the rotated stores are written for D = 128");
     constexpr int NT = 64 * NWAVE;
     constexpr int BLOCK_M = NWAVE * QT * 16;
     constexpr int CH = DP / 8;
@@ -202,6 +216,12 @@
         const int qi = qw0 + t * 16 + c;
         if (qi < Lq) {
             unsigned short* row = p.dq + (long)(qs + qi) * p.dq_st + (long)hq * p.dq_sh;
+            if constexpr (ROPE) {
+#pragma unroll
+                for (int d = 0; d < DT / 2; ++d)
+                    store_rotated(row, d * 16 + 4 * g, dqacc[t][d], dqacc[t][d + DT / 2], p.cos_q + (long)(qs + qi) * DP, p.sin_q + (long)(qs + qi) * DP);
+                continue;
+            }
 #pragma unroll
             for (int d = 0; d < DT; ++d) {
                 const int dd = d * 16 + 4 * g;
@@ -217,8 +237,9 @@
     }
 }
 
-template <int DP, int NWAVE, bool SPLIT, bool PAIR>
+template <int DP, int NWAVE, bool SPLIT, bool PAIR, bool ROPE = false>
 __global__ __launch_bounds__(64 * NWAVE) void attn_bwd_dkv_kernel(AttnBwdArgs p) {
+    static_assert(!ROPE || (DP == 128 && !SPLIT), "the rotated stores are written for D = 128; the split path rotates in attn_dkv_reduce_kernel");
     constexpr int NT = 64 * NWAVE;
     constexpr int BLOCK_N = NWAVE * 16;
     constexpr int CH = DP / 8;
@@ -401,17 +422,23 @@
                 u32x2 a, b;
                 a[0] = pack_bf2(dkacc[d][0], dkacc[d][1]); a[1] = pack_bf2(dkacc[d][2], dkacc[d][3]);
                 b[0] = pack_bf2(dvacc[d][0], dvacc[d][1]); b[1] = pack_bf2(dvacc[d][2], dvacc[d][3]);
-                *(u32x2*)(rk + dd) = a;
+                if constexpr (!ROPE) *(u32x2*)(rk + dd) = a;
                 *(u32x2*)(rv + dd) = b;
             }
         }
-    }
-    }
-}
-
+        if constexpr (ROPE) {
+#pragma unroll
+            for (int d = 0; d < DT / 2; ++d)
+                store_rotated(rk, d * 16 + 4 * g, dkacc[d], dkacc[d + DT / 2], p.cos_k + (long)(ks + key) * DP, p.sin_k + (long)(ks + key) * DP);
+        }
+    }
+    }
+}
+
+template <bool ROPE = false>
 __global__ __launch_bounds__(256) void attn_dkv_reduce_kernel(AttnBwdArgs p) {
     const int group = p.Hq / p.Hkv;
-    const int d4 = p.D / 4;
+    const int d4 = ROPE ? p.D / 8 : p.D / 4;
     const long idx = (long)blockIdx.x * 256 + threadIdx.x;
     const long total = p.total_k * p.Hkv * d4;
     if (idx >= total) return;
@@ -429,8 +456,18 @@
     u32x2 a, b;
     a[0] = pack_bf2(sk[0], sk[1]); a[1] = pack_bf2(sk[2], sk[3]);
     b[0] = pack_bf2(sv[0], sv[1]); b[1] = pack_bf2(sv[2], sv[3]);
-    *(u32x2*)(p.dk + key * p.dk_st + (long)hk * p.dk_sh + dd) = a;
+    if constexpr (!ROPE) *(u32x2*)(p.dk + key * p.dk_st + (long)hk * p.dk_sh + dd) = a;
     *(u32x2*)(p.dv + key * p.dv_st + (long)hk * p.dv_sh + dd) = b;
+    if constexpr (ROPE) {
+        f32x4 sk2 = *(const f32x4*)(w + 64), sv2 = *(const f32x4*)(w + half + 64);
+        for (int h = 1; h < group; ++h) {
+            sk2 += *(const f32x4*)(w + h * plane + 64);
+            sv2 += *(const f32x4*)(w + half + h * plane + 64);
+        }
+        b[0] = pack_bf2(sv2[0], sv2[1]); b[1] = pack_bf2(sv2[2], sv2[3]);
+        *(u32x2*)(p.dv + key * p.dv_st + (long)hk * p.dv_sh + dd + 64) = b;
+        store_rotated(p.dk + key * p.dk_st + (long)hk * p.dk_sh, dd, sk, sk2, p.cos_k + key * 128, p.sin_k + key * 128);
+    }
 }
 
 template <auto K>
@@ -439,7 +476,7 @@
     return launch_lds<K>(dim3(gx * (unsigned)gy * (unsigned)nseg), dim3(64 * nwave), lds, st, name, a);
 }
 
-template <int DP>
+template <int DP, bool ROPE = false>
 static int launch_bwd(const AttnBwdArgs& a0, int nseg, int max_q, int max_k, hipStream_t st) {
     AttnBwdArgs a = a0;
     a.gx = 1; a.gy = 1;
@@ -455,30 +492,29 @@
     const unsigned nqb = (unsigned)cdiv(max_q, BLOCK_M), nkb = (unsigned)cdiv(max_k, 16 * NW);
     const bool pair = a.causal && nqb >= 4 && nkb >= 4;
     const unsigned gq = pair ? (nqb + 1) / 2 : nqb, gk = pair ? (nkb + 1) / 2 : nkb;
-    if (int rc = pair ? launch_bwd_grid<attn_bwd_dq_kernel<DP, QT, NWQ, true>>(a, LDS_DQ, gq, a.Hq, nseg, NWQ, st, "attn_bwd_dq_kernel")
-                      : launch_bwd_grid<attn_bwd_dq_kernel<DP, QT, NWQ, false>>(a, LDS_DQ, gq, a.Hq, nseg, NWQ, st, "attn_bwd_dq_kernel"))
+    if (int rc = pair ? launch_bwd_grid<attn_bwd_dq_kernel<DP, QT, NWQ, true, ROPE>>(a, LDS_DQ, gq, a.Hq, nseg, NWQ, st, "attn_bwd_dq_kernel")
+                      : launch_bwd_grid<attn_bwd_dq_kernel<DP, QT, NWQ, false, ROPE>>(a, LDS_DQ, gq, a.Hq, nseg, NWQ, st, "attn_bwd_dq_kernel"))
         return rc;
     if (a.dkv_ws && a.Hq > a.Hkv) {
         if (int rc = pair ? launch_bwd_grid<attn_bwd_dkv_kernel<DP, NW, true, true>>(a, LDS_DKV, gk, a.Hq, nseg, NW, st, "attn_bwd_dkv_kernel<split>")
                           : launch_bwd_grid<attn_bwd_dkv_kernel<DP, NW, true, false>>(a, LDS_DKV, gk, a.Hq, nseg, NW, st, "attn_bwd_dkv_kernel<split>"))
             return rc;
         const long rows = a.total_k * a.Hkv;
-        hipLaunchKernelGGL(attn_dkv_reduce_kernel, dim3((unsigned)cdiv(rows * (a.D / 4), 256)), dim3(256), 0, st, a);
+        hipLaunchKernelGGL(attn_dkv_reduce_kernel<ROPE>, dim3((unsigned)cdiv(rows * (a.D / (ROPE ? 8 : 4)), 256)), dim3(256), 0, st, a);
         RGA3_CHECK_LAUNCH("attn_dkv_reduce_kernel");
         return 0;
     }
-    return pair ? launch_bwd_grid<attn_bwd_dkv_kernel<DP, NW, false, true>>(a, LDS_DKV, gk, a.Hkv, nseg, NW, st, "attn_bwd_dkv_kernel")
-                : launch_bwd_grid<attn_bwd_dkv_kernel<DP, NW, false, false>>(a, LDS_DKV, gk, a.Hkv, nseg, NW, st, "attn_bwd_dkv_kernel");
+    return pair ? launch_bwd_grid<attn_bwd_dkv_kernel<DP, NW, false, true, ROPE>>(a, LDS_DKV, gk, a.Hkv, nseg, NW, st, "attn_bwd_dkv_kernel")
+                : launch_bwd_grid<attn_bwd_dkv_kernel<DP, NW, false, false, ROPE>>(a, LDS_DKV, gk, a.Hkv, nseg, NW, st, "attn_bwd_dkv_kernel");
 }
 
 }
 
 using namespace rga3;
 
-extern "C" int rga3_attn_varlen_bwd(const void* q, const void* k, const void* v, const void* o, const void* dout, const float* lse,
-                                    void* dq, void* dk, void* dv, float* delta_ws, const int32_t* cu_q, const int32_t* cu_k, int nseg,
-                                    int max_q, int max_k, int64_t total_q, int Hq, int Hkv, int D, const int64_t* strides16, float scale,
-                                    int causal, float* dkv_ws, int64_t total_k, void* stream) {
+static int attn_varlen_bwd_impl(const void* q, const void* k, const void* v, const void* o, const void* dout, const float* lse, void* dq, void* dk, void* dv,
+                                float* delta_ws, const int32_t* cu_q, const int32_t* cu_k, int nseg, int max_q, int max_k, int64_t total_q, int Hq, int Hkv, int D,
+                                const int64_t* strides16, float scale, int causal, float* dkv_ws, int64_t total_k, const float* const rope[4], void* stream) {
     RGA3_CHECK_ARG(q && k && v && o && dout && lse && dq && dk && dv && delta_ws && cu_q && cu_k && strides16, "attn_bwd: null pointer");
     RGA3_CHECK_ARG(nseg > 0 && max_q > 0 && max_k > 0 && total_q > 0, "attn_bwd: sizes");
     RGA3_CHECK_ARG(Hq > 0 && Hkv > 0 && Hq % Hkv == 0, "attn_bwd: Hq=%d Hkv=%d", Hq, Hkv);
@@ -501,10 +537,35 @@
     a.dk_st = strides16[12]; a.dk_sh = strides16[13]; a.dv_st = strides16[14]; a.dv_sh = strides16[15];
     a.Hq = Hq; a.Hkv = Hkv; a.D = D; a.total_q = total_q; a.scale = scale; a.scale_log2 = scale * 1.4426950408889634f; a.causal = causal;
     a.dkv_ws = dkv_ws; a.total_k = total_k;
+    a.cos_q = rope[0]; a.sin_q = rope[1]; a.cos_k = rope[2]; a.sin_k = rope[3];
     RGA3_CHECK_ARG(!dkv_ws || (total_k > 0 && D % 4 == 0), "attn_bwd: dkv_ws needs total_k");
     hipStream_t st = (hipStream_t)stream;
+    if (rope[0]) return launch_bwd<128, true>(a, nseg, max_q, max_k, st);
     if (D <= 32) return launch_bwd<32>(a, nseg, max_q, max_k, st);
     if (D <= 64) return launch_bwd<64>(a, nseg, max_q, max_k, st);
     if (D <= 96) return launch_bwd<96>(a, nseg, max_q, max_k, st);
     return launch_bwd<128>(a, nseg, max_q, max_k, st);
 }
+
+extern "C" int rga3_attn_varlen_bwd(const void* q, const void* k, const void* v, const void* o, const void* dout, const float* lse,
+                                    void* dq, void* dk, void* dv, float* delta_ws, const int32_t* cu_q, const int32_t* cu_k, int nseg,
+                                    int max_q, int max_k, int64_t total_q, int Hq, int Hkv, int D, const int64_t* strides16, float scale,
+                                    int causal, float* dkv_ws, int64_t total_k, void* stream) {
+    static const float* const none[4] = {nullptr, nullptr, nullptr, nullptr};
+    return attn_varlen_bwd_impl(q, k, v, o, dout, lse, dq, dk, dv, delta_ws, cu_q, cu_k, nseg, max_q, max_k, total_q, Hq, Hkv, D, strides16, scale, causal, dkv_ws,
+                                total_k, none, stream);
+}
+
+extern "C" int rga3_attn_varlen_bwd_rope(const void* q, const void* k, const void* v, const void* o, const void* dout, const float* lse,
+                                         void* dq, void* dk, void* dv, float* delta_ws, const int32_t* cu_q, const int32_t* cu_k, int nseg,
+                                         int max_q, int max_k, int64_t total_q, int Hq, int Hkv, int D, const int64_t* strides16, float scale,
+                                         int causal, float* dkv_ws, int64_t total_k, const float* cos_q, const float* sin_q, const float* cos_k,
+                                         const float* sin_k, void* stream) {
+    RGA3_CHECK_ARG(D == 128, "attn_bwd_rope: head dim %d: the rotated stores are written for 128 only", D);
+    RGA3_CHECK_ARG(cos_q && sin_q && cos_k && sin_k, "attn_bwd_rope: null table");
+    RGA3_CHECK_ARG((((uintptr_t)cos_q | (uintptr_t)sin_q | (uintptr_t)cos_k | (uintptr_t)sin_k) & 15) == 0, "attn_bwd_rope: cos / sin tables must be 16-byte aligned");
+    RGA3_CHECK_ARG(total_k > 0, "attn_bwd_rope: total_k=%ld (rows of the key tables)", (long)total_k);
+    const float* const rope[4] = {cos_q, sin_q, cos_k, sin_k};
+    return attn_varlen_bwd_impl(q, k, v, o, dout, lse, dq, dk, dv, delta_ws, cu_q, cu_k, nseg, max_q, max_k, total_q, Hq, Hkv, D, strides16, scale, causal, dkv_ws,
+                                total_k, rope, stream);
+}
diff --git a/rga3-release_amd/csrc/common.h b/rga3-release_amd/csrc/common.h
--- a/rga3-release_amd/csrc/common.h
+++ b/rga3-release_amd/csrc/common.h
@@ -94,6 +94,36 @@
     dg = d * u * sg * (1.f + g * (1.f - sg));
 }
 
+__device__ __forceinline__ unsigned dropout_hash(unsigned long long seed, unsigned long long ctr) {
+    unsigned x = (unsigned)ctr ^ (unsigned)seed, y = (unsigned)(ctr >> 32) ^ (unsigned)(seed >> 32);
+    x *= 0xcc9e2d51u; x = (x << 15) | (x >> 17); x *= 0x1b873593u;
+    y ^= x; y = (y << 13) | (y >> 19); y = y * 5u + 0xe6546b64u;
+    y ^= y >> 16; y *= 0x85ebca6bu; y ^= y >> 13; y *= 0xc2b2ae35u; y ^= y >> 16;
+    return y;
+}
+struct DropPair {
+    unsigned thr_a, thr_b;
+    float ik_a, ik_b;
+    unsigned long long seed_a, seed_b;
+};
+static inline DropPair drop_pair_of(float pa, int64_t seed_a, float pb, int64_t seed_b) {
+    const unsigned ta = (unsigned)(pa * 65536.0f + 0.5f), tb = (unsigned)(pb * 65536.0f + 0.5f);
+    return DropPair{ta, tb, 1.0f / (1.0f - (float)ta / 65536.0f), 1.0f / (1.0f - (float)tb / 65536.0f), (unsigned long long)seed_a, (unsigned long long)seed_b};
+}
+__device__ __forceinline__ void drop_pair_word(const DropPair& m, unsigned long long g, int j, unsigned wa, unsigned wb, float& alo, float& ahi, float& blo,
+                                               float& bhi) {
+    const unsigned ha = dropout_hash(m.seed_a, g * 4 + j), hb = dropout_hash(m.seed_b, g * 4 + j);
+    alo = ((ha & 0xffffu) >= m.thr_a) ? __uint_as_float(wa << 16) * m.ik_a : 0.f;
+    ahi = ((ha >> 16) >= m.thr_a) ? __uint_as_float(wa & 0xffff0000u) * m.ik_a : 0.f;
+    blo = ((hb & 0xffffu) >= m.thr_b) ? __uint_as_float(wb << 16) * m.ik_b : 0.f;
+    bhi = ((hb >> 16) >= m.thr_b) ? __uint_as_float(wb & 0xffff0000u) * m.ik_b : 0.f;
+}
+
+__device__ __forceinline__ void rope_rotate(float a, float b, float c1, float s1, float c2, float s2, float& o1, float& o2) {
+    o1 = __builtin_fmaf(a, c1, -(b * s1));
+    o2 = __builtin_fmaf(b, c2, a * s2);
+}
+
 static inline int64_t cdiv(int64_t a, int64_t b) { return (a + b - 1) / b; }
 
 static inline unsigned grid1d(long total, int per_block = 256, long cap = 256L * 32) {
diff --git a/rga3-release_amd/csrc/rowops.hip b/rga3-release_amd/csrc/rowops.hip
--- a/rga3-release_amd/csrc/rowops.hip
+++ b/rga3-release_amd/csrc/rowops.hip
@@ -60,10 +60,12 @@
     }
 }
 
-template <int MAXC>
+template <int MAXC, bool DROP = false>
 __global__ __launch_bounds__(256) void rmsnorm_block_kernel(const unsigned short* __restrict__ x, const unsigned short* __restrict__ add,
                                                             const unsigned short* __restrict__ w, unsigned short* __restrict__ y,
-                                                            unsigned short* __restrict__ res_out, long rows, int dim, long ldx, float eps) {
+                                                            unsigned short* __restrict__ res_out, long rows, int dim, long ldx, float eps,
+                                                            unsigned short* __restrict__ ya = nullptr, unsigned short* __restrict__ yb = nullptr,
+                                                            DropPair m = DropPair{}) {
     __shared__ float part[4];
     const int tid = threadIdx.x;
     const long row = blockIdx.x;
@@ -106,7 +108,21 @@
             unpack8(wv[i], fw);
 #pragma unroll
             for (int e = 0; e < 8; ++e) f[e] = fw[e] * bf2f(f2bf(f[e] * rinv));
-            *(u32x4*)(y + row * ldx + ch * 8) = pack8(f);
+            const u32x4 o = pack8(f);
+            *(u32x4*)(y + row * ldx + ch * 8) = o;
+            if constexpr (DROP) {
+                const long g = row * nch + ch;
+                u32x4 oa, ob;
+#pragma unroll
+                for (int j = 0; j < 4; ++j) {
+                    float alo, ahi, blo, bhi;
+                    drop_pair_word(m, (unsigned long long)g, j, o[j], o[j], alo, ahi, blo, bhi);
+                    oa[j] = pack_bf2(alo, ahi);
+                    ob[j] = pack_bf2(blo, bhi);
+                }
+                *(u32x4*)(ya + g * 8) = oa;
+                *(u32x4*)(yb + g * 8) = ob;
+            }
         }
     }
 }
@@ -318,10 +334,7 @@
         unpack8(va[h], a);
         unpack8(vb[h], b);
 #pragma unroll
-        for (int e = 0; e < 8; ++e) {
-            o1[e] = a[e] * c1[e] - b[e] * s1[e];
-            o2[e] = b[e] * c2[e] + a[e] * s2[e];
-        }
+        for (int e = 0; e < 8; ++e) rope_rotate(a[e], b[e], c1[e], s1[e], c2[e], s2[e], o1[e], o2[e]);
         *(u32x4*)(p1 + h * sh) = pack8(o1);
         *(u32x4*)(p1 + h * sh + half) = pack8(o2);
     }
@@ -497,6 +510,28 @@
     return 0;
 }
 
+extern "C" int rga3_rmsnorm_drop_pair_fwd(const void* x, const void* weight, void* y, void* ya, void* yb, int64_t rows, int64_t dim, int64_t ldx, int64_t ldy,
+                                          int64_t ld_ya, int64_t ld_yb, float eps, float pa, int64_t seed_a, float pb, int64_t seed_b, void* stream) {
+    RGA3_CHECK_ARG(x && weight && y && ya && yb, "rmsnorm_drop_pair: null pointer");
+    RGA3_CHECK_ARG(rows > 0 && dim >= 2048 && dim % 8 == 0 && dim <= 8192, "rmsnorm_drop_pair: rows=%ld / dim=%ld outside [2048, 8192] or no multiple of 8",
+                   (long)rows, (long)dim);
+    RGA3_CHECK_ARG(ldx == dim && ldy == dim && ld_ya == dim && ld_yb == dim, "rmsnorm_drop_pair: ldx=%ld ldy=%ld ld_ya=%ld ld_yb=%ld: all must be contiguous [rows, %ld]",
+                   (long)ldx, (long)ldy, (long)ld_ya, (long)ld_yb, (long)dim);
+    RGA3_CHECK_ARG(pa >= 0.f && pa < 1.f && pb >= 0.f && pb < 1.f, "rmsnorm_drop_pair: p=%f / %f", pa, pb);
+    RGA3_CHECK_ARG((((uintptr_t)x | (uintptr_t)weight | (uintptr_t)y | (uintptr_t)ya | (uintptr_t)yb) & 15) == 0, "rmsnorm_drop_pair: pointers must be 16-byte aligned");
+    const DropPair m = drop_pair_of(pa, seed_a, pb, seed_b);
+    hipStream_t st = (hipStream_t)stream;
+    dim3 g2((unsigned)rows);
+    if (cdiv(dim / 8, 256) <= 2)
+        hipLaunchKernelGGL((rmsnorm_block_kernel<2, true>), g2, dim3(256), 0, st, (cus)x, (cus) nullptr, (cus)weight, (us)y, (us) nullptr, (long)rows, (int)dim, (long)ldx,
+                           eps, (us)ya, (us)yb, m);
+    else
+        hipLaunchKernelGGL((rmsnorm_block_kernel<4, true>), g2, dim3(256), 0, st, (cus)x, (cus) nullptr, (cus)weight, (us)y, (us) nullptr, (long)rows, (int)dim, (long)ldx,
+                           eps, (us)ya, (us)yb, m);
+    RGA3_CHECK_LAUNCH("rmsnorm_block_kernel (drop pair)");
+    return 0;
+}
+
 extern "C" int rga3_layernorm_fwd(const void* x, const void* weight, const void* bias, void* y, int64_t rows, int64_t dim,
                                   int64_t ldx, int64_t ldy, float eps, int act, void* stream) {
     RGA3_CHECK_ARG(x && weight && y, "layernorm: null pointer");
diff --git a/rga3-release_amd/csrc/trainops.hip b/rga3-release_amd/csrc/trainops.hip
--- a/rga3-release_amd/csrc/trainops.hip
+++ b/rga3-release_amd/csrc/trainops.hip
@@ -49,10 +49,12 @@
     }
 }
 
-template <int NC>
+template <int NC, bool LORA = false>
 __global__ __launch_bounds__(256) void rmsnorm_bwd_block_kernel(const unsigned short* __restrict__ x, const unsigned short* __restrict__ w,
                                                                 const unsigned short* __restrict__ dy, const unsigned short* __restrict__ add,
-                                                                unsigned short* __restrict__ dx, int dim, float eps) {
+                                                                unsigned short* __restrict__ dx, int dim, float eps,
+                                                                const unsigned short* __restrict__ pq = nullptr, const unsigned short* __restrict__ pv = nullptr,
+                                                                DropPair m = DropPair{}) {
     __shared__ float red[2][4];
     const int lane = threadIdx.x & 63, wv = threadIdx.x >> 6;
     const long row = blockIdx.x;
@@ -65,7 +67,18 @@
         if (ch < nch) {
             float fw[8];
             unpack8(*(const u32x4*)(x + row * dim + ch * 8), fx[i]);
-            unpack8(*(const u32x4*)(dy + row * dim + ch * 8), fg[i]);
+            u32x4 dv = *(const u32x4*)(dy + row * dim + ch * 8);
+            if constexpr (LORA) {
+                const u32x4 va = *(const u32x4*)(pq + row * dim + ch * 8), vb = *(const u32x4*)(pv + row * dim + ch * 8);
+                const unsigned long long g = (unsigned long long)(row * nch + ch);
+#pragma unroll
+                for (int j = 0; j < 4; ++j) {
+                    float alo, ahi, blo, bhi;
+                    drop_pair_word(m, g, j, va[j], vb[j], alo, ahi, blo, bhi);
+                    dv[j] = pack_bf2(__uint_as_float(dv[j] << 16) + alo + blo, __uint_as_float(dv[j] & 0xffff0000u) + ahi + bhi);
+                }
+            }
+            unpack8(dv, fg[i]);
             unpack8(*(const u32x4*)(w + ch * 8), fw);
 #pragma unroll
             for (int e = 0; e < 8; ++e) {
@@ -303,14 +316,6 @@
     }
 }
 
-__device__ __forceinline__ unsigned dropout_hash(unsigned long long seed, unsigned long long ctr) {
-    unsigned x = (unsigned)ctr ^ (unsigned)seed, y = (unsigned)(ctr >> 32) ^ (unsigned)(seed >> 32);
-    x *= 0xcc9e2d51u; x = (x << 15) | (x >> 17); x *= 0x1b873593u;
-    y ^= x; y = (y << 13) | (y >> 19); y = y * 5u + 0xe6546b64u;
-    y ^= y >> 16; y *= 0x85ebca6bu; y ^= y >> 13; y *= 0xc2b2ae35u; y ^= y >> 16;
-    return y;
-}
-
 __global__ __launch_bounds__(256) void dropout_kernel(const unsigned short* __restrict__ x, unsigned short* __restrict__ y, long n8, unsigned thr,
                                                       float inv_keep, unsigned long long seed, int accumulate) {
     for (long g = (long)blockIdx.x * 256 + threadIdx.x; g < n8; g += (long)gridDim.x * 256) {
@@ -333,6 +338,7 @@
                                                            unsigned short* yb, long n8, unsigned thr_a, float ik_a, unsigned long long seed_a, unsigned thr_b,
                                                            float ik_b, unsigned long long seed_b, int sum) {
     const bool same = xa == xb;
+    const DropPair m{thr_a, thr_b, ik_a, ik_b, seed_a, seed_b};
     for (long g = (long)blockIdx.x * 256 + threadIdx.x; g < n8; g += (long)gridDim.x * 256) {
         const u32x4 va = *(const u32x4*)(xa + g * 8);
         const u32x4 vb = same ? va : *(const u32x4*)(xb + g * 8);
@@ -341,11 +347,8 @@
         u32x4 oa, ob;
 #pragma unroll
         for (int j = 0; j < 4; ++j) {
-            const unsigned ha = dropout_hash(seed_a, (unsigned long long)g * 4 + j), hb = dropout_hash(seed_b, (unsigned long long)g * 4 + j);
-            const float alo = ((ha & 0xffffu) >= thr_a) ? __uint_as_float(va[j] << 16) * ik_a : 0.f;
-            const float ahi = ((ha >> 16) >= thr_a) ? __uint_as_float(va[j] & 0xffff0000u) * ik_a : 0.f;
-            const float blo = ((hb & 0xffffu) >= thr_b) ? __uint_as_float(vb[j] << 16) * ik_b : 0.f;
-            const float bhi = ((hb >> 16) >= thr_b) ? __uint_as_float(vb[j] & 0xffff0000u) * ik_b : 0.f;
+            float alo, ahi, blo, bhi;
+            drop_pair_word(m, (unsigned long long)g, j, va[j], vb[j], alo, ahi, blo, bhi);
             if (sum) {
                 oa[j] = pack_bf2(__uint_as_float(o[j] << 16) + alo + blo, __uint_as_float(o[j] & 0xffff0000u) + ahi + bhi);
             } else {
@@ -382,6 +385,25 @@
     return 0;
 }
 
+extern "C" int rga3_rmsnorm_bwd_lora(const void* x, const void* weight, const void* dy, const void* add, void* dx, const void* pq, const void* pv, int64_t rows,
+                                     int64_t dim, int64_t ld_pq, int64_t ld_pv, float eps, float pa, int64_t seed_a, float pb, int64_t seed_b, void* stream) {
+    RGA3_CHECK_ARG(x && weight && dy && dx && pq && pv && rows > 0 && dim > 1024 && dim % 8 == 0 && dim <= 8192,
+                   "rmsnorm_bwd_lora: null pointer / rows=%ld / dim=%ld outside (1024, 8192] or no multiple of 8", (long)rows, (long)dim);
+    RGA3_CHECK_ARG(ld_pq == dim && ld_pv == dim, "rmsnorm_bwd_lora: ld_pq=%ld ld_pv=%ld: the LoRA gradients must be contiguous [rows, %ld]", (long)ld_pq, (long)ld_pv,
+                   (long)dim);
+    RGA3_CHECK_ARG(pa >= 0.f && pa < 1.f && pb >= 0.f && pb < 1.f, "rmsnorm_bwd_lora: p=%f / %f", pa, pb);
+    RGA3_CHECK_ARG((((uintptr_t)x | (uintptr_t)weight | (uintptr_t)dy | (uintptr_t)add | (uintptr_t)dx | (uintptr_t)pq | (uintptr_t)pv) & 15) == 0,
+                   "rmsnorm_bwd_lora: pointers must be 16-byte aligned");
+    const DropPair m = drop_pair_of(pa, seed_a, pb, seed_b);
+    hipStream_t st = (hipStream_t)stream;
+    dim3 gb((unsigned)rows);
+    if (dim <= 2048) hipLaunchKernelGGL((rmsnorm_bwd_block_kernel<1, true>), gb, dim3(256), 0, st, (cus)x, (cus)weight, (cus)dy, (cus)add, (us)dx, (int)dim, eps, (cus)pq, (cus)pv, m);
+    else if (dim <= 4096) hipLaunchKernelGGL((rmsnorm_bwd_block_kernel<2, true>), gb, dim3(256), 0, st, (cus)x, (cus)weight, (cus)dy, (cus)add, (us)dx, (int)dim, eps, (cus)pq, (cus)pv, m);
+    else hipLaunchKernelGGL((rmsnorm_bwd_block_kernel<4, true>), gb, dim3(256), 0, st, (cus)x, (cus)weight, (cus)dy, (cus)add, (us)dx, (int)dim, eps, (cus)pq, (cus)pv, m);
+    RGA3_CHECK_LAUNCH("rmsnorm_bwd_block (lora)");
+    return 0;
+}
+
 extern "C" int rga3_dropout_bf16(const void* x, void* y, int64_t n, float p, int64_t seed, int accumulate, void* stream) {
     RGA3_CHECK_ARG(x && y && n > 0 && n % 8 == 0, "dropout: n=%ld must be a positive multiple of 8", (long)n);
     RGA3_CHECK_ARG(p >= 0.f && p < 1.f, "dropout: p=%f", p);
@@ -400,11 +422,11 @@
     RGA3_CHECK_ARG(xa && xb && ya && (sum || yb) && n > 0 && n % 8 == 0, "dropout_pair: null pointer / n=%ld must be a positive multiple of 8", (long)n);
     RGA3_CHECK_ARG(pa >= 0.f && pa < 1.f && pb >= 0.f && pb < 1.f, "dropout_pair: p=%f / %f", pa, pb);
     RGA3_CHECK_ARG((((uintptr_t)xa | (uintptr_t)xb | (uintptr_t)ya | (uintptr_t)yb) & 15) == 0, "dropout_pair: pointers must be 16-byte aligned");
-    const unsigned ta = (unsigned)(pa * 65536.0f + 0.5f), tb = (unsigned)(pb * 65536.0f + 0.5f);
+    const DropPair m = drop_pair_of(pa, seed_a, pb, seed_b);
     long blocks = cdiv(n / 8, 256);
     if (blocks > 65536) blocks = 65536;
-    hipLaunchKernelGGL(dropout_pair_kernel, dim3((unsigned)blocks), dim3(256), 0, (hipStream_t)stream, (cus)xa, (cus)xb, (us)ya, (us)yb, (long)(n / 8), ta,
-                       1.0f / (1.0f - (float)ta / 65536.0f), (unsigned long long)seed_a, tb, 1.0f / (1.0f - (float)tb / 65536.0f), (unsigned long long)seed_b, sum);
+    hipLaunchKernelGGL(dropout_pair_kernel, dim3((unsigned)blocks), dim3(256), 0, (hipStream_t)stream, (cus)xa, (cus)xb, (us)ya, (us)yb, (long)(n / 8), m.thr_a,
+                       m.ik_a, m.seed_a, m.thr_b, m.ik_b, m.seed_b, sum);
     RGA3_CHECK_LAUNCH("dropout_pair_kernel");
     return 0;
 }
diff --git a/rga3-release_amd/rga3/hip/lib.py b/rga3-release_amd/rga3/hip/lib.py
--- a/rga3-release_amd/rga3/hip/lib.py
+++ b/rga3-release_amd/rga3/hip/lib.py
@@ -58,6 +58,7 @@
     "rga3_stom_shift_composite": [_p, _p, _p, _p, _i64, _i64, _i64, _i, _p],
     "rga3_stom_mask_composite": [_p, _p, _p, _p, _p, _p, _i64, _i64, _i64, _i64, _i64, _i, _p, _i, _p, _i, _p],
     "rga3_attn_varlen_bwd": [_p, _p, _p, _p, _p, _p, _p, _p, _p, _p, _p, _p, _i, _i, _i, _i64, _i, _i, _i, _p, _f, _i, _p, _i64, _p],
+    "rga3_attn_varlen_bwd_rope": [_p, _p, _p, _p, _p, _p, _p, _p, _p, _p, _p, _p, _i, _i, _i, _i64, _i, _i, _i, _p, _f, _i, _p, _i64, _p, _p, _p, _p, _p],
     "rga3_transpose16_many": [_p, _p, _i, _p],
     "rga3_hiera_mlp144": [_p, _p, _p, _p, _p, _p, _p, _i64, _f, _p],
     "rga3_hiera_mlp288_pack_bytes": [],
@@ -87,6 +88,8 @@
     "rga3_rmsnorm_bwd": [_p, _p, _p, _p, _p, _i64, _i64, _f, _p],
     "rga3_dropout_bf16": [_p, _p, _i64, _f, _i64, _i, _p],
     "rga3_dropout_pair_bf16": [_p, _p, _p, _p, _i64, _f, _i64, _f, _i64, _i, _p],
+    "rga3_rmsnorm_drop_pair_fwd": [_p, _p, _p, _p, _p, _i64, _i64, _i64, _i64, _i64, _i64, _f, _f, _i64, _f, _i64, _p],
+    "rga3_rmsnorm_bwd_lora": [_p, _p, _p, _p, _p, _p, _p, _i64, _i64, _i64, _i64, _f, _f, _i64, _f, _i64, _p],
     "rga3_swiglu_fwd": [_p, _p, _i64, _i64, _p],
     "rga3_swiglu_bwd": [_p, _p, _p, _i64, _i64, _p],
     "rga3_transpose16": [_p, _p, _i64, _i64, _i64, _i64, _p],
diff --git a/rga3-release_amd/rga3/hip/ops.py b/rga3-release_amd/rga3/hip/ops.py
--- a/rga3-release_amd/rga3/hip/ops.py
+++ b/rga3-release_amd/rga3/hip/ops.py
@@ -947,7 +947,7 @@
     return out
 
 
-def attn_varlen_bwd(q, k, v, o, dout, lse, cu_q, cu_k, max_q: int, max_k: int, scale: float, causal: bool, dq=None, dk=None, dv=None):
+def attn_varlen_bwd(q, k, v, o, dout, lse, cu_q, cu_k, max_q: int, max_k: int, scale: float, causal: bool, dq=None, dk=None, dv=None, rope=None, split_ws=True):
     import ctypes
     _need_cuda(q, k, v, o, dout, lse)
     Tq, Hq, D = q.shape
@@ -959,9 +959,20 @@
         assert t.dtype == torch.bfloat16 and t.stride(2) == 1
     delta = torch.empty((Hq, Tq), dtype=torch.float32, device=q.device)
     Tk = k.shape[0]
-    dkv_ws = torch.empty((2 * Hq * Tk * D,), dtype=torch.float32, device=q.device) if (Hq > Hkv and D % 4 == 0) else None
+    dkv_ws = torch.empty((2 * Hq * Tk * D,), dtype=torch.float32, device=q.device) if (Hq > Hkv and D % 4 == 0 and split_ws) else None
     st = (ctypes.c_int64 * 16)(q.stride(0), q.stride(1), k.stride(0), k.stride(1), v.stride(0), v.stride(1), o.stride(0), o.stride(1),
                                dout.stride(0), dout.stride(1), dq.stride(0), dq.stride(1), dk.stride(0), dk.stride(1), dv.stride(0), dv.stride(1))
+    if rope is not None:
+        cos, sin = rope
+        _need_cuda(cos, sin)
+        assert cos.dtype == sin.dtype == torch.float32 and cos.is_contiguous() and sin.is_contiguous() and tuple(cos.shape) == tuple(sin.shape) == (Tq, D)
+        assert Tk == Tq, "rope needs keys packed like the queries (self-attention)"
+        rc = _lib.load().rga3_attn_varlen_bwd_rope(q.data_ptr(), k.data_ptr(), v.data_ptr(), o.data_ptr(), dout.data_ptr(), lse.data_ptr(), dq.data_ptr(),
+                                                   dk.data_ptr(), dv.data_ptr(), delta.data_ptr(), cu_q.data_ptr(), cu_k.data_ptr(), cu_q.numel() - 1, int(max_q),
+                                                   int(max_k), Tq, Hq, Hkv, D, ctypes.cast(st, ctypes.c_void_p), float(scale), int(bool(causal)), _ptr(dkv_ws), Tk,
+                                                   cos.data_ptr(), sin.data_ptr(), cos.data_ptr(), sin.data_ptr(), _stream())
+        _lib.check(rc, "attn_varlen_bwd_rope")
+        return dq, dk, dv
     rc = _lib.load().rga3_attn_varlen_bwd(q.data_ptr(), k.data_ptr(), v.data_ptr(), o.data_ptr(), dout.data_ptr(), lse.data_ptr(), dq.data_ptr(),
                                           dk.data_ptr(), dv.data_ptr(), delta.data_ptr(), cu_q.data_ptr(), cu_k.data_ptr(), cu_q.numel() - 1, int(max_q),
                                           int(max_k), Tq, Hq, Hkv, D, ctypes.cast(st, ctypes.c_void_p), float(scale), int(bool(causal)), _ptr(dkv_ws), Tk, _stream())
@@ -1047,6 +1058,33 @@
     _lib.check(L.rga3_dropout_pair_bf16(xa.data_ptr(), xb.data_ptr(), out.data_ptr(), None, xa.numel(), float(pa), int(seed_a), float(pb), int(seed_b), 1, _stream()),
                "dropout_pair_bf16")
     return out
+
+
+def rmsnorm_drop_pair(x, weight, eps: float, pa: float, seed_a: int, pb: float, seed_b: int):
+    _need_cuda(x, weight)
+    assert x.dtype == weight.dtype == torch.bfloat16 and x.dim() == 2 and x.stride(1) == 1 and 0.0 <= pa < 1.0 and 0.0 <= pb < 1.0
+    rows, dim = x.shape
+    if not (x.stride(0) == dim and 2048 <= dim <= 8192 and dim % 8 == 0):
+        y = rmsnorm(x, weight, eps)
+        return (y,) + tuple(dropout_pair(y, pa, seed_a, y, pb, seed_b))
+    y, ya, yb = (torch.empty((rows, dim), dtype=torch.bfloat16, device=x.device) for _ in range(3))
+    _lib.check(_lib.load().rga3_rmsnorm_drop_pair_fwd(x.data_ptr(), weight.data_ptr(), y.data_ptr(), ya.data_ptr(), yb.data_ptr(), rows, dim, x.stride(0), y.stride(0),
+                                                      ya.stride(0), yb.stride(0), float(eps), float(pa), int(seed_a), float(pb), int(seed_b), _stream()),
+               "rmsnorm_drop_pair_fwd")
+    return y, ya, yb
+
+
+def rmsnorm_bwd_lora(x, weight, dy, eps: float, gq, pa: float, seed_a: int, gv, pb: float, seed_b: int, add=None):
+    _need_cuda(x, weight, dy, gq, gv, add)
+    assert x.dim() == 2 and x.dtype == dy.dtype == gq.dtype == gv.dtype == torch.bfloat16 and x.shape == dy.shape == gq.shape == gv.shape
+    assert x.is_contiguous() and dy.is_contiguous() and (add is None or (add.is_contiguous() and add.shape == x.shape and add.dtype == torch.bfloat16))
+    rows, dim = x.shape
+    if not (gq.is_contiguous() and gv.is_contiguous() and 1024 < dim <= 8192 and dim % 8 == 0):
+        return rmsnorm_bwd(x, weight, dropout_pair(gq.contiguous(), pa, seed_a, gv.contiguous(), pb, seed_b, accumulate_into=dy.clone()), eps, add=add)
+    dx = torch.empty_like(x)
+    _lib.check(_lib.load().rga3_rmsnorm_bwd_lora(x.data_ptr(), weight.data_ptr(), dy.data_ptr(), _ptr(add), dx.data_ptr(), gq.data_ptr(), gv.data_ptr(), rows, dim,
+                                                 gq.stride(0), gv.stride(0), float(eps), float(pa), int(seed_a), float(pb), int(seed_b), _stream()), "rmsnorm_bwd_lora")
+    return dx
 
 
 def swiglu_fwd(gu):
diff --git a/rga3-release_amd/rga3/model/qwen_train.py b/rga3-release_amd/rga3/model/qwen_train.py
--- a/rga3-release_amd/rga3/model/qwen_train.py
+++ b/rga3-release_amd/rga3/model/qwen_train.py
@@ -164,6 +164,7 @@
 
 _LORA_FOLD = os.environ.get("RGA3_LORA_FOLD", "1") != "0"
 _SWIGLU_PRE = os.environ.get("RGA3_SWIGLU_PRE", "1") != "0"
+_ROW_FOLDS = {"norm_drop": True, "lora_grad": True, "rope": True}
 _lora_cat = {}
 _lora_cat_store = {}
 
@@ -252,7 +253,14 @@
     return (ops.dropout(h1, pq, seeds[0]) if pq > 0.0 else h1), (ops.dropout(h1, pv, seeds[1]) if pv > 0.0 else h1)
 
 
-def qkv_with_lora(at, h1, seeds=None, want_inputs=False):
+def _norm_drop_ok(at, x, seeds) -> bool:
+    if not _ROW_FOLDS["norm_drop"] or _fp8["on"] or seeds is None or x.shape[0] <= 16 or not _lora_cat_ok(at):
+        return False
+    pq, pv = _lora_dropout(at)
+    return pq > 0.0 and pv > 0.0 and x.is_contiguous()
+
+
+def qkv_with_lora(at, h1, seeds=None, want_inputs=False, dropped=None):
     Hq, Hk, D = at.num_heads, at.num_kv, at.head_dim
     wqkv, bqkv = at._packed()
     lq, lv = _lora_parts(at.q_proj), _lora_parts(at.v_proj)
@@ -262,7 +270,7 @@
         seeds = (next_dropout_seed(lid, 0), next_dropout_seed(lid, 1, advance=False))
     if not _fp8["on"] and h1.shape[0] > 16 and _lora_cat_ok(at):
         r = lq[0].shape[0]
-        hq, hv = _drop_pair(h1, pq, pv, seeds)
+        hq, hv = dropped if dropped is not None else _drop_pair(h1, pq, pv, seeds)
         tt = torch.empty((h1.shape[0], 2 * r), dtype=h1.dtype, device=h1.device)
         tq = ops.gemm(hq, _lora_ops(at.q_proj)[0], out=tt[:, :r])
         tv = ops.gemm(hv, _lora_ops(at.v_proj)[0], out=tt[:, r:])
@@ -328,8 +336,13 @@
     Hq, Hk, D = at.num_heads, at.num_kv, at.head_dim
     T = x.shape[0]
     w1, w2 = layer.input_layernorm, layer.post_attention_layernorm
-    h1 = ops.rmsnorm(x, w1.weight, w1.variance_epsilon)
-    qkv2, tq, tv, hq_in, hv_in = qkv_with_lora(at, h1, seeds=seeds, want_inputs=True)
+    dropped = None
+    if _norm_drop_ok(at, x, seeds):
+        pq, pv = _lora_dropout(at)
+        h1, *dropped = ops.rmsnorm_drop_pair(x, w1.weight, w1.variance_epsilon, pq, seeds[0], pv, seeds[1])
+    else:
+        h1 = ops.rmsnorm(x, w1.weight, w1.variance_epsilon)
+    qkv2, tq, tv, hq_in, hv_in = qkv_with_lora(at, h1, seeds=seeds, want_inputs=True, dropped=dropped)
     qkv = qkv2.view(T, Hq + 2 * Hk, D)
     ops.rope_(qkv, cos, sin, 0, Hq + Hk)
     att, lse = ops.attn_varlen(qkv[:, :Hq], qkv[:, Hq:Hq + Hk], qkv[:, Hq + Hk:], cu, cu, max_len, D ** -0.5, causal=True, return_lse=True)
@@ -418,9 +431,11 @@
             dx1 = ops.rmsnorm_bwd(x1, w2.weight, dh2, w2.variance_epsilon, add=dy)
             datt = _fgemm(dx1, at, "wo_t", (at.o_proj.weight,), lambda: ops.transpose(at.o_proj.weight.detach())).view(T, Hq, D)
             dqkv = torch.empty_like(qkv)
+            rope_fold = ctx.stored and not _fp8["on"] and _ROW_FOLDS["rope"] and D == 128
             ops.attn_varlen_bwd(q, k, v, att, datt, lse, cu, cu, max_len, max_len, D ** -0.5, True, dq=dqkv[:, :Hq], dk=dqkv[:, Hq:Hq + Hk],
-                                dv=dqkv[:, Hq + Hk:])
-            ops.rope_(dqkv, cos, _neg_table(sin), 0, Hq + Hk)
+                                dv=dqkv[:, Hq + Hk:], rope=(cos, _neg_table(sin)) if rope_fold else None)
+            if not rope_fold:
+                ops.rope_(dqkv, cos, _neg_table(sin), 0, Hq + Hk)
             dqkv2 = dqkv.view(T, (Hq + 2 * Hk) * D)
             fold = (not _fp8["on"]) and T > 16 and _lora_cat_ok(at)
             dtt = None
@@ -430,6 +445,7 @@
             else:
                 dh1 = _fgemm(dqkv2, at, "wqkv_t", (at.q_proj.weight, at.k_proj.weight, at.v_proj.weight), lambda: ops.transpose(wqkv))
             grads = [None, None, None, None]
+            pend_norm = None
             if lq is not None or lv is not None:
                 tn_pairs, tn_slots = [], []
                 pend = []
@@ -450,14 +466,20 @@
                         ops.gemm(dt, At, residual=dh1, out=dh1)
                     else:
                         pend.append((ops.gemm(dt, At), pdrop, ctx.seeds[sd]))
-                if len(pend) == 2 and dh1.is_contiguous():
+                if len(pend) == 2 and dh1.is_contiguous() and fold and ctx.stored and _ROW_FOLDS["lora_grad"] and x.is_contiguous():
+                    pend_norm, pend = pend, []
+                elif len(pend) == 2 and dh1.is_contiguous():
                     ops.dropout_pair(pend[0][0], pend[0][1], pend[0][2], pend[1][0], pend[1][1], pend[1][2], accumulate_into=dh1)
                 else:
                     for xg, pg, sg in pend:
                         ops.dropout(xg, pg, sg, out=dh1, accumulate=True)
                 for sl, gw in zip(tn_slots, ops.gemm_tn_many(tn_pairs)):
                     grads[sl] = gw
-            dx = ops.rmsnorm_bwd(x, w1.weight, dh1, w1.variance_epsilon, add=dx1)
+            if pend_norm is not None:
+                (gq, pgq, sq), (gv, pgv, sv) = pend_norm
+                dx = ops.rmsnorm_bwd_lora(x, w1.weight, dh1, w1.variance_epsilon, gq, pgq, sq, gv, pgv, sv, add=dx1)
+            else:
+                dx = ops.rmsnorm_bwd(x, w1.weight, dh1, w1.variance_epsilon, add=dx1)
         return (dx, grads[0], grads[1], grads[2], grads[3], None, None, None, None, None, None)
 
 
```

Result: no change. 7.593, median of 2 (-0.1%).
